# joejep/FOCNeRF

Hardware: AMD Instinct MI355X
Metric: train_samples_per_sec (higher is better)
Workload: dtype f16

## Files before the change

focnerf_amd/_lib.py:

```python
import ctypes
import os

import torch

_HERE = os.path.dirname(os.path.abspath(__file__))
LIB_PATH = os.environ.get("FOCNERF_LIB_PATH") or os.path.join(_HERE, "libfocnerf_hip.so")

c_u8p = ctypes.c_void_p
c_vp = ctypes.c_void_p
u32 = ctypes.c_uint32
u64 = ctypes.c_uint64
f32 = ctypes.c_float
i32 = ctypes.c_int

FOC_F32 = 0
FOC_F16 = 1



class FocOccTrainNode(ctypes.Structure):
    _fields_ = [
        ("struct_bytes", u32),
        ("n_rays", u32), ("max_steps", u32), ("cascade", u32), ("grid_size", u32), ("cap", u32), ("pad_align", u32),
        ("bound", f32), ("dt_gamma", f32), ("min_near", f32),
        ("rays_o", c_vp), ("rays_d", c_vp), ("aabb", c_vp), ("jitter", c_vp),
        ("bitfield", c_vp),
        ("nears", c_vp), ("fars", c_vp), ("enc_in", c_vp), ("deltas", c_vp),
        ("sh_rows", c_vp),
        ("rays", c_vp), ("counter", c_vp), ("march_scratch", c_vp),
        ("levels", u32), ("base_resolution", u32), ("gridtype", u32), ("interp", u32),
        ("align_corners", ctypes.c_int32), ("table_dtype", ctypes.c_int32),
        ("per_level_scale_log2", f32),
        ("embeddings", c_vp),
        ("offsets", c_vp), ("offsets_host", c_vp),
        ("planes", c_vp), ("grid_workspace", c_vp),
        ("grid_workspace_bytes", u64),
        ("sigma_input_dim", u32), ("sigma_hidden", u32), ("sigma_layers", u32), ("sigma_activation", u32), ("sigma_output_activation", u32),
        ("color_hidden", u32), ("color_layers", u32), ("color_activation", u32), ("c_width", u32),
        ("w_sigma", c_vp), ("w_color", c_vp),
        ("h", c_vp), ("c", c_vp),
        ("T_thresh", f32), ("density_scale", f32), ("bg_scalar", f32),
        ("bg_ray", c_vp),
        ("weights_sum", c_vp), ("image_raw", c_vp), ("image", c_vp), ("depth", c_vp),
        ("precounted", ctypes.c_int32),
        ("grad_image", c_vp), ("grad_ws", c_vp),
        ("grad_c", c_vp), ("grad_h0", c_vp), ("grad_h", c_vp), ("grad_planes", c_vp), ("grad_w_color", c_vp), ("grad_w_sigma", c_vp),
        ("grad_embeddings", c_vp), ("mlp_workspace", c_vp),
        ("mlp_workspace_bytes", u64),
    ]


class FocOccTrainObject(ctypes.Structure):
    _fields_ = [
        ("struct_bytes", u32),
        ("input_pad", f32),
        ("obj_feat", c_vp),
        ("ray_sumsq", c_vp),
        ("grad_sumsq", c_vp),
        ("grad_obj", c_vp),
    ]


class FocOccTrainTail(ctypes.Structure):
    _fields_ = [
        ("struct_bytes", u32),
        ("ray_dist", c_vp), ("ray_wm", c_vp), ("depth_raw", c_vp),
        ("grad_dist", c_vp), ("grad_depth", c_vp),
    ]


SIGNATURES = {
    "foc_abi_version": (i32, []),
    "foc_last_error": (ctypes.c_char_p, []),
    "foc_arch": (ctypes.c_char_p, []),
    "foc_near_far_from_aabb": (i32, [c_vp, c_vp, c_vp, u32, f32, c_vp, c_vp, c_vp]),
    "foc_sph_from_ray": (i32, [c_vp, c_vp, f32, u32, c_vp, c_vp]),
    "foc_morton3D": (i32, [c_vp, u32, c_vp, c_vp]),
    "foc_morton3D_invert": (i32, [c_vp, u32, c_vp, c_vp]),
    "foc_packbits": (i32, [c_vp, u32, f32, c_vp, c_vp]),
    "foc_march_rays_train": (i32, [c_vp, c_vp, c_vp, f32, f32, u32, u32, u32, u32, u32, c_vp, c_vp,
                                   c_vp, c_vp, c_vp, c_vp, c_vp, c_vp, c_vp, c_vp]),
    "foc_march_rays_train_field": (i32, [c_vp, c_vp, c_vp, f32, f32, u32, u32, u32, u32, u32, c_vp, c_vp,
                                         c_vp, c_vp, c_vp, c_vp, c_vp, c_vp, c_vp, u32, c_vp, f32, c_vp]),
    "foc_set_option": (i32, [ctypes.c_char_p, i32]),
    "foc_get_option": (i32, [ctypes.c_char_p, c_vp]),
    "foc_guard_pick_device": (i32, [i32, i32, i32, i32]),
    "foc_grid_forward_index_path": (i32, [u32, u32, u32]),
    "foc_view_tile_order": (i32, [c_vp, u32, u32, u32, c_vp, c_vp, c_vp]),
    "foc_occ_train_forward": (i32, [ctypes.POINTER(FocOccTrainNode), c_vp]),
    "foc_occ_train_backward": (i32, [ctypes.POINTER(FocOccTrainNode), c_vp]),
    "foc_occ_train_forward_pad31": (i32, [ctypes.POINTER(FocOccTrainNode), f32, c_vp]),
    "foc_occ_train_backward_pad31": (i32, [ctypes.POINTER(FocOccTrainNode), f32, c_vp]),
    "foc_occ_train_forward_obj": (i32, [ctypes.POINTER(FocOccTrainNode), ctypes.POINTER(FocOccTrainObject), c_vp]),
    "foc_occ_train_backward_obj": (i32, [ctypes.POINTER(FocOccTrainNode), ctypes.POINTER(FocOccTrainObject), c_vp]),
    "foc_occ_tail_forward_sumsq": (i32, [c_vp, c_vp, u32, c_vp, c_vp, u32, u32, f32, f32, c_vp, f32, c_vp, c_vp, c_vp, c_vp, c_vp, c_vp, c_vp, c_vp]),
    "foc_occ_tail_backward_sumsq": (i32, [c_vp, c_vp, c_vp, c_vp, u32, c_vp, c_vp, c_vp, c_vp, c_vp, u32, u32, f32, f32, c_vp, f32, c_vp, c_vp, c_vp, c_vp]),
    "foc_occ_tail_forward": (i32, [c_vp, c_vp, u32, c_vp, c_vp, u32, u32, f32, f32, c_vp, f32, c_vp, c_vp, c_vp, c_vp, c_vp, c_vp, c_vp]),
    "foc_occ_tail_backward": (i32, [c_vp, c_vp, c_vp, c_vp, u32, c_vp, c_vp, c_vp, c_vp, c_vp, u32, u32, f32, f32, c_vp, f32, c_vp, c_vp, c_vp]),
    "foc_occ_tail_forward_dist": (i32, [c_vp, c_vp, u32, c_vp, c_vp, u32, u32, f32, f32, c_vp, f32, c_vp, c_vp, c_vp, c_vp, c_vp, c_vp, c_vp, c_vp, c_vp,
                                        c_vp]),
    "foc_occ_tail_backward_dist": (i32, [c_vp, c_vp, c_vp, c_vp, u32, c_vp, c_vp, c_vp, c_vp, c_vp, u32, u32, f32, f32, c_vp, f32, c_vp, c_vp, c_vp, c_vp,
                                         c_vp, c_vp, c_vp]),
    "foc_occ_tail_forward_depth": (i32, [c_vp, c_vp, u32, c_vp, c_vp, u32, u32, f32, f32, c_vp, f32, c_vp, c_vp, c_vp, c_vp, c_vp, c_vp, c_vp, c_vp, c_vp,
                                         c_vp, c_vp]),
    "foc_occ_tail_backward_depth": (i32, [c_vp, c_vp, c_vp, c_vp, u32, c_vp, c_vp, c_vp, c_vp, c_vp, u32, u32, f32, f32, c_vp, f32, c_vp, c_vp, c_vp, c_vp,
                                          c_vp, c_vp, c_vp, c_vp, c_vp, c_vp, c_vp]),
    "foc_occ_train_forward_tail": (i32, [ctypes.POINTER(FocOccTrainNode), ctypes.POINTER(FocOccTrainObject), f32, ctypes.POINTER(FocOccTrainTail), c_vp]),
    "foc_occ_train_backward_tail": (i32, [ctypes.POINTER(FocOccTrainNode), ctypes.POINTER(FocOccTrainObject), f32, ctypes.POINTER(FocOccTrainTail), c_vp]),
    "foc_march_rays_train_scratch_bytes": (u64, [u32, u32]),
    "foc_composite_rays_train_forward": (i32, [c_vp, c_vp, c_vp, c_vp, u32, u32, f32, c_vp, c_vp, c_vp, c_vp]),
    "foc_composite_rays_train_backward": (i32, [c_vp, c_vp, c_vp, c_vp, c_vp, c_vp, c_vp, c_vp, u32, u32, f32,
                                                c_vp, c_vp, c_vp]),
    "foc_march_rays": (i32, [u32, u32, c_vp, c_vp, c_vp, c_vp, f32, f32, u32, u32, u32, c_vp, c_vp, c_vp,
                             c_vp, c_vp, c_vp, c_vp, c_vp]),
    "foc_composite_rays": (i32, [u32, u32, f32, c_vp, c_vp, c_vp, c_vp, c_vp, c_vp, c_vp, c_vp, c_vp]),
    "foc_compact_alive": (i32, [c_vp, u32, c_vp, c_vp, c_vp, c_vp]),
    "foc_march_rays_two_phase": (i32, [u32, u32, c_vp, c_vp, c_vp, c_vp, f32, f32, u32, u32, u32, c_vp, c_vp, c_vp, c_vp, c_vp, c_vp, c_vp, c_vp, i32, c_vp]),
    "foc_composite_compact": (i32, [u32, u32, f32, c_vp, c_vp, c_vp, c_vp, c_vp, c_vp, c_vp, c_vp, c_vp, c_vp, c_vp, c_vp, u32, u32, i32, c_vp]),
    "foc_march_rays_two_phase_fills": (i32, [u32, i32]),
    "foc_march_rays_two_phase_sample_major": (i32, [u32, u32, i32]),
    "foc_occ_render_step_scratch_bytes": (u64, [u32]),
    "foc_occ_render_step": (i32, [u32, u32, c_vp, c_vp, c_vp, c_vp, c_vp, c_vp, f32, f32, u32, u32, u32, c_vp, c_vp, c_vp, c_vp, c_vp, c_vp, c_vp, c_vp,
                                  c_vp, c_vp, c_vp, u32, f32, u32, c_vp, u32, c_vp, u32, u32, c_vp, f32, c_vp, c_vp, c_vp, c_vp, u32, c_vp, u32, u32, c_vp]),
    "foc_occ_render_step_pad31": (i32, [u32, u32, c_vp, c_vp, c_vp, c_vp, c_vp, c_vp, f32, f32, u32, u32, u32, c_vp, c_vp, c_vp, c_vp, c_vp, c_vp, c_vp, c_vp,
                                        c_vp, c_vp, c_vp, u32, f32, u32, c_vp, u32, c_vp, u32, u32, c_vp, f32, c_vp, c_vp, c_vp, c_vp, u32, c_vp, u32, u32, f32,
                                        c_vp]),
    "foc_occ_render_step_pad": (i32, [u32, u32, c_vp, c_vp, c_vp, c_vp, c_vp, c_vp, f32, f32, u32, u32, u32, c_vp, c_vp, c_vp, c_vp, c_vp, c_vp, c_vp, c_vp,
                                      c_vp, c_vp, c_vp, u32, f32, u32, c_vp, u32, c_vp, u32, u32, c_vp, f32, c_vp, c_vp, c_vp, c_vp, u32, c_vp, u32, u32, f32,
                                      c_vp]),
    "foc_grid_encode_forward": (i32, [c_vp, c_vp, c_vp, c_vp, u32, u32, u32, u32, f32, u32, c_vp, u32, i32, u32,
                                      i32, c_vp, c_vp]),
    "foc_grid_encode_forward_bl": (i32, [c_vp, c_vp, c_vp, c_vp, u32, u32, u32, u32, f32, u32, c_vp, u32, i32, u32,
                                         i32, c_vp, c_vp]),
    "foc_grid_encode_backward": (i32, [c_vp, c_vp, c_vp, c_vp, c_vp, u32, u32, u32, u32, f32, u32, c_vp, c_vp,
                                       u32, i32, u32, i32, i32, c_vp, c_vp]),
    "foc_grid_encode_backward_workspace_bytes": (u64, [u32, u32, u32, u32, i32]),
    "foc_grid_planes_to_rows": (i32, [c_vp, c_vp, u32, u32, u32, c_vp]),
    "foc_grid_rows_to_planes": (i32, [c_vp, c_vp, u32, u32, u32, c_vp]),
    "foc_grid_encode_backward_binned": (i32, [c_vp, c_vp, c_vp, c_vp, c_vp, u32, u32, u32, u32, f32, u32, c_vp, c_vp,
                                              u32, i32, u32, i32, i32, c_vp, c_vp, u64, c_vp]),
    "foc_grid_encode_forward_counted": (i32, [c_vp, c_vp, c_vp, c_vp, u32, u32, u32, u32, f32, u32, u32, i32, u32, i32, c_vp, c_vp, u64, c_vp]),
    "foc_grid_encode_backward_count": (i32, [c_vp, c_vp, u32, u32, u32, u32, f32, u32, u32, i32, u32, i32, c_vp, c_vp, u64, c_vp]),
    "foc_grid_encode_backward_binned_counted": (i32, [c_vp, c_vp, c_vp, c_vp, c_vp, u32, u32, u32, u32, f32, u32, c_vp, c_vp,
                                                      u32, i32, u32, i32, i32, c_vp, c_vp, u64, c_vp]),
    "foc_grad_total_variation": (i32, [c_vp, c_vp, c_vp, c_vp, f32, u32, u32, u32, u32, f32, u32, u32, i32, i32, c_vp]),
    "foc_freq_encode_forward": (i32, [c_vp, u32, u32, u32, u32, c_vp, c_vp]),
    "foc_freq_encode_backward": (i32, [c_vp, c_vp, u32, u32, u32, u32, c_vp, c_vp]),
    "foc_ffmlp_forward": (i32, [c_vp, c_vp, u32, u32, u32, u32, u32, u32, u32, c_vp, c_vp, c_vp]),
    "foc_ffmlp_inference": (i32, [c_vp, c_vp, u32, u32, u32, u32, u32, u32, u32, c_vp, c_vp, c_vp]),
    "foc_ffmlp_backward": (i32, [c_vp, c_vp, c_vp, c_vp, u32, u32, u32, u32, u32, u32, u32, i32,
                                 c_vp, c_vp, c_vp, c_vp, u64, c_vp]),
    "foc_ffmlp_backward_workspace_bytes": (u64, [u32, u32, u32]),
    "foc_ffmlp_forward_planar": (i32, [c_vp, c_vp, u32, u32, u32, u32, u32, u32, u32, c_vp, c_vp]),
    "foc_ffmlp_backward_planar": (i32, [c_vp, c_vp, c_vp, u32, u32, u32, u32, u32, u32, u32, i32, c_vp, c_vp, c_vp, u64, c_vp]),
    "foc_allocate_splitk": (i32, [u64]),
    "foc_free_splitk": (i32, []),
    "foc_combine_select": (i32, [c_vp, c_vp, c_vp, c_vp, u64, c_vp]),
    "foc_combine_pack_keys": (i32, [c_vp, u32, c_vp, u64, c_vp]),
    "foc_combine_unpack": (i32, [c_vp, u32, c_vp, c_vp, c_vp, u64, c_vp]),
    "foc_combine_select_composite": (i32, [c_vp, u32, c_vp, c_vp, u32, u32, c_vp, u32, c_vp, c_vp, c_vp, c_vp]),
    "foc_combine_select4": (i32, [c_vp, c_vp, u64, c_vp]),
    "foc_combine_select_composite_attr": (i32, [c_vp, u32, c_vp, c_vp, u32, c_vp, c_vp, u32, u32, c_vp, u32, c_vp, c_vp, c_vp, c_vp, c_vp, c_vp, c_vp, c_vp]),
    "foc_combine_select4_ids": (i32, [c_vp, u32, c_vp, c_vp, u64, c_vp]),
    "foc_mo_select": (i32, [c_vp, c_vp, c_vp, c_vp, u64, u32, u32, c_vp]),
    "foc_fixed_field_pack": (i32, [c_vp, c_vp, c_vp, c_vp, c_vp, c_vp, f32, u32, u32, f32, f32, c_vp, c_vp, c_vp, c_vp, u32, c_vp]),
    "foc_fixed_cull_scratch_bytes": (u64, [u32, u32]),
    "foc_fixed_cull": (i32, [c_vp, c_vp, c_vp, c_vp, c_vp, u32, u32, f32, c_vp, u32, u32, c_vp, c_vp, c_vp, c_vp, u64, c_vp]),
    "foc_fixed_cull_emit": (i32, [c_vp, c_vp, c_vp, c_vp, c_vp, u32, u32, f32, c_vp, c_vp, u32, c_vp, c_vp, c_vp]),
    "foc_fixed_field_pack_culled": (i32, [c_vp, c_vp, c_vp, c_vp, u32, c_vp, c_vp, u32, u32, f32, f32, c_vp, c_vp]),
    "foc_fixed_cull_placed": (i32, [c_vp, c_vp, c_vp, c_vp, c_vp, u32, u32, c_vp, c_vp, f32, c_vp, u32, u32, c_vp, c_vp, c_vp, c_vp, u64, c_vp]),
    "foc_fixed_cull_emit_placed": (i32, [c_vp, c_vp, c_vp, c_vp, c_vp, u32, u32, c_vp, f32, f32, c_vp, c_vp, u32, c_vp, c_vp, c_vp]),
    "foc_fixed_field_pack_culled_gain": (i32, [c_vp, c_vp, c_vp, c_vp, u32, c_vp, c_vp, u32, u32, f32, f32, f32, c_vp, c_vp]),
    "foc_composite_fixed_steps":(i32, [c_vp, c_vp, c_vp, c_vp, u32, u32, f32, c_vp, c_vp, c_vp]),
    "foc_fixed_sample": (i32, [c_vp, c_vp, c_vp, c_vp, c_vp, c_vp, u32, u32, f32, c_vp, c_vp, c_vp, u32, c_vp]),
    "foc_fixed_tail_forward": (i32, [c_vp, c_vp, c_vp, c_vp, c_vp, c_vp, f32, u32, u32, f32, f32, c_vp, c_vp, c_vp, c_vp, c_vp, c_vp, u32, c_vp, c_vp]),
    "foc_fixed_tail_backward": (i32, [c_vp, c_vp, c_vp, c_vp, c_vp, c_vp, c_vp, c_vp, c_vp, c_vp, c_vp, f32, u32, u32, f32, f32, c_vp, c_vp, u32, c_vp, c_vp]),
    "foc_fixed_tail_forward_dist": (i32, [c_vp, c_vp, c_vp, c_vp, c_vp, c_vp, f32, u32, u32, f32, f32, c_vp, c_vp, c_vp, c_vp, c_vp, c_vp, u32, c_vp, c_vp,
                                          c_vp, c_vp]),
    "foc_fixed_tail_backward_dist": (i32, [c_vp, c_vp, c_vp, c_vp, c_vp, c_vp, c_vp, c_vp, c_vp, c_vp, c_vp, c_vp, f32, u32, u32, f32, f32, c_vp, c_vp, u32,
                                           c_vp, c_vp, c_vp, c_vp, c_vp]),
    "foc_fixed_head_forward": (i32, [c_vp, c_vp, c_vp, c_vp, c_vp, u32, u32, f32, c_vp, c_vp, c_vp, c_vp, c_vp, c_vp, c_vp, u32, c_vp]),
    "foc_fixed_head_backward": (i32, [c_vp, c_vp, c_vp, c_vp, c_vp, c_vp, c_vp, c_vp, c_vp, c_vp, u32, u32, f32, c_vp, u32, c_vp]),
    "foc_color_head_forward": (i32, [c_vp, c_vp, u32, c_vp, u32, u32, u32, u32, c_vp, u32, c_vp, c_vp]),
    "foc_field_forward_train": (i32, [c_vp, c_vp, u32, c_vp, u32, c_vp, u32, u32, u32, u32, c_vp, c_vp, u32, c_vp, c_vp]),
    "foc_color_head_backward": (i32, [c_vp, c_vp, c_vp, u32, c_vp, c_vp, u32, u32, u32, u32, c_vp, c_vp, c_vp, u64, u32, c_vp, c_vp, c_vp]),
    "foc_color_head_forward_pad": (i32, [c_vp, c_vp, u32, c_vp, u32, u32, u32, u32, c_vp, u32, c_vp, f32, c_vp]),
    "foc_color_head_backward_pad": (i32, [c_vp, c_vp, c_vp, u32, c_vp, c_vp, u32, u32, u32, u32, c_vp, c_vp, c_vp, u64, u32, c_vp, c_vp, f32, c_vp]),
    "foc_field_forward_train_pad": (i32, [c_vp, c_vp, u32, c_vp, u32, c_vp, u32, u32, u32, u32, c_vp, c_vp, u32, c_vp, f32, c_vp]),
    "foc_color_head_forward_pad31": (i32, [c_vp, c_vp, u32, c_vp, u32, u32, u32, u32, c_vp, u32, c_vp, f32, c_vp]),
    "foc_color_head_backward_pad31": (i32, [c_vp, c_vp, c_vp, u32, c_vp, c_vp, u32, u32, u32, u32, c_vp, c_vp, c_vp, u64, u32, c_vp, c_vp, f32, c_vp]),
    "foc_field_forward_train_pad31": (i32, [c_vp, c_vp, u32, c_vp, u32, c_vp, u32, u32, u32, u32, c_vp, c_vp, u32, c_vp, f32, c_vp]),
    "foc_fixed_composite_forward": (i32, [c_vp, c_vp, c_vp, f32, u32, u32, f32, c_vp, c_vp]),
    "foc_fixed_composite_backward": (i32, [c_vp, c_vp, c_vp, c_vp, f32, u32, u32, f32, c_vp, c_vp, c_vp]),
    "foc_sample_head_forward": (i32, [c_vp, c_vp, u64, c_vp, c_vp, c_vp, u32, c_vp]),
    "foc_sample_head_backward": (i32, [c_vp, c_vp, c_vp, u64, c_vp, u32, c_vp]),
    "foc_sh_encode": (i32, [c_vp, u64, c_vp, c_vp]),
    "foc_rgb_head_forward": (i32, [c_vp, u64, c_vp, c_vp]),
    "foc_rgb_head_backward": (i32, [c_vp, c_vp, u64, c_vp, c_vp]),
    "foc_fixed_render_inference": (i32, [c_vp, c_vp, c_vp, c_vp, c_vp, c_vp, f32, u32, u32, f32, f32, c_vp, c_vp, c_vp, c_vp, u32, c_vp, c_vp]),
    "foc_nerf_field_inference": (i32, [c_vp, i32, c_vp, u32, u32, u32, c_vp, u32, c_vp, u32, u32, u32, u32, c_vp, c_vp, c_vp, c_vp]),
    "foc_nerf_field_inference_pad": (i32, [c_vp, i32, c_vp, u32, u32, u32, c_vp, u32, c_vp, u32, u32, u32, u32, c_vp, c_vp, c_vp, f32, c_vp]),
    "foc_nerf_field_inference_pad31": (i32, [c_vp, i32, c_vp, u32, u32, u32, c_vp, u32, c_vp, u32, u32, u32, u32, c_vp, c_vp, c_vp, f32, c_vp]),
    "foc_mark_untrained_grid": (i32, [c_vp, u32, f32, f32, f32, f32, f32, u32, u32, c_vp, c_vp, c_vp]),
    "foc_grid_cells_xyz": (i32, [u32, u32, f32, c_vp, c_vp, c_vp]),
    "foc_grid_update_sample_workspace_bytes": (u64, [u32, u32]),
    "foc_grid_update_sample": (i32, [c_vp, u32, u32, f32, u32, c_vp, c_vp, c_vp, c_vp, c_vp, c_vp, u64, c_vp]),
    "foc_grid_update_apply_workspace_bytes": (u64, [u32, u32]),
    "foc_grid_update_apply": (i32, [c_vp, u32, u32, c_vp, c_vp, u32, f32, f32, f32, c_vp, c_vp, c_vp, u64, c_vp]),
    "foc_background_forward": (i32, [c_vp, c_vp, c_vp, f32, u32, c_vp, c_vp, f32, u32, c_vp, c_vp, c_vp]),
    "foc_background_backward_workspace_bytes": (u64, [u32]),
    "foc_background_backward": (i32, [c_vp, c_vp, c_vp, c_vp, f32, u32, c_vp, c_vp, f32, u32, c_vp, c_vp, c_vp, c_vp, u64, c_vp]),
}


def _load():
    if not os.path.exists(LIB_PATH):
        raise ImportError(
            f"focnerf_amd: {LIB_PATH} is missing. Build it with `python -c 'import __graft_entry__ as g; g.build()'` "
            f"or `make -C focnerf_amd/csrc`. There is no CPU or PyTorch fallback for these ops.")
    try:
        lib = ctypes.CDLL(LIB_PATH)
    except OSError as e:
        raise ImportError(f"focnerf_amd: failed to load {LIB_PATH}: {e}") from e
    for name, (res, args) in SIGNATURES.items():
        fn = getattr(lib, name)
        fn.restype = res
        fn.argtypes = args
    return lib


class _Stream(ctypes.c_void_p):
    device_index = None


_multi_device = None


def _on_tensor_device(fn):
    def call(*args):
        global _multi_device
        if _multi_device is None:
            _multi_device = torch.cuda.device_count() > 1
        if _multi_device and args:
            idx = getattr(args[-1], "device_index", None)
            if idx is not None and idx != torch.cuda.current_device():
                with torch.cuda.device(idx):
                    return fn(*args)
        return fn(*args)
    call.__name__ = getattr(fn, "__name__", "foc_call")
    return call


class _Lib:

    def __init__(self, cdll):
        self._cdll = cdll
        for name, (_, args) in SIGNATURES.items():
            fn = getattr(cdll, name)
            setattr(self, name, _on_tensor_device(fn) if args and args[-1] is c_vp and not name.endswith("_bytes") else fn)


lib = _Lib(_load())


def check(rc, what=""):
    if rc != 0:
        msg = lib.foc_last_error().decode("utf-8", "replace")
        raise RuntimeError(f"focnerf_amd {what}: {msg} (code {rc})")


def ptr(t):
    if t is None:
        return None
    return ctypes.c_void_p(t.data_ptr())


_raw_stream = getattr(torch._C, "_cuda_getCurrentRawStream", None) if os.environ.get("FOC_RAW_STREAM", "1") != "0" else None


def raw_stream(index):
    if _raw_stream is not None:
        return _raw_stream(index)
    return torch.cuda.current_stream(index).cuda_stream


def stream_of(t=None):
    dev = t.device if t is not None else None
    index = dev.index if dev is not None and dev.index is not None else torch.cuda.current_device()
    s = _Stream(raw_stream(index))
    s.device_index = index
    return s


def require_cuda(*tensors):
    for t in tensors:
        if t is not None and not t.is_cuda:
            raise RuntimeError("focnerf_amd: expected a CUDA(HIP) tensor; these ops have no CPU implementation")


def dtype_code(t):
    if t.dtype == torch.float32:
        return FOC_F32
    if t.dtype == torch.float16:
        return FOC_F16
    raise RuntimeError(f"focnerf_amd: unsupported dtype {t.dtype} (float32 or float16 expected)")


def get_option(name):
    v = ctypes.c_int(0)
    check(lib.foc_get_option(name.encode(), ctypes.cast(ctypes.byref(v), ctypes.c_void_p)), "get_option")
    return v.value


def set_option(name, value):
    check(lib.foc_set_option(name.encode(), int(value)), "set_option")


class option:

    def __init__(self, name, value):
        self.name, self.value = name, int(value)

    def __enter__(self):
        self.old = get_option(self.name)
        set_option(self.name, self.value)
        return self

# ... 4 lines not shown
```

focnerf_amd/csrc/combine.hip:

```cpp
#include "common.h"
#include "fs_common.h"
#include <string.h>

static thread_local char g_err[512] = "";

void foc_set_error(const char *fmt, ...) {
    va_list ap;
    va_start(ap, fmt);
    vsnprintf(g_err, sizeof(g_err), fmt, ap);
    va_end(ap);
}

__global__ void __launch_bounds__(256) k_combine_select(const float *__restrict__ dens, const float *__restrict__ rgb,
                                                        float *__restrict__ max_dens, float *__restrict__ best_rgb, uint64_t n) {
    for (uint64_t i = (uint64_t)blockIdx.x * 256 + threadIdx.x; i < n; i += (uint64_t)gridDim.x * 256) {
        const float d = dens[i], m = max_dens[i];
        if (d > m) { best_rgb[i * 3] = rgb[i * 3]; best_rgb[i * 3 + 1] = rgb[i * 3 + 1]; best_rgb[i * 3 + 2] = rgb[i * 3 + 2]; }
        max_dens[i] = (d != d || m != m) ? __builtin_nanf("") : (d > m ? d : m);
    }
}

__global__ void __launch_bounds__(256) k_combine_pack(const float *__restrict__ dens, uint32_t rank, uint64_t *__restrict__ keys, uint64_t n) {
    for (uint64_t i = (uint64_t)blockIdx.x * 256 + threadIdx.x; i < n; i += (uint64_t)gridDim.x * 256) {
        float d = dens[i];
// ... 64 lines not shown
__device__ __forceinline__ void combine_select_composite_body(const CombineFields &fields, const CombineAttr *at, uint32_t K,
                                                              const float *__restrict__ nears, const float *__restrict__ fars, uint32_t N,
                                                              uint32_t T, float bg0, float bg1, uint32_t n_bg, float *__restrict__ image4,
                                                              float *__restrict__ depth, float4 *__restrict__ merged4) {
    const uint32_t lane = threadIdx.x & 63;
    const uint32_t n = blockIdx.x * 4 + (threadIdx.x >> 6);
    if (n >= N) return;
    const FsGeom geo = fs_geom(nears, fars, n, T);
    float Tc = 1.0f, r = 0, g = 0, b = 0, a = 0, d = 0, ws = 0;
    float aw[NOBJ > 0 ? NOBJ : 1], ad[NOBJ > 0 ? NOBJ : 1];
    (void)aw; (void)ad;
    if constexpr (NOBJ > 0) {
#pragma unroll
        for (int k = 0; k < NOBJ; k++) aw[k] = ad[k] = 0.0f;
    }
    for (uint32_t base = 0; base < T; base += 64) {
        const uint32_t i = base + lane;
        const bool valid = i < T;
        float alpha = 0, sigma = 0, c0 = 0, c1 = 0, c2 = 0, oz = 0;
        uint32_t win = 0xFFu;
        if (valid) {
            const uint64_t s = (uint64_t)n * T + i;
            float4 best = fields.p[0][s];
            if constexpr (NOBJ > 0) win = at->plane[0] ? (uint32_t)at->plane[0][s] : at->id[0];
            for (uint32_t k = 1; k < K; k++) {
                const float4 f = fields.p[k][s];
                const float m = best.x;
                if constexpr (NOBJ > 0) {
                    const uint32_t idk = at->plane[k] ? (uint32_t)at->plane[k][s] : at->id[k];
                    if (f.x > m) win = idk;
                }
                if (f.x > m) { best.y = f.y; best.z = f.z; best.w = f.w; }
                best.x = (f.x != f.x || m != m) ? __builtin_nanf("") : (f.x > m ? f.x : m);
            }
            if (merged4) merged4[s] = best;
            if constexpr (NOBJ > 0) {
                if (at->winner) at->winner[s] = (uint8_t)win;
            }
            sigma = best.x; c0 = best.y; c1 = best.z; c2 = best.w;
            const FsSample p = fs_sample(geo, i, i, T, false, 0.0f, 0.0f);
            alpha = 1 - __expf(-p.delta * sigma);
            oz = p.oz;
        }
        const float om = valid ? (1 - alpha + 1e-15f) : 1.0f;
        const float w = alpha * fs_trans_scan(om, lane, Tc);
        r = fmaf(w, c0, r); g = fmaf(w, c1, g); b = fmaf(w, c2, b);
        a = fmaf(w, sigma, a); d = fmaf(w, oz, d); ws += w;
        if constexpr (NOBJ > 0) {
#pragma unroll
            for (int k = 0; k < NOBJ; k++) {
                const bool mine = win == (uint32_t)k;
                aw[k] = mine ? aw[k] + w : aw[k];
                ad[k] = mine ? fmaf(w, oz, ad[k]) : ad[k];
            }
        }
    }
    r = wave_sum(r); g = wave_sum(g); b = wave_sum(b); a = wave_sum(a); d = wave_sum(d); ws = wave_sum(ws);
    if constexpr (NOBJ > 0) {
        const uint32_t n_obj = at->n_obj;
        float my_w = 0.0f, my_d = 0.0f, top = 0.0f;
        int32_t inst = -1;
#pragma unroll
        for (int k = 0; k < NOBJ; k++) {
            if ((uint32_t)k < n_obj) {
                const float sw = wave_sum(aw[k]), sd = wave_sum(ad[k]);
                if (lane == (uint32_t)k) { my_w = sw; my_d = sd; }
                if (sw > top) { top = sw; inst = k; }
            }
        }
        if (lane < n_obj) {
            at->obj_weights[(uint64_t)n * n_obj + lane] = my_w;
            at->obj_depth[(uint64_t)n * n_obj + lane] = my_d;
        }
        if (lane == 0) at->instance[n] = inst;
    }
    if (lane == 0) {
        for (uint32_t q = 0; q < n_bg; q++) {
            const float rest = (1 - ws) * (q == 0 ? bg0 : bg1);
            const float o[4] = {r + rest, g + rest, b + rest, a + rest};
#pragma unroll
            for (int k = 0; k < 4; k++) image4[((uint64_t)q * N + n) * 4 + k] = fminf(1.0f, fmaxf(0.0f, o[k]));
        }
        depth[n] = d;
    }
}

__global__ void __launch_bounds__(256) k_combine_select_composite(CombineFields fields, uint32_t K, const float *__restrict__ nears,
                                                                  const float *__restrict__ fars, uint32_t N, uint32_t T, float bg0, float bg1,
                                                                  uint32_t n_bg, float *__restrict__ image4, float *__restrict__ depth,
                                                                  float4 *__restrict__ merged4) {
    combine_select_composite_body<0>(fields, nullptr, K, nears, fars, N, T, bg0, bg1, n_bg, image4, depth, merged4);
}

template <int NOBJ>
__global__ void __launch_bounds__(256) k_combine_select_composite_attr(CombineFields fields, CombineAttr at, uint32_t K,
                                                                       const float *__restrict__ nears, const float *__restrict__ fars, uint32_t N,
                                                                       uint32_t T, float bg0, float bg1, uint32_t n_bg, float *__restrict__ image4,
                                                                       float *__restrict__ depth, float4 *__restrict__ merged4) {
    combine_select_composite_body<NOBJ>(fields, &at, K, nears, fars, N, T, bg0, bg1, n_bg, image4, depth, merged4);
}

__global__ void __launch_bounds__(256) k_combine_select4(const float4 *__restrict__ f4, float4 *__restrict__ acc4, uint64_t n) {
    for (uint64_t i = (uint64_t)blockIdx.x * 256 + threadIdx.x; i < n; i += (uint64_t)gridDim.x * 256) {
        const float4 f = f4[i];
        float4 best = acc4[i];
        const float m = best.x;
        if (f.x > m) { best.y = f.y; best.z = f.z; best.w = f.w; }
        best.x = (f.x != f.x || m != m) ? __builtin_nanf("") : (f.x > m ? f.x : m);
        acc4[i] = best;
    }
}

__global__ void __launch_bounds__(256) k_combine_select4_ids(const float4 *__restrict__ f4, uint8_t id, float4 *__restrict__ acc4,
                                                             uint8_t *__restrict__ acc_ids, uint64_t n) {
    for (uint64_t i = (uint64_t)blockIdx.x * 256 + threadIdx.x; i < n; i += (uint64_t)gridDim.x * 256) {
        const float4 f = f4[i];
        float4 best = acc4[i];
        const float m = best.x;
        if (f.x > m) { best.y = f.y; best.z = f.z; best.w = f.w; acc_ids[i] = id; }
        best.x = (f.x != f.x || m != m) ? __builtin_nanf("") : (f.x > m ? f.x : m);
        acc4[i] = best;
    }
}

template <typename T>
__global__ void __launch_bounds__(256) k_mo_select(const T *__restrict__ sig_new, const T *__restrict__ feat_new, T *__restrict__ sig_best,
                                                   T *__restrict__ feat_best, uint64_t n, uint32_t width) {
    const uint64_t s0 = ((uint64_t)blockIdx.x * 4u + (threadIdx.x >> 6)) * 64u;
    if (s0 >= n) return;
    const uint32_t lane = threadIdx.x & 63u;
    bool take = false;
    if (s0 + lane < n) {
        const T a_raw = sig_new[s0 + lane];
        const float a = (float)a_raw, b = (float)sig_best[s0 + lane];
        take = (a != a) || (b == b && a >= b);
        if (take) sig_best[s0 + lane] = a_raw;
    }
    const uint64_t rows = __ballot(take);
    const uint32_t live = (uint32_t)(n - s0 < 64u ? n - s0 : 64u);
    const uint64_t base = s0 * width;
    for (uint32_t e = lane; e < live * width; e += 64u)
        if ((rows >> (e / width)) & 1ull) feat_best[base + e] = feat_new[base + e];
}

#include <stdlib.h>
#include <string.h>
#include <atomic>
#include <mutex>
struct FocOptionRow { const char *name; std::atomic<int> value; };
static FocOptionRow foc_option_table[FOC_OPT_COUNT] = {
    {"FOC_MLP_BWD_FUSED", 1}, {"FOC_FIELD_FWD_FUSED", 1}, {"FOC_GB_MERGE_MAX_RES", 480}, {"FOC_GB_FACTORED", 1}, {"FOC_GB_TAIL_SPLIT", 16}, {"FOC_GRID_FUSE_SMALL", 1},
    {"FOC_GRID_PAIRS", 1}, {"FOC_GRID_FAST", 1}, {"FOC_MARCH_SERIAL", -1}, {"FOC_MARCH_RAYS_ROW_MAX", 131072}, {"FOC_OCC_MARCH_FORM", -1},
    {"FOC_OCC_SAMPLE_MAJOR", 1}, {"FOC_OCC_FIELD_PIECE", 1 << 23}, {"FOC_DETERMINISTIC", 0},
};
static int foc_option_parse(int which, const char *text) {
    if (which == FOC_OPT_OCC_MARCH_FORM) {
        if (text[0] == 't') return 0;
        if (text[0] == 'r') return 1;
        if (text[0] == 'l') return 2;
        if (text[0] == 's') return 3;
    }
    return atoi(text);
}
static void foc_options_init() {
    static std::once_flag once;
    std::call_once(once, [] {
        for (int i = 0; i < FOC_OPT_COUNT; i++) {
            const char *e = getenv(foc_option_table[i].name);
            if (e && e[0]) foc_option_table[i].value.store(foc_option_parse(i, e), std::memory_order_relaxed);
        }
    });
}
int foc_opt(FocOpt which) { foc_options_init(); return foc_option_table[which].value.load(std::memory_order_relaxed); }

extern "C" {

int foc_set_option(const char *name, int value) {
    foc_options_init();
    for (int i = 0; i < FOC_OPT_COUNT; i++)
        if (name && strcmp(name, foc_option_table[i].name) == 0) { foc_option_table[i].value.store(value, std::memory_order_relaxed); return FOC_OK; }
    foc_set_error("set_option: unknown option '%s'", name ? name : "(null)");
    return FOC_E_INVALID;
}

int foc_get_option(const char *name, int *value) {
    foc_options_init();
    for (int i = 0; i < FOC_OPT_COUNT; i++)
        if (name && value && strcmp(name, foc_option_table[i].name) == 0) { *value = foc_option_table[i].value.load(std::memory_order_relaxed); return FOC_OK; }
    foc_set_error("get_option: unknown option '%s'", name ? name : "(null)");
    return FOC_E_INVALID;
}

int foc_guard_pick_device(int stream_is_null, int stream_device, int pointer_device, int current_device) {
    return foc_guard_pick(stream_is_null != 0, stream_device, pointer_device, current_device);
}


int foc_combine_select_composite(const float *const *fields4, uint32_t K, const float *nears, const float *fars, uint32_t N, uint32_t T,
                                 const float *bgs, uint32_t n_bg, float *image4, float *depth, float *merged4, void *stream) {
    FocDeviceGuard foc_guard_(stream, nears);
    FOC_REQUIRE(K >= 1 && K <= FOC_COMBINE_MAX_OBJECTS, FOC_E_INVALID, "combine_select_composite: 1 <= K <= %d objects per call (got %u)",
                FOC_COMBINE_MAX_OBJECTS, K);
    FOC_REQUIRE(n_bg >= 1 && n_bg <= 2 && bgs, FOC_E_INVALID, "combine_select_composite: one or two backgrounds");
    FOC_REQUIRE(T >= 2, FOC_E_INVALID, "combine_select_composite: T must be >= 2");
    if (N == 0) return FOC_OK;
    FOC_REQUIRE(fields4 && nears && fars && image4 && depth, FOC_E_INVALID, "combine_select_composite: null pointer");
    CombineFields f;
    for (uint32_t k = 0; k < FOC_COMBINE_MAX_OBJECTS; k++) {
        f.p[k] = reinterpret_cast<const float4 *>(k < K ? fields4[k] : fields4[0]);
        FOC_REQUIRE(f.p[k] && ((uintptr_t)f.p[k] & 15) == 0, FOC_E_INVALID, "combine_select_composite: field %u is null or not 16-byte aligned", k);
    }
    FOC_REQUIRE(((uintptr_t)merged4 & 15) == 0, FOC_E_INVALID, "combine_select_composite: merged4 must be 16-byte aligned");
    hipLaunchKernelGGL(k_combine_select_composite, dim3(foc_div_up(N, 4)), dim3(256), 0, (hipStream_t)stream, f, K, nears, fars, N, T, bgs[0],
                       n_bg > 1 ? bgs[1] : 0.0f, n_bg, image4, depth, reinterpret_cast<float4 *>(merged4));
    FOC_CHECK_LAUNCH("combine_select_composite");
    return FOC_OK;
}

int foc_combine_select4(const float *field4, float *acc4, uint64_t n, void *stream) {
    FocDeviceGuard foc_guard_(stream, field4);
    FOC_REQUIRE(n == 0 || (field4 && acc4), FOC_E_INVALID, "combine_select4: null pointer");
    FOC_REQUIRE((((uintptr_t)field4 | (uintptr_t)acc4) & 15) == 0, FOC_E_INVALID, "combine_select4: fields must be 16-byte aligned");
    if (n == 0) return FOC_OK;
    hipLaunchKernelGGL(k_combine_select4, dim3(foc_grid_1d(n, 256)), dim3(256), 0, (hipStream_t)stream, reinterpret_cast<const float4 *>(field4),
                       reinterpret_cast<float4 *>(acc4), n);
    FOC_CHECK_LAUNCH("combine_select4");
    return FOC_OK;
}

int foc_combine_select_composite_attr(const float *const *fields4, uint32_t K, const uint8_t *const *id_planes, const uint32_t *ids,
                                      uint32_t n_obj, const float *nears, const float *fars, uint32_t N, uint32_t T, const float *bgs,
                                      uint32_t n_bg, float *image4, float *depth, float *merged4, float *obj_weights, float *obj_depth,
                                      int32_t *instance, uint8_t *winner, void *stream) {
    FocDeviceGuard foc_guard_(stream, nears);
    FOC_REQUIRE(K >= 1 && K <= FOC_COMBINE_MAX_OBJECTS, FOC_E_INVALID, "combine_select_composite_attr: 1 <= K <= %d fields per call (got %u)",
                FOC_COMBINE_MAX_OBJECTS, K);
    FOC_REQUIRE(n_obj >= 1 && n_obj <= FOC_COMBINE_MAX_OBJECTS, FOC_E_INVALID, "combine_select_composite_attr: 1 <= n_obj <= %d objects (got %u)",
                FOC_COMBINE_MAX_OBJECTS, n_obj);
    FOC_REQUIRE(n_bg >= 1 && n_bg <= 2 && bgs, FOC_E_INVALID, "combine_select_composite_attr: one or two backgrounds");
    FOC_REQUIRE(T >= 2, FOC_E_INVALID, "combine_select_composite_attr: T must be >= 2");
    FOC_REQUIRE(fields4, FOC_E_INVALID, "combine_select_composite_attr: fields4 is null");
    CombineFields f;
    CombineAttr at;
    for (uint32_t k = 0; k < FOC_COMBINE_MAX_OBJECTS; k++) {
        const uint32_t j = k < K ? k : 0;
        at.plane[k] = id_planes ? id_planes[j] : nullptr;
        FOC_REQUIRE(at.plane[k] || ids, FOC_E_INVALID, "combine_select_composite_attr: field %u has neither an id plane nor a constant id (ids is null)", j);
        at.id[k] = at.plane[k] ? 0u : ids[j];
        FOC_REQUIRE(at.id[k] < n_obj, FOC_E_INVALID, "combine_select_composite_attr: ids[%u] = %u is not below n_obj = %u", j, at.id[k], n_obj);
    }
    if (N == 0) return FOC_OK;
    FOC_REQUIRE(nears && fars && image4 && depth, FOC_E_INVALID, "combine_select_composite_attr: null pointer");
    FOC_REQUIRE(obj_weights && obj_depth && instance, FOC_E_INVALID, "combine_select_composite_attr: obj_weights, obj_depth and instance must not be null");
    for (uint32_t k = 0; k < FOC_COMBINE_MAX_OBJECTS; k++) {
        f.p[k] = reinterpret_cast<const float4 *>(k < K ? fields4[k] : fields4[0]);
        FOC_REQUIRE(f.p[k] && ((uintptr_t)f.p[k] & 15) == 0, FOC_E_INVALID, "combine_select_composite_attr: field %u is null or not 16-byte aligned", k);
    }
    FOC_REQUIRE(((uintptr_t)merged4 & 15) == 0, FOC_E_INVALID, "combine_select_composite_attr: merged4 must be 16-byte aligned");
    FOC_REQUIRE(((uintptr_t)obj_weights & 3) == 0 && ((uintptr_t)obj_depth & 3) == 0 && ((uintptr_t)instance & 3) == 0, FOC_E_INVALID,
                "combine_select_composite_attr: obj_weights, obj_depth and instance must be 4-byte aligned");
    at.n_obj = n_obj;
    at.obj_weights = obj_weights; at.obj_depth = obj_depth; at.instance = instance; at.winner = winner;
    const dim3 grid(foc_div_up(N, 4)), block(256);
    const float bg1 = n_bg > 1 ? bgs[1] : 0.0f;
    float4 *m4 = reinterpret_cast<float4 *>(merged4);
    if (n_obj <= 4)
        hipLaunchKernelGGL(k_combine_select_composite_attr<4>, grid, block, 0, (hipStream_t)stream, f, at, K, nears, fars, N, T, bgs[0], bg1, n_bg, image4, depth, m4);
    else if (n_obj <= 8)
        hipLaunchKernelGGL(k_combine_select_composite_attr<8>, grid, block, 0, (hipStream_t)stream, f, at, K, nears, fars, N, T, bgs[0], bg1, n_bg, image4, depth, m4);
    else
        hipLaunchKernelGGL(k_combine_select_composite_attr<16>, grid, block, 0, (hipStream_t)stream, f, at, K, nears, fars, N, T, bgs[0], bg1, n_bg, image4, depth, m4);
    FOC_CHECK_LAUNCH("combine_select_composite_attr");
    return FOC_OK;
}

int foc_combine_select4_ids(const float *field4, uint32_t id, float *acc4, uint8_t *acc_ids, uint64_t n, void *stream) {
    FocDeviceGuard foc_guard_(stream, field4);
    FOC_REQUIRE(id < FOC_COMBINE_MAX_OBJECTS, FOC_E_INVALID, "combine_select4_ids: id %u is not below %d", id, FOC_COMBINE_MAX_OBJECTS);
    FOC_REQUIRE(n == 0 || (field4 && acc4 && acc_ids), FOC_E_INVALID, "combine_select4_ids: null pointer");
    FOC_REQUIRE((((uintptr_t)field4 | (uintptr_t)acc4) & 15) == 0, FOC_E_INVALID, "combine_select4_ids: fields must be 16-byte aligned");
    if (n == 0) return FOC_OK;
    hipLaunchKernelGGL(k_combine_select4_ids, dim3(foc_grid_1d(n, 256)), dim3(256), 0, (hipStream_t)stream, reinterpret_cast<const float4 *>(field4),
                       (uint8_t)id, reinterpret_cast<float4 *>(acc4), acc_ids, n);
    FOC_CHECK_LAUNCH("combine_select4_ids");
    return FOC_OK;
}

int foc_mo_select(const void *sigma_new, const void *feat_new, void *sigma_best, void *feat_best, uint64_t n, uint32_t feat_width,
                  uint32_t elem_bytes, void *stream) {
    FocDeviceGuard foc_guard_(stream, sigma_new);
    FOC_REQUIRE(elem_bytes == 2 || elem_bytes == 4, FOC_E_INVALID, "mo_select: elem_bytes must be 2 (half) or 4 (float), got %u", elem_bytes);
    FOC_REQUIRE(feat_width >= 1 && feat_width <= 64, FOC_E_INVALID, "mo_select: feat_width %u outside 1..64", feat_width);
    FOC_REQUIRE(n == 0 || (sigma_new && feat_new && sigma_best && feat_best), FOC_E_INVALID, "mo_select: null pointer");
    FOC_REQUIRE(n < (1ull << 38), FOC_E_INVALID, "mo_select: n too large");
    if (n == 0) return FOC_OK;
    const dim3 grid((uint32_t)((n + 255u) / 256u));
    if (elem_bytes == 2)
        hipLaunchKernelGGL(k_mo_select<__half>, grid, dim3(256), 0, (hipStream_t)stream, (const __half *)sigma_new, (const __half *)feat_new,
                           (__half *)sigma_best, (__half *)feat_best, n, feat_width);
    else
        hipLaunchKernelGGL(k_mo_select<float>, grid, dim3(256), 0, (hipStream_t)stream, (const float *)sigma_new, (const float *)feat_new,
                           (float *)sigma_best, (float *)feat_best, n, feat_width);
    FOC_CHECK_LAUNCH("mo_select");
    return FOC_OK;
}

// ... 44 lines not shown
```

focnerf_amd/csrc/common.h:

```cpp
#pragma once
#include <hip/hip_runtime.h>
#include <hip/hip_fp16.h>
#include <stdint.h>
#include <stdio.h>
#include <stdarg.h>
#include "../../include/focnerf.h"

#define FOC_WAVE 64

void foc_set_error(const char *fmt, ...);

enum FocOpt {
    FOC_OPT_MLP_BWD_FUSED,
    FOC_OPT_FIELD_FWD_FUSED,
    FOC_OPT_GB_MERGE_MAX_RES,
    FOC_OPT_GB_FACTORED,
    FOC_OPT_GB_TAIL_SPLIT,
    FOC_OPT_GRID_FUSE_SMALL,
    FOC_OPT_GRID_PAIRS,
    FOC_OPT_GRID_FAST,
    FOC_OPT_MARCH_SERIAL,
    FOC_OPT_MARCH_RAYS_ROW_MAX,
    FOC_OPT_OCC_MARCH_FORM,
    FOC_OPT_OCC_SAMPLE_MAJOR,
    FOC_OPT_OCC_FIELD_PIECE,
    FOC_OPT_DETERMINISTIC,
    FOC_OPT_COUNT
};
int foc_opt(FocOpt which);

#define FOC_REQUIRE(cond, code, ...)                    \
    do {                                                \
        if (!(cond)) {                                  \
            foc_set_error(__VA_ARGS__);                 \
            return (code);                              \
        }                                               \
    } while (0)

#define FOC_CHECK_LAUNCH(name)                                                     \
    do {                                                                           \
        hipError_t e_ = hipGetLastError();                                         \
        if (e_ != hipSuccess) {                                                    \
            foc_set_error("%s: launch failed: %s", name, hipGetErrorString(e_));   \
            return FOC_E_LAUNCH;                                                   \
        }                                                                          \
    } while (0)

static inline int foc_guard_pick(bool stream_is_null, int stream_device, int pointer_device, int current_device) {
    if (!stream_is_null && stream_device >= 0) return stream_device;
    if (pointer_device >= 0) return pointer_device;
    return current_device;
}
struct FocDeviceGuard {
    int prev = -1;
    explicit FocDeviceGuard(void *stream, const void *first_pointer = nullptr) {
        static int n_devices = -1;
        if (n_devices < 0 && hipGetDeviceCount(&n_devices) != hipSuccess) { (void)hipGetLastError(); n_devices = 0; }
        if (n_devices == 1) return;
        int cur = 0;
        if (hipGetDevice(&cur) != hipSuccess) return;
        int sdev = -1, pdev = -1;
        if (stream != nullptr) {
            if (hipStreamGetDevice(static_cast<hipStream_t>(stream), &sdev) != hipSuccess) { (void)hipGetLastError(); sdev = -1; }
        } else if (first_pointer != nullptr) {
            hipPointerAttribute_t attr;
            if (hipPointerGetAttributes(&attr, first_pointer) == hipSuccess && attr.type == hipMemoryTypeDevice) pdev = attr.device;
            else (void)hipGetLastError();
        }
        const int want = foc_guard_pick(stream == nullptr, sdev, pdev, cur);
        if (want != cur && hipSetDevice(want) == hipSuccess) prev = cur;
    }
    ~FocDeviceGuard() { if (prev >= 0) (void)hipSetDevice(prev); }
    FocDeviceGuard(const FocDeviceGuard &) = delete;
    FocDeviceGuard &operator=(const FocDeviceGuard &) = delete;
};

static inline uint32_t foc_div_up(uint64_t a, uint64_t b) { return (uint32_t)((a + b - 1) / b); }

static inline uint32_t foc_grid_1d(uint64_t n, uint32_t block, uint32_t max_blocks = 256 * 8) {
    uint64_t g = (n + block - 1) / block;
    if (g < 1) g = 1;
    if (g > max_blocks) g = max_blocks;
    return (uint32_t)g;
}

__device__ __forceinline__ _Float16 foc_f2h(float v) { asm volatile("" : "+v"(v)); return (_Float16)v; }

__global__ static void __launch_bounds__(256) k_foc_zero(uint32_t *__restrict__ p, uint64_t n_words) {
    for (uint64_t i = (uint64_t)blockIdx.x * 256 + threadIdx.x; i < n_words; i += (uint64_t)gridDim.x * 256) p[i] = 0u;
}
static inline hipError_t foc_zero_async(void *p, size_t bytes, hipStream_t st) {
    const uint64_t n = bytes / 4;
    if (n == 0) return hipSuccess;
    uint64_t blocks = (n + 255) / 256;
    if (blocks > 4096) blocks = 4096;
    hipLaunchKernelGGL(k_foc_zero, dim3((uint32_t)blocks), dim3(256), 0, st, reinterpret_cast<uint32_t *>(p), n);
    return hipGetLastError();
}

__device__ __forceinline__ void foc_lds_barrier() { asm volatile("s_waitcnt lgkmcnt(0)\n\ts_barrier" ::: "memory"); }

__device__ __forceinline__ float wave_sum(float v) {
#pragma unroll
    for (int o = 32; o > 0; o >>= 1) v += __shfl_xor(v, o, 64);
    return v;
}
__device__ __forceinline__ int wave_sum_i(int v) {
#pragma unroll
    for (int o = 32; o > 0; o >>= 1) v += __shfl_xor(v, o, 64);
    return v;
}
__device__ __forceinline__ float wave_incl_prod(float v, int lane) {
#pragma unroll
    for (int o = 1; o < 64; o <<= 1) {
        float u = __shfl_up(v, o, 64);
        if (lane >= o) v *= u;
    }
    return v;
}
__device__ __forceinline__ float wave_prod_scan(float om, uint32_t lane, float &P) {
    P = wave_incl_prod(om, (int)lane);
    float Pex = __shfl_up(P, 1, 64);
    if (lane == 0) Pex = 1.0f;
    return Pex;
}
__device__ __forceinline__ float wave_incl_sum(float v, int lane) {
#pragma unroll
    for (int o = 1; o < 64; o <<= 1) {
        float u = __shfl_up(v, o, 64);
        if (lane >= o) v += u;
    }
    return v;
}
__device__ __forceinline__ int wave_incl_sum_i(int v, int lane) {
#pragma unroll
    for (int o = 1; o < 64; o <<= 1) {
        int u = __shfl_up(v, o, 64);
        if (lane >= o) v += u;
    }
    return v;
}
```

focnerf_amd/csrc/fixedstep.hip:

```cpp
#include "common.h"
#include "fs_common.h"
#include <float.h>

__global__ void __launch_bounds__(256) k_fs_sample(const float *__restrict__ rays_o, const float *__restrict__ rays_d, const float *__restrict__ nears,
                                                   const float *__restrict__ fars, const float *__restrict__ aabb, const float *__restrict__ noise,
                                                   uint32_t N, uint32_t T, float bound, float *__restrict__ xyzs, float *__restrict__ enc_in,
                                                   _Float16 *__restrict__ ray_sh, uint32_t ray_block) {
    const uint64_t total = ray_block ? (uint64_t)((N + FS_RAY_BLOCK - 1) / FS_RAY_BLOCK) * FS_RAY_BLOCK * T : (uint64_t)N * T;
    const FsBox box = fs_box(aabb);
    const float two_b = 2 * bound;
    for (uint64_t s = (uint64_t)blockIdx.x * 256 + threadIdx.x; s < total; s += (uint64_t)gridDim.x * 256) {
        uint32_t n, i;
        bool own = true;
        if (ray_block) {
            const uint32_t blk = (uint32_t)(s / ((uint64_t)FS_RAY_BLOCK * T)), in = (uint32_t)(s - (uint64_t)blk * FS_RAY_BLOCK * T);
            i = in / FS_RAY_BLOCK;
            n = blk * FS_RAY_BLOCK + in % FS_RAY_BLOCK;
            own = n < N;
            n = own ? n : N - 1;
        } else {
            n = (uint32_t)(s / T); i = (uint32_t)(s - (uint64_t)n * T);
        }
        const FsGeom g = fs_geom(nears, fars, n, T);
        const float z = fs_z(g, i, T, noise, (uint64_t)n * T + i);
        float x, y, w;
        fs_point(rays_o[n * 3], rays_o[n * 3 + 1], rays_o[n * 3 + 2], rays_d[n * 3], rays_d[n * 3 + 1], rays_d[n * 3 + 2], z, box, x, y, w);
        if (xyzs) { xyzs[s * 3] = x; xyzs[s * 3 + 1] = y; xyzs[s * 3 + 2] = w; }
        if (enc_in) { enc_in[s * 3] = fs_norm(x, bound, two_b); enc_in[s * 3 + 1] = fs_norm(y, bound, two_b); enc_in[s * 3 + 2] = fs_norm(w, bound, two_b); }
        if (ray_sh && i == 0 && own) {
            h8 lo, hi;
            foc_sh16_h(rays_d[n * 3], rays_d[n * 3 + 1], rays_d[n * 3 + 2], lo, hi);
            h8 *dst = reinterpret_cast<h8 *>(ray_sh + (uint64_t)n * 16);
            dst[0] = lo; dst[1] = hi;
        }
    }
}

__global__ void __launch_bounds__(256) k_fs_head_fwd(const _Float16 *__restrict__ h, const float *__restrict__ rays_d, const float *__restrict__ nears,
                                                     const float *__restrict__ fars, const float *__restrict__ noise, uint32_t N, uint32_t T,
                                                     float density_scale, float *__restrict__ sigma_out, float *__restrict__ trans_out,
                                                     float *__restrict__ weights_out, float *__restrict__ weights_sum, float *__restrict__ depth,
                                                     _Float16 *__restrict__ cin, const _Float16 *__restrict__ obj, uint32_t cin_ld) {
    const uint32_t lane = threadIdx.x & 63;
    const uint32_t n = blockIdx.x * 4 + (threadIdx.x >> 6);
    if (n >= N) return;
    const FsGeom g = fs_geom(nears, fars, n, T);
    h8 shlo, shhi;
    h8 ob1 = {0, 0, 0, 0, 0, 0, 0, 0}, ob2 = {0, 0, 0, 0, 0, 0, 0, 0};
    _Float16 ob0 = (_Float16)0;
    if (cin) {
        foc_sh16_h(rays_d[n * 3], rays_d[n * 3 + 1], rays_d[n * 3 + 2], shlo, shhi);
        if (obj) {
            ob0 = obj[0];
#pragma unroll
            for (int k = 0; k < 8; k++) ob1[k] = obj[1 + k];
#pragma unroll
            for (int k = 0; k < 7; k++) ob2[k] = obj[9 + k];
        }
    }
    float Tc = 1.0f, ws = 0, dp = 0;
    for (uint32_t base = 0; base < T; base += 64) {
        const uint32_t i = base + lane;
        const bool valid = i < T;
        const uint64_t s = (uint64_t)n * T + (valid ? i : T - 1);
        h8 r0, r1;
        if (cin) { r0 = *reinterpret_cast<const h8 *>(h + s * 16); r1 = *reinterpret_cast<const h8 *>(h + s * 16 + 8); }
        else r0[0] = h[s * 16];
        const float sigma = expf((float)r0[0]);
        const FsSample p = fs_sample_ld(g, i, valid ? i : T - 1, T, noise, s);
        const float alpha = valid ? 1 - expf((-p.delta * density_scale) * sigma) : 0.0f;
        const float om = valid ? (1 - alpha + 1e-15f) : 1.0f;
        const float Tb = fs_trans_scan(om, lane, Tc);
        const float w = alpha * Tb;
        if (valid) {
            sigma_out[s] = sigma; trans_out[s] = Tb; weights_out[s] = w;
            ws += w; dp += w * p.oz;
            if (cin) {
                h8 c2, c3;
#pragma unroll
                for (int k = 0; k < 7; k++) { c2[k] = r0[k + 1]; c3[k] = r1[k + 1]; }
                c2[7] = r1[0]; c3[7] = ob0;
                h8 *dst = reinterpret_cast<h8 *>(cin + s * cin_ld);
                dst[0] = shlo; dst[1] = shhi; dst[2] = c2; dst[3] = c3;
                if (cin_ld == 48) { dst[4] = ob1; dst[5] = ob2; }
            }
        }
    }
    ws = wave_sum(ws); dp = wave_sum(dp);
    if (lane == 0) { weights_sum[n] = ws; depth[n] = dp; }
}

__global__ void __launch_bounds__(256) k_fs_head_bwd(const _Float16 *__restrict__ h, const float *__restrict__ sigma_in, const float *__restrict__ trans_in,
                                                     const float *__restrict__ nears, const float *__restrict__ fars, const float *__restrict__ noise,
                                                     const float *__restrict__ grad_w, const float *__restrict__ grad_ws, const float *__restrict__ grad_depth,
                                                     const _Float16 *__restrict__ grad_cin, uint32_t N, uint32_t T, float density_scale,
                                                     _Float16 *__restrict__ grad_h, uint32_t cin_ld) {
    const uint32_t lane = threadIdx.x & 63;
    const uint32_t n = blockIdx.x * 4 + (threadIdx.x >> 6);
    if (n >= N) return;
    const FsGeom g = fs_geom(nears, fars, n, T);
    const float gws = grad_ws ? grad_ws[n] : 0.0f, gdp = grad_depth ? grad_depth[n] : 0.0f;
    float S_carry = 0.0f;
    const uint32_t n_chunks = (T + 63) / 64;
    for (uint32_t cidx = n_chunks; cidx-- > 0;) {
        const uint32_t i = cidx * 64 + lane;
        const bool valid = i < T;
        const uint64_t s = (uint64_t)n * T + (valid ? i : T - 1);
        const float sigma = sigma_in[s], Tb = trans_in[s];
        const FsSample p = fs_sample_ld(g, i, valid ? i : T - 1, T, noise, s);
        const float dsigma = fs_head_bwd_step(p, valid, sigma, Tb, (grad_w ? grad_w[s] : 0.0f) + gws, gdp, density_scale, lane, S_carry);
        const float dh0 = dsigma * foc_trunc_exp_bwd((float)h[s * 16]);
        if (valid) {
            h8 o0, o1;
            if (grad_cin) {
                const h8 c2 = *reinterpret_cast<const h8 *>(grad_cin + s * cin_ld + 16), c3 = *reinterpret_cast<const h8 *>(grad_cin + s * cin_ld + 24);
#pragma unroll
                for (int k = 0; k < 7; k++) { o0[k + 1] = c2[k]; o1[k + 1] = c3[k]; }
                o1[0] = c2[7];
            } else {
#pragma unroll
                for (int k = 0; k < 8; k++) { o0[k] = (_Float16)0; o1[k] = (_Float16)0; }
            }
            o0[0] = foc_f2h(dh0);
            h8 *dst = reinterpret_cast<h8 *>(grad_h + s * 16);
            dst[0] = o0; dst[1] = o1;
        }
    }
}

__global__ void __launch_bounds__(256) k_fs_composite_fwd(const _Float16 *__restrict__ c, const float *__restrict__ weights, const float *__restrict__ bg_ray,
                                                          float bg_scalar, uint32_t N, uint32_t T, float thresh, float *__restrict__ image) {
    const uint32_t lane = threadIdx.x & 63;
    const uint32_t n = blockIdx.x * 4 + (threadIdx.x >> 6);
    if (n >= N) return;
    float r = 0, g = 0, b = 0, ws = 0;
    for (uint32_t i = lane; i < T; i += 64) {
        const uint64_t s = (uint64_t)n * T + i;
        const float w = weights[s];
        ws += w;
        if (w > thresh) {
            const uint2 raw = *reinterpret_cast<const uint2 *>(c + s * 16);
            const _Float16 *cc = reinterpret_cast<const _Float16 *>(&raw);
            r += w * foc_sigmoid_h((float)cc[0]); g += w * foc_sigmoid_h((float)cc[1]); b += w * foc_sigmoid_h((float)cc[2]);
        }
    }
    r = wave_sum(r); g = wave_sum(g); b = wave_sum(b); ws = wave_sum(ws);
    if (lane == 0) {
        const FocBg bg = foc_bg(bg_ray, bg_scalar, n);
        image[n * 3] = r + (1 - ws) * bg.b0; image[n * 3 + 1] = g + (1 - ws) * bg.b1; image[n * 3 + 2] = b + (1 - ws) * bg.b2;
    }
}

__global__ void __launch_bounds__(256) k_fs_composite_bwd(const float *__restrict__ grad_image, const _Float16 *__restrict__ c, const float *__restrict__ weights,
                                                          const float *__restrict__ bg_ray, float bg_scalar, uint32_t N, uint32_t T, float thresh,
                                                          _Float16 *__restrict__ grad_c, float *__restrict__ grad_w) {
    const uint64_t total = (uint64_t)N * T;
    for (uint64_t s = (uint64_t)blockIdx.x * 256 + threadIdx.x; s < total; s += (uint64_t)gridDim.x * 256) {
        const uint32_t n = (uint32_t)(s / T);
        const FsRayGrad q = fs_ray_grad(grad_image, bg_ray, bg_scalar, n);
        h8 o0;
        const h8 o1 = {0, 0, 0, 0, 0, 0, 0, 0};
        grad_w[s] = fs_composite_bwd_sample(q, weights[s], thresh, c + s * 16, o0);
        h8 *dst = reinterpret_cast<h8 *>(grad_c + s * 16);
        dst[0] = o0; dst[1] = o1;
    }
}

template <bool NOISE, bool DIST>
__global__ void __launch_bounds__(256) k_fs_tail_fwd(const _Float16 *__restrict__ h, const _Float16 *__restrict__ c, const float *__restrict__ nears,
                                                     const float *__restrict__ fars, const float *__restrict__ noise, const float *__restrict__ bg_ray,
                                                     float bg_scalar, uint32_t N, uint32_t T, float density_scale, float thresh,
                                                     float *__restrict__ sigma_out, float *__restrict__ trans_out, float *__restrict__ weights_out,
                                                     float *__restrict__ weights_sum, float *__restrict__ depth, float *__restrict__ image, uint32_t c_ld,
                                                     float *__restrict__ ray_sumsq, float *__restrict__ ray_dist, float *__restrict__ ray_wm) {
    const uint32_t lane = threadIdx.x & 63;
    const uint32_t n = blockIdx.x * 4 + (threadIdx.x >> 6);
    if (n >= N) return;
    const FsGeom g = fs_geom(nears, fars, n, T);
    float Tc = 1.0f, ws = 0, dp = 0, r = 0, gg = 0, b = 0, sq = 0;
    FsDist dist = {0, 0, 0};
    const bool live = g.far > g.near;
    for (uint32_t base = 0; base < T; base += 64) {
        const uint32_t i = base + lane;
        const bool valid = i < T;
        const uint32_t ic = valid ? i : T - 1;
        const uint64_t s = (uint64_t)n * T + ic;
        const _Float16 h0 = h[s * 16];
        const uint2 raw = *reinterpret_cast<const uint2 *>(c + s * c_ld);
        float u0 = 0.0f, u1 = 0.0f;
        if (NOISE) { u0 = noise[s]; u1 = noise[(uint64_t)n * T + min(ic + 1u, T - 1u)]; }
        const float sigma = expf((float)h0);
        const FsSample p = fs_sample(g, i, ic, T, NOISE, u0, u1);
        const float alpha = valid ? 1 - expf((-p.delta * density_scale) * sigma) : 0.0f;
        const float om = valid ? (1 - alpha + 1e-15f) : 1.0f;
        const float Tb = fs_trans_scan(om, lane, Tc);
        const float w = alpha * Tb;
        if constexpr (DIST) {
            if (live) fs_dist_fwd_step(dist, w, fs_dist_m(g, p), p.delta, lane);
        }
        if (valid) {
            sigma_out[s] = sigma; trans_out[s] = Tb; weights_out[s] = w;
            ws += w; dp += w * p.oz; sq = fmaf(sigma, sigma, sq);
            if (w > thresh) {
                const _Float16 *cc = reinterpret_cast<const _Float16 *>(&raw);
                r += w * foc_sigmoid_h((float)cc[0]); gg += w * foc_sigmoid_h((float)cc[1]); b += w * foc_sigmoid_h((float)cc[2]);
            }
        }
    }
    ws = wave_sum(ws); dp = wave_sum(dp); r = wave_sum(r); gg = wave_sum(gg); b = wave_sum(b);
    if (ray_sumsq) {
        sq = wave_sum(sq);
        if (lane == 0) ray_sumsq[n] = sq;
    }
    if constexpr (DIST) {
        const float ds = wave_sum(dist.acc);
        if (lane == 0) { ray_dist[n] = ds; ray_wm[n] = dist.WM; }
    }
    if (lane == 0) {
        const FocBg bg = foc_bg(bg_ray, bg_scalar, n);
        image[n * 3] = r + (1 - ws) * bg.b0; image[n * 3 + 1] = gg + (1 - ws) * bg.b1; image[n * 3 + 2] = b + (1 - ws) * bg.b2;
        weights_sum[n] = ws; depth[n] = dp;
    }
}

template <bool NOISE, bool DIST>
__global__ void __launch_bounds__(256) k_fs_tail_bwd(const float *__restrict__ grad_image, const float *__restrict__ grad_ws, const float *__restrict__ grad_depth,
                                                     const _Float16 *__restrict__ c, const float *__restrict__ sigma_in, const float *__restrict__ trans_in,
                                                     const float *__restrict__ weights, const float *__restrict__ nears, const float *__restrict__ fars,
                                                     const float *__restrict__ noise, const float *__restrict__ bg_ray, float bg_scalar, uint32_t N, uint32_t T,
                                                     float density_scale, float thresh, _Float16 *__restrict__ grad_c, _Float16 *__restrict__ grad_h0, uint32_t c_ld,
                                                     const float *__restrict__ grad_sumsq, const float *__restrict__ weights_sum,
                                                     const float *__restrict__ ray_wm, const float *__restrict__ grad_dist) {
    const uint32_t lane = threadIdx.x & 63;
    const uint32_t n = blockIdx.x * 4 + (threadIdx.x >> 6);
    if (n >= N) return;
    const FsGeom g = fs_geom(nears, fars, n, T);
    const float gws = grad_ws ? grad_ws[n] : 0.0f, gdp = grad_depth ? grad_depth[n] : 0.0f;
    const float gsq2 = grad_sumsq ? 2.0f * grad_sumsq[n] : 0.0f;
    float gdist = 0.0f, W_total = 0.0f, WM_total = 0.0f;
    FsDist dist = {0, 0, 0};
    if constexpr (DIST) {
        if (g.far > g.near) gdist = grad_dist[n];
        W_total = weights_sum[n]; WM_total = ray_wm[n];
    }
    const FsRayGrad q = fs_ray_grad(grad_image, bg_ray, bg_scalar, n);
    const FocExp15 e15 = foc_exp15();
    float S_carry = 0.0f;
    const uint32_t n_chunks = (T + 63) / 64;
    for (uint32_t cidx = n_chunks; cidx-- > 0;) {
        const uint32_t i = cidx * 64 + lane;
        const bool valid = i < T;
        const uint32_t ic = valid ? i : T - 1;
        const uint64_t s = (uint64_t)n * T + ic;
        const float sigma = sigma_in[s], Tb = trans_in[s], w = weights[s];
        const uint2 raw = *reinterpret_cast<const uint2 *>(c + s * c_ld);
        float u0 = 0.0f, u1 = 0.0f;
        if (NOISE) { u0 = noise[s]; u1 = noise[(uint64_t)n * T + min(ic + 1u, T - 1u)]; }
        h8 o0;
        const h8 o1 = {0, 0, 0, 0, 0, 0, 0, 0};
        const float gw = fs_composite_bwd_sample(q, w, thresh, reinterpret_cast<const _Float16 *>(&raw), o0);
        if (valid) {
            if (c_ld == 4u) *reinterpret_cast<uint2 *>(grad_c + s * 4) = *reinterpret_cast<const uint2 *>(&o0);
            else { h8 *dst = reinterpret_cast<h8 *>(grad_c + s * 16); dst[0] = o0; dst[1] = o1; }
        }
        const FsSample p = fs_sample(g, i, ic, T, NOISE, u0, u1);
        float gi = gw + gws;
        if constexpr (DIST) {
            if (gdist != 0.0f) gi = fmaf(gdist, fs_dist_bwd_step(dist, valid ? w : 0.0f, fs_dist_m(g, p), p.delta, W_total, WM_total, lane), gi);
        }
        float dsigma = fs_head_bwd_step(p, valid, sigma, Tb, gi, gdp, density_scale, lane, S_carry);
        if (gsq2 != 0.0f) dsigma = fmaf(gsq2, sigma, dsigma);
        const float dh0 = dsigma * foc_trunc_exp_bwd_of_sigma(sigma, e15);
        if (valid) grad_h0[s] = foc_f2h(dh0);
    }
}


template <bool PACK>
__device__ __forceinline__ void fs_infer_finish(FsRayAcc &a, uint32_t n, uint32_t lane, const float *__restrict__ bg_ray, float bg_scalar,
                                                float *__restrict__ image, float *__restrict__ depth, float *__restrict__ weights_sum) {
    const float ws = wave_sum(a.ws), dp = wave_sum(a.dp), r = wave_sum(a.r), gg = wave_sum(a.g), b = wave_sum(a.b);
    if (lane == 0 && (!PACK || image)) {
        const FocBg bg = foc_bg(bg_ray, bg_scalar, n);
        image[n * 3] = r + (1 - ws) * bg.b0; image[n * 3 + 1] = gg + (1 - ws) * bg.b1; image[n * 3 + 2] = b + (1 - ws) * bg.b2;
        depth[n] = dp;
        weights_sum[n] = ws;
    }
}

template <bool PACK>
__global__ void __launch_bounds__(256) k_fs_render_infer(const float *__restrict__ sigma_in, const float *__restrict__ rgb_in, const float *__restrict__ nears,
                                                         const float *__restrict__ fars, const float *__restrict__ noise, const float *__restrict__ bg_ray,
                                                         float bg_scalar, uint32_t N, uint32_t T, float density_scale, float thresh,
                                                         float *__restrict__ image, float *__restrict__ depth, float *__restrict__ weights_sum,
                                                         float *__restrict__ rgb_masked, float4 *__restrict__ field4) {
    const uint32_t lane = threadIdx.x & 63;
    const uint32_t n = blockIdx.x * 4 + (threadIdx.x >> 6);
    if (n >= N) return;
    const FsGeom g = fs_geom(nears, fars, n, T);
    FsRayAcc a = {1.0f, 0, 0, 0, 0, 0};
    for (uint32_t base = 0; base < T; base += 64) {
        const uint32_t i = base + lane;
        const bool valid = i < T;
        const uint64_t s = (uint64_t)n * T + (valid ? i : T - 1);
        const float sigma = sigma_in[s];
        float c0 = 0, c1 = 0, c2 = 0;
        if (valid) { c0 = rgb_in[s * 3]; c1 = rgb_in[s * 3 + 1]; c2 = rgb_in[s * 3 + 2]; }
        fs_infer_tile<PACK>(a, g, n, i, lane, T, sigma, c0, c1, c2, noise, density_scale, thresh, rgb_masked, field4, nullptr);
    }
    fs_infer_finish<PACK>(a, n, lane, bg_ray, bg_scalar, image, depth, weights_sum);
}

#define FS_BLK_RAYS 16u
template <bool PACK>
__global__ void __launch_bounds__(1024) k_fs_render_infer_blk(const float *__restrict__ sigma_in, const float *__restrict__ rgb_in, const float *__restrict__ nears,
                                                              const float *__restrict__ fars, const float *__restrict__ noise, const float *__restrict__ bg_ray,
                                                              float bg_scalar, uint32_t N, uint32_t T, float density_scale, float thresh,
                                                              float *__restrict__ image, float *__restrict__ depth, float *__restrict__ weights_sum,
                                                              float *__restrict__ rgb_masked, float4 *__restrict__ field4, float *__restrict__ sigma_rm) {
    __shared__ float tile_s[64][FS_BLK_RAYS + 1];
    __shared__ float tile_c[64][FS_BLK_RAYS * 3 + 1];
    const uint32_t tid = threadIdx.x, lane = tid & 63;
    const uint32_t wv = __builtin_amdgcn_readfirstlane(tid >> 6);
    const uint32_t n0 = blockIdx.x * FS_BLK_RAYS;
    const uint64_t row0 = fs_block_row(n0, 0, T);
    const bool is_s = tid < 256;
    const uint32_t li = is_s ? tid : tid - 256;
    const uint32_t l_step = is_s ? li >> 2 : li / 12, l_part = is_s ? (li & 3) : li % 12;
    const float *src = is_s ? sigma_in + row0 + l_part * 4 : rgb_in + row0 * 3 + l_part * 4;
    const uint32_t src_ld = is_s ? FS_RAY_BLOCK : FS_RAY_BLOCK * 3;
    float *dst = is_s ? &tile_s[l_step][l_part * 4] : &tile_c[l_step][l_part * 4];
    float4 nx = make_float4(0, 0, 0, 0);
    if (l_step < T) nx = *reinterpret_cast<const float4 *>(src + (uint64_t)l_step * src_ld);
    const uint32_t n = n0 + wv;
    const bool own = n < N;
    const FsGeom g = fs_geom(nears, fars, own ? n : N - 1, T);
    FsRayAcc a = {1.0f, 0, 0, 0, 0, 0};
    for (uint32_t base = 0; base < T; base += 64) {
        dst[0] = nx.x; dst[1] = nx.y; dst[2] = nx.z; dst[3] = nx.w;
        __syncthreads();
        if (base + 64 + l_step < T) nx = *reinterpret_cast<const float4 *>(src + (uint64_t)(base + 64 + l_step) * src_ld);
        if (own)
            fs_infer_tile<PACK>(a, g, n, base + lane, lane, T, tile_s[lane][wv], tile_c[lane][wv * 3], tile_c[lane][wv * 3 + 1], tile_c[lane][wv * 3 + 2],
                                noise, density_scale, thresh, rgb_masked, field4, sigma_rm);
        __syncthreads();
    }
    if (own) fs_infer_finish<PACK>(a, n, lane, bg_ray, bg_scalar, image, depth, weights_sum);
}

struct VtState { uint32_t count, first_enc, bad, pad; };

__device__ __forceinline__ bool vt_turn(const float *__restrict__ d, uint32_t i) {
    const float ax = d[(i + 1) * 3] - d[i * 3], ay = d[(i + 1) * 3 + 1] - d[i * 3 + 1], az = d[(i + 1) * 3 + 2] - d[i * 3 + 2];
    const float bx = d[(i + 2) * 3] - d[(i + 1) * 3], by = d[(i + 2) * 3 + 1] - d[(i + 1) * 3 + 1], bz = d[(i + 2) * 3 + 2] - d[(i + 1) * 3 + 2];
    return (bx * ax + by * ay) + bz * az < 0.0f;
}

__global__ void __launch_bounds__(256) k_vt_find(const float *__restrict__ d, uint32_t N, VtState *__restrict__ st) {
    for (uint32_t i = blockIdx.x * 256 + threadIdx.x; i + 2 < N; i += gridDim.x * 256)
        if (vt_turn(d, i)) { atomicAdd(&st->count, 1u); atomicMax(&st->first_enc, N - i); }
}

__global__ void __launch_bounds__(256) k_vt_check(const float *__restrict__ d, uint32_t N, VtState *__restrict__ st) {
    const uint32_t fe = st->first_enc;
    if (fe == 0u) return;
    const uint32_t W = N - fe + 2u;
    for (uint32_t i = blockIdx.x * 256 + threadIdx.x; i + 2 < N; i += gridDim.x * 256) {
        const bool expect = (i + 2u) % W == 0u || (i + 1u) % W == 0u;
        if (vt_turn(d, i) != expect) st->bad = 1u;
    }
}

__global__ void __launch_bounds__(256) k_vt_perm(uint32_t N, uint32_t th, uint32_t tw, const VtState *__restrict__ st, int64_t *__restrict__ perm) {
    const uint32_t fe = st->first_enc, W = fe ? N - fe + 2u : 0u;
    const uint32_t H = W ? N / W : 0u;
    const bool grid = W >= 16u && N % W == 0u && H >= 8u && st->count == 2u * (H - 1u) && st->bad == 0u;
    for (uint32_t p = blockIdx.x * 256 + threadIdx.x; p < N; p += gridDim.x * 256) {
        uint32_t src = p;
        if (grid) {
            const uint64_t wt = (uint64_t)W * th;
            const uint32_t ty = (uint32_t)(p / wt), rem = (uint32_t)(p - ty * wt);
            const uint32_t rows_here = min(th, H - ty * th);
            const uint32_t tx = min(rem / (rows_here * tw), (W - 1u) / tw), r2 = rem - tx * rows_here * tw;
            const uint32_t cols_here = min(tw, W - tx * tw);
            src = (ty * th + r2 / cols_here) * W + tx * tw + r2 % cols_here;
        }
        perm[p] = (int64_t)src;
    }
}

extern "C" {

int foc_fixed_sample(const float *rays_o, const float *rays_d, const float *nears, const float *fars, const float *aabb, const float *noise,
                     uint32_t N, uint32_t T, float bound, float *xyzs, float *enc_in, void *ray_sh, uint32_t ray_block, void *stream) {
    FocDeviceGuard foc_guard_(stream, rays_o);
    if (N == 0) return FOC_OK;
    FOC_REQUIRE(rays_o && rays_d && nears && fars && aabb && (xyzs || enc_in), FOC_E_INVALID, "fixed_sample: null pointer");
    FOC_REQUIRE(T >= 2, FOC_E_INVALID, "fixed_sample: T must be >= 2");
    FOC_REQUIRE(ray_block == 0 || ray_block == FS_RAY_BLOCK, FOC_E_INVALID, "fixed_sample: ray_block must be 0 (ray-major) or %u (got %u)", FS_RAY_BLOCK, ray_block);
    const uint64_t rows = ray_block ? (uint64_t)foc_div_up(N, FS_RAY_BLOCK) * FS_RAY_BLOCK * T : (uint64_t)N * T;
    hipLaunchKernelGGL(k_fs_sample, dim3(foc_grid_1d(rows, 256, 256 * 16)), dim3(256), 0, (hipStream_t)stream, rays_o, rays_d, nears, fars, aabb,
                       noise, N, T, bound, xyzs, enc_in, (_Float16 *)ray_sh, ray_block);
    FOC_CHECK_LAUNCH("fixed_sample");
    return FOC_OK;
}

int foc_fixed_head_forward(const void *h, const float *rays_d, const float *nears, const float *fars, const float *noise, uint32_t N, uint32_t T,
                           float density_scale, float *sigma, float *trans, float *weights, float *weights_sum, float *depth, void *cin,
                           const void *obj_feat, uint32_t cin_width, void *stream) {
    FocDeviceGuard foc_guard_(stream, h);
    if (N == 0) return FOC_OK;
    FOC_REQUIRE(h && rays_d && nears && fars && sigma && trans && weights && weights_sum && depth, FOC_E_INVALID, "fixed_head_forward: null pointer");
    FOC_REQUIRE(T >= 2, FOC_E_INVALID, "fixed_head_forward: T must be >= 2");
    FOC_REQUIRE(cin_width == 32 || cin_width == 48, FOC_E_INVALID, "fixed_head_forward: cin_width must be 32 or 48 (got %u)", cin_width);
    FOC_REQUIRE(!obj_feat || cin_width == 48, FOC_E_INVALID, "fixed_head_forward: an object feature needs the 48-wide colour input");
    hipLaunchKernelGGL(k_fs_head_fwd, dim3(foc_div_up(N, 4)), dim3(256), 0, (hipStream_t)stream, (const _Float16 *)h, rays_d, nears, fars, noise, N, T,
                       density_scale, sigma, trans, weights, weights_sum, depth, (_Float16 *)cin, (const _Float16 *)obj_feat, cin_width);
    FOC_CHECK_LAUNCH("fixed_head_forward");
    return FOC_OK;
}

int foc_fixed_head_backward(const void *h, const float *sigma, const float *trans, const float *nears, const float *fars, const float *noise,
                            const float *grad_w, const float *grad_ws, const float *grad_depth, const void *grad_cin, uint32_t N, uint32_t T,
                            float density_scale, void *grad_h, uint32_t cin_width, void *stream) {
    FocDeviceGuard foc_guard_(stream, h);
    if (N == 0) return FOC_OK;
    FOC_REQUIRE(h && sigma && trans && nears && fars && grad_h, FOC_E_INVALID, "fixed_head_backward: null pointer");
    FOC_REQUIRE(T >= 2, FOC_E_INVALID, "fixed_head_backward: T must be >= 2");
    FOC_REQUIRE(cin_width == 32 || cin_width == 48, FOC_E_INVALID, "fixed_head_backward: cin_width must be 32 or 48 (got %u)", cin_width);
    hipLaunchKernelGGL(k_fs_head_bwd, dim3(foc_div_up(N, 4)), dim3(256), 0, (hipStream_t)stream, (const _Float16 *)h, sigma, trans, nears, fars, noise,
                       grad_w, grad_ws, grad_depth, (const _Float16 *)grad_cin, N, T, density_scale, (_Float16 *)grad_h, cin_width);
    FOC_CHECK_LAUNCH("fixed_head_backward");
    return FOC_OK;
}

int foc_fixed_composite_forward(const void *c, const float *weights, const float *bg_ray, float bg_scalar, uint32_t N, uint32_t T, float thresh,
                                float *image, void *stream) {
    FocDeviceGuard foc_guard_(stream, c);
    if (N == 0) return FOC_OK;
    FOC_REQUIRE(c && weights && image, FOC_E_INVALID, "fixed_composite_forward: null pointer");
    hipLaunchKernelGGL(k_fs_composite_fwd, dim3(foc_div_up(N, 4)), dim3(256), 0, (hipStream_t)stream, (const _Float16 *)c, weights, bg_ray, bg_scalar, N, T,
                       thresh, image);
    FOC_CHECK_LAUNCH("fixed_composite_forward");
    return FOC_OK;
}

int foc_fixed_composite_backward(const float *grad_image, const void *c, const float *weights, const float *bg_ray, float bg_scalar, uint32_t N,
                                 uint32_t T, float thresh, void *grad_c, float *grad_w, void *stream) {
    FocDeviceGuard foc_guard_(stream, grad_image);
    if (N == 0) return FOC_OK;
    FOC_REQUIRE(grad_image && c && weights && grad_c && grad_w, FOC_E_INVALID, "fixed_composite_backward: null pointer");
    hipLaunchKernelGGL(k_fs_composite_bwd, dim3(foc_grid_1d((uint64_t)N * T, 256, 256 * 16)), dim3(256), 0, (hipStream_t)stream, grad_image,
                       (const _Float16 *)c, weights, bg_ray, bg_scalar, N, T, thresh, (_Float16 *)grad_c, grad_w);
    FOC_CHECK_LAUNCH("fixed_composite_backward");
    return FOC_OK;
}

static int fixed_tail_forward(const char *who, const void *h, const void *c, const float *nears, const float *fars, const float *noise, const float *bg_ray,
                              float bg_scalar, uint32_t N, uint32_t T, float density_scale, float thresh, float *sigma, float *trans, float *weights,
                              float *weights_sum, float *depth, float *image, uint32_t c_width, float *ray_sumsq, float *ray_dist, float *ray_wm, void *stream) {
    FocDeviceGuard foc_guard_(stream, h);
    if (N == 0) return FOC_OK;
    FOC_REQUIRE(c_width == 16 || c_width == 4, FOC_E_INVALID, "%s: c_width must be 16 or 4 (got %u)", who, c_width);
    FOC_REQUIRE(h && c && nears && fars && sigma && trans && weights && weights_sum && depth && image, FOC_E_INVALID, "%s: null pointer", who);
    FOC_REQUIRE(T >= 2, FOC_E_INVALID, "%s: T must be >= 2", who);
    auto kern = ray_dist ? (noise ? k_fs_tail_fwd<true, true> : k_fs_tail_fwd<false, true>) : (noise ? k_fs_tail_fwd<true, false> : k_fs_tail_fwd<false, false>);
    hipLaunchKernelGGL(kern, dim3(foc_div_up(N, 4)), dim3(256), 0, (hipStream_t)stream, (const _Float16 *)h, (const _Float16 *)c, nears, fars, noise,
                       bg_ray, bg_scalar, N, T, density_scale, thresh, sigma, trans, weights, weights_sum, depth, image, c_width, ray_sumsq, ray_dist, ray_wm);
    FOC_CHECK_LAUNCH(who);
    return FOC_OK;
}

int foc_fixed_tail_forward(const void *h, const void *c, const float *nears, const float *fars, const float *noise, const float *bg_ray, float bg_scalar,
                           uint32_t N, uint32_t T, float density_scale, float thresh, float *sigma, float *trans, float *weights, float *weights_sum,
                           float *depth, float *image, uint32_t c_width, float *ray_sumsq, void *stream) {
    return fixed_tail_forward("fixed_tail_forward", h, c, nears, fars, noise, bg_ray, bg_scalar, N, T, density_scale, thresh, sigma, trans, weights, weights_sum,
                              depth, image, c_width, ray_sumsq, nullptr, nullptr, stream);
}

int foc_fixed_tail_forward_dist(const void *h, const void *c, const float *nears, const float *fars, const float *noise, const float *bg_ray, float bg_scalar,
                                uint32_t N, uint32_t T, float density_scale, float thresh, float *sigma, float *trans, float *weights, float *weights_sum,
                                float *depth, float *image, uint32_t c_width, float *ray_sumsq, float *ray_dist, float *ray_wm, void *stream) {
    FOC_REQUIRE((ray_dist && ray_wm) || N == 0, FOC_E_INVALID, "fixed_tail_forward_dist: null ray_dist / ray_wm");
    return fixed_tail_forward("fixed_tail_forward_dist", h, c, nears, fars, noise, bg_ray, bg_scalar, N, T, density_scale, thresh, sigma, trans, weights,
                              weights_sum, depth, image, c_width, ray_sumsq, ray_dist, ray_wm, stream);
}

static int fixed_tail_backward(const char *who, const float *grad_image, const float *grad_ws, const float *grad_depth, const void *c, const float *sigma,
                               const float *trans, const float *weights, const float *nears, const float *fars, const float *noise, const float *bg_ray,
                               float bg_scalar, uint32_t N, uint32_t T, float density_scale, float thresh, void *grad_c, void *grad_h0, uint32_t c_width,
                               const float *grad_sumsq, const float *weights_sum, const float *ray_wm, const float *grad_dist, void *stream) {
    FocDeviceGuard foc_guard_(stream, grad_image);
    if (N == 0) return FOC_OK;
    FOC_REQUIRE(c_width == 16 || c_width == 4, FOC_E_INVALID, "%s: c_width must be 16 or 4 (got %u)", who, c_width);
    FOC_REQUIRE(grad_image && c && sigma && trans && weights && nears && fars && grad_c && grad_h0, FOC_E_INVALID, "%s: null pointer", who);
    FOC_REQUIRE(T >= 2, FOC_E_INVALID, "%s: T must be >= 2", who);
    auto kern = grad_dist ? (noise ? k_fs_tail_bwd<true, true> : k_fs_tail_bwd<false, true>) : (noise ? k_fs_tail_bwd<true, false> : k_fs_tail_bwd<false, false>);
    hipLaunchKernelGGL(kern, dim3(foc_div_up(N, 4)), dim3(256), 0, (hipStream_t)stream, grad_image, grad_ws, grad_depth, (const _Float16 *)c, sigma,
                       trans, weights, nears, fars, noise, bg_ray, bg_scalar, N, T, density_scale, thresh, (_Float16 *)grad_c, (_Float16 *)grad_h0, c_width,
                       grad_sumsq, weights_sum, ray_wm, grad_dist);
    FOC_CHECK_LAUNCH(who);
    return FOC_OK;
}

int foc_fixed_tail_backward(const float *grad_image, const float *grad_ws, const float *grad_depth, const void *c, const float *sigma, const float *trans,
                            const float *weights, const float *nears, const float *fars, const float *noise, const float *bg_ray, float bg_scalar,
                            uint32_t N, uint32_t T, float density_scale, float thresh, void *grad_c, void *grad_h0, uint32_t c_width, const float *grad_sumsq,
                            void *stream) {
    return fixed_tail_backward("fixed_tail_backward", grad_image, grad_ws, grad_depth, c, sigma, trans, weights, nears, fars, noise, bg_ray, bg_scalar, N, T,
                               density_scale, thresh, grad_c, grad_h0, c_width, grad_sumsq, nullptr, nullptr, nullptr, stream);
}

int foc_fixed_tail_backward_dist(const float *grad_image, const float *grad_ws, const float *grad_depth, const void *c, const float *sigma, const float *trans,
                                 const float *weights, const float *weights_sum, const float *nears, const float *fars, const float *noise, const float *bg_ray,
                                 float bg_scalar, uint32_t N, uint32_t T, float density_scale, float thresh, void *grad_c, void *grad_h0, uint32_t c_width,
                                 const float *grad_sumsq, const float *ray_wm, const float *ray_dist, const float *grad_dist, void *stream) {
    (void)ray_dist;
    FOC_REQUIRE(!grad_dist || (weights_sum && ray_wm) || N == 0, FOC_E_INVALID, "fixed_tail_backward_dist: grad_dist needs weights_sum and ray_wm");
    return fixed_tail_backward("fixed_tail_backward_dist", grad_image, grad_ws, grad_depth, c, sigma, trans, weights, nears, fars, noise, bg_ray, bg_scalar, N,
                               T, density_scale, thresh, grad_c, grad_h0, c_width, grad_sumsq, weights_sum, ray_wm, grad_dist, stream);
}

int foc_fixed_render_inference(const float *sigma, const float *rgb, const float *nears, const float *fars, const float *noise, const float *bg_ray,
                               float bg_scalar, uint32_t N, uint32_t T, float density_scale, float thresh, float *image, float *depth, float *weights_sum,
                               float *rgb_masked, uint32_t ray_block, float *sigma_raymajor, void *stream) {
    FocDeviceGuard foc_guard_(stream, sigma);
    if (N == 0) return FOC_OK;
    FOC_REQUIRE(sigma && rgb && nears && fars && image && depth && weights_sum, FOC_E_INVALID, "fixed_render_inference: null pointer");
    FOC_REQUIRE(T >= 2, FOC_E_INVALID, "fixed_render_inference: T must be >= 2");
    FOC_REQUIRE(ray_block == 0 || ray_block == FS_RAY_BLOCK, FOC_E_INVALID, "fixed_render_inference: ray_block must be 0 or %u (got %u)", FS_RAY_BLOCK, ray_block);
    FOC_REQUIRE(ray_block || !sigma_raymajor, FOC_E_INVALID, "fixed_render_inference: sigma_raymajor is the un-blocked copy of a blocked sigma (ray_block == 0: sigma already is ray-major)");
    if (ray_block) {
        FOC_REQUIRE((((uintptr_t)sigma | (uintptr_t)rgb) & 15) == 0, FOC_E_INVALID, "fixed_render_inference: blocked sigma / rgb must be 16-byte aligned");
        hipLaunchKernelGGL(k_fs_render_infer_blk<false>, dim3(foc_div_up(N, FS_BLK_RAYS)), dim3(1024), 0, (hipStream_t)stream, sigma, rgb, nears, fars, noise, bg_ray, bg_scalar,
                           N, T, density_scale, thresh, image, depth, weights_sum, rgb_masked, (float4 *)nullptr, sigma_raymajor);
        FOC_CHECK_LAUNCH("fixed_render_inference");
        return FOC_OK;
    }
    hipLaunchKernelGGL(k_fs_render_infer<false>, dim3(foc_div_up(N, 4)), dim3(256), 0, (hipStream_t)stream, sigma, rgb, nears, fars, noise, bg_ray, bg_scalar, N, T,
                       density_scale, thresh, image, depth, weights_sum, rgb_masked, (float4 *)nullptr);
    FOC_CHECK_LAUNCH("fixed_render_inference");
    return FOC_OK;
}

int foc_fixed_field_pack(const float *sigma, const float *rgb, const float *nears, const float *fars, const float *noise, const float *bg_ray,
                         float bg_scalar, uint32_t N, uint32_t T, float density_scale, float thresh, float *image, float *depth, float *weights_sum,
                         float *field4, uint32_t ray_block, void *stream) {
    FocDeviceGuard foc_guard_(stream, sigma);
    if (N == 0) return FOC_OK;
    FOC_REQUIRE(sigma && rgb && nears && fars && field4, FOC_E_INVALID, "fixed_field_pack: null pointer");
    FOC_REQUIRE((image && depth && weights_sum) || (!image && !depth && !weights_sum), FOC_E_INVALID,
                "fixed_field_pack: image, depth and weights_sum go together (all or none)");
    FOC_REQUIRE(((uintptr_t)field4 & 15) == 0, FOC_E_INVALID, "fixed_field_pack: field4 must be 16-byte aligned");
    FOC_REQUIRE(T >= 2, FOC_E_INVALID, "fixed_field_pack: T must be >= 2");
    FOC_REQUIRE(ray_block == 0 || ray_block == FS_RAY_BLOCK, FOC_E_INVALID, "fixed_field_pack: ray_block must be 0 or %u (got %u)", FS_RAY_BLOCK, ray_block);
    if (ray_block) {
        FOC_REQUIRE((((uintptr_t)sigma | (uintptr_t)rgb) & 15) == 0, FOC_E_INVALID, "fixed_field_pack: blocked sigma / rgb must be 16-byte aligned");
        hipLaunchKernelGGL(k_fs_render_infer_blk<true>, dim3(foc_div_up(N, FS_BLK_RAYS)), dim3(1024), 0, (hipStream_t)stream, sigma, rgb, nears, fars, noise, bg_ray, bg_scalar,
                           N, T, density_scale, thresh, image, depth, weights_sum, (float *)nullptr, (float4 *)field4, (float *)nullptr);
        FOC_CHECK_LAUNCH("fixed_field_pack");
        return FOC_OK;
    }
    hipLaunchKernelGGL(k_fs_render_infer<true>, dim3(foc_div_up(N, 4)), dim3(256), 0, (hipStream_t)stream, sigma, rgb, nears, fars, noise, bg_ray, bg_scalar, N, T,
                       density_scale, thresh, image, depth, weights_sum, (float *)nullptr, (float4 *)field4);
    FOC_CHECK_LAUNCH("fixed_field_pack");
    return FOC_OK;
}

int foc_view_tile_order(const float *rays_d, uint32_t N, uint32_t tile_h, uint32_t tile_w, int64_t *perm, void *state16, void *stream) {
    FocDeviceGuard foc_guard_(stream, rays_d);
    if (N == 0) return FOC_OK;
    FOC_REQUIRE(rays_d && perm && state16, FOC_E_INVALID, "view_tile_order: null pointer");
    FOC_REQUIRE(tile_h >= 1 && tile_w >= 1 && tile_h * tile_w <= 4096, FOC_E_INVALID, "view_tile_order: tile %u x %u", tile_h, tile_w);
    FOC_REQUIRE(N < (1u << 31), FOC_E_INVALID, "view_tile_order: N too large");
    hipStream_t st = (hipStream_t)stream;
    VtState *state = reinterpret_cast<VtState *>(state16);
    if (foc_zero_async(state, sizeof(VtState), st) != hipSuccess) { foc_set_error("view_tile_order: zero fill failed"); return FOC_E_LAUNCH; }
    if (N >= 3) {
        hipLaunchKernelGGL(k_vt_find, dim3(foc_grid_1d(N, 256)), dim3(256), 0, st, rays_d, N, state);
        hipLaunchKernelGGL(k_vt_check, dim3(foc_grid_1d(N, 256)), dim3(256), 0, st, rays_d, N, state);
    }
    hipLaunchKernelGGL(k_vt_perm, dim3(foc_grid_1d(N, 256)), dim3(256), 0, st, N, tile_h, tile_w, state, perm);
    FOC_CHECK_LAUNCH("view_tile_order");
    return FOC_OK;
}

}
```

focnerf_amd/csrc/fs_common.h:

```cpp
#pragma once
#include "common.h"
#include "sample_math.h"

struct FsGeom { float near, far, span, sample_dist, step; };

#define FS_RAY_BLOCK 64u
__host__ __device__ __forceinline__ uint64_t fs_block_row(uint32_t n, uint32_t i, uint32_t T) {
    return (uint64_t)(n / FS_RAY_BLOCK) * FS_RAY_BLOCK * T + (uint64_t)i * FS_RAY_BLOCK + n % FS_RAY_BLOCK;
}

__device__ __forceinline__ FsGeom fs_geom(const float *__restrict__ nears, const float *__restrict__ fars, uint32_t n, uint32_t T) {
    FsGeom g;
    g.near = nears[n]; g.far = fars[n];
    g.span = g.far - g.near;
    g.sample_dist = g.span / (float)T;
    g.step = 1.0f / (float)(T - 1);
    return g;
}
__device__ __forceinline__ float fs_z0(const FsGeom &g, uint32_t i, uint32_t T) {
    const float lin = (i < T / 2) ? (g.step * (float)i) : fmaf(-g.step, (float)(T - 1 - i), 1.0f);
    return g.near + g.span * lin;
}
__device__ __forceinline__ float fs_jitter(const FsGeom &g, float z, float u) { return z + (u - 0.5f) * g.sample_dist; }
__device__ __forceinline__ float fs_z(const FsGeom &g, uint32_t i, uint32_t T, const float *__restrict__ noise, uint64_t s) {
    float z = fs_z0(g, i, T);
    if (noise) z = fs_jitter(g, z, noise[s]);
    return z;
}
__device__ __forceinline__ float fs_zu(const FsGeom &g, uint32_t i, uint32_t T, bool jitter, float u) {
    float z = fs_z0(g, i, T);
    if (jitter) z = fs_jitter(g, z, u);
    return z;
}

struct FsSample { float z, delta, oz; };
__device__ __forceinline__ FsSample fs_sample(const FsGeom &g, uint32_t i, uint32_t ic, uint32_t T, bool jitter, float u0, float u1) {
    FsSample p;
    p.z = fs_zu(g, ic, T, jitter, u0);
    p.delta = g.sample_dist;
    if (i + 1 < T) p.delta = fs_zu(g, i + 1, T, jitter, u1) - p.z;
    p.oz = (p.z - g.near) / g.span;
    p.oz = p.oz < 0.0f ? 0.0f : (p.oz > 1.0f ? 1.0f : p.oz);
    return p;
}
__device__ __forceinline__ FsSample fs_sample_ld(const FsGeom &g, uint32_t i, uint32_t ic, uint32_t T, const float *__restrict__ noise, uint64_t s) {
    const bool jitter = noise != nullptr;
    return fs_sample(g, i, ic, T, jitter, jitter ? noise[s] : 0.0f, jitter && i + 1 < T ? noise[s + 1] : 0.0f);
}

__device__ __forceinline__ float fs_trans_scan(float om, uint32_t lane, float &Tc) {
    float P;
    const float Tb = Tc * wave_prod_scan(om, lane, P);
    Tc *= __shfl(P, 63, 64);
    return Tb;
}

__device__ __forceinline__ float wave_suffix_incl_sum(float v, int lane) {
#pragma unroll
    for (int o = 1; o < 64; o <<= 1) {
        const float u = __shfl_down(v, o, 64);
        if (lane + o < 64) v += u;
    }
    return v;
}
__device__ __forceinline__ float fs_head_bwd_step(const FsSample &p, bool valid, float sigma, float Tb, float gi, float gdp, float density_scale, uint32_t lane,
                                                  float &S_carry) {
    const float ex = expf((-p.delta * density_scale) * sigma);
    const float alpha = 1 - ex;
    const float om = 1 - alpha + 1e-15f;
    if (gdp != 0.0f) gi += gdp * p.oz;
    const float gw_i = valid ? gi * (alpha * Tb) : 0.0f;
    const float incl = wave_suffix_incl_sum(gw_i, (int)lane);
    const float S_i = S_carry + (incl - gw_i);
    const float dalpha = gi * Tb - S_i / om;
    S_carry += __shfl(incl, 0, 64);
    return dalpha * (p.delta * density_scale) * ex;
}

struct FsDist { float W, WM, acc; };
__device__ __forceinline__ float fs_dist_m(const FsGeom &g, const FsSample &p) { return (p.z - g.near) + 0.5f * p.delta; }
__device__ __forceinline__ void fs_dist_fwd_step(FsDist &d, float w, float m, float delta, uint32_t lane) {
    const float wm = w * m;
    const float iw = wave_incl_sum(w, (int)lane), iwm = wave_incl_sum(wm, (int)lane);
    float ew = __shfl_up(iw, 1, 64), ewm = __shfl_up(iwm, 1, 64);
    if (lane == 0) { ew = 0.0f; ewm = 0.0f; }
    const float Wb = d.W + ew, WMb = d.WM + ewm;
    d.acc += (1.0f / 3.0f) * delta * (w * w) + 2.0f * (w * (m * Wb - WMb));
    d.W += __shfl(iw, 63, 64); d.WM += __shfl(iwm, 63, 64);
}
__device__ __forceinline__ float fs_dist_bwd_step(FsDist &d, float w, float m, float delta, float W_total, float WM_total, uint32_t lane) {
    const float wm = w * m;
    const float iw = wave_suffix_incl_sum(w, (int)lane), iwm = wave_suffix_incl_sum(wm, (int)lane);
    float ew = __shfl_down(iw, 1, 64), ewm = __shfl_down(iwm, 1, 64);
    if (lane == 63) { ew = 0.0f; ewm = 0.0f; }
    const float Wa = d.W + ew, WMa = d.WM + ewm;
    const float Wb = (W_total - Wa) - w, WMb = (WM_total - WMa) - wm;
    d.W += __shfl(iw, 0, 64); d.WM += __shfl(iwm, 0, 64);
    return (2.0f / 3.0f) * delta * w + 2.0f * (m * (Wb - Wa) + (WMa - WMb));
}

struct FsRayGrad { float g0, g1, g2; FocBg bg; };
__device__ __forceinline__ FsRayGrad fs_ray_grad(const float *__restrict__ grad_image, const float *__restrict__ bg_ray, float bg_scalar, uint32_t n) {
    return FsRayGrad{grad_image[n * 3], grad_image[n * 3 + 1], grad_image[n * 3 + 2], foc_bg(bg_ray, bg_scalar, n)};
}
__device__ __forceinline__ float fs_composite_bwd_sample(const FsRayGrad &q, float w, float thresh, const _Float16 *cc, h8 &o0) {
    float gw = -(q.g0 * q.bg.b0 + q.g1 * q.bg.b1 + q.g2 * q.bg.b2);
#pragma unroll
    for (int k = 0; k < 8; k++) o0[k] = (_Float16)0;
    if (w > thresh) {
        const uint2 raw = *reinterpret_cast<const uint2 *>(cc);
        const _Float16 *y = reinterpret_cast<const _Float16 *>(&raw);
        const float y0 = foc_sigmoid_h((float)y[0]), y1 = foc_sigmoid_h((float)y[1]), y2 = foc_sigmoid_h((float)y[2]);
        gw += q.g0 * y0 + q.g1 * y1 + q.g2 * y2;
        o0[0] = foc_f2h(q.g0 * w * y0 * (1 - y0)); o0[1] = foc_f2h(q.g1 * w * y1 * (1 - y1)); o0[2] = foc_f2h(q.g2 * w * y2 * (1 - y2));
    }
    return gw;
}

struct FsBox { float a0, a1, a2, a3, a4, a5; };
__device__ __forceinline__ FsBox fs_box(const float *__restrict__ aabb) { return FsBox{aabb[0], aabb[1], aabb[2], aabb[3], aabb[4], aabb[5]}; }
__device__ __forceinline__ void fs_point(float ox, float oy, float oz, float dx, float dy, float dz, float z, const FsBox &b, float &x, float &y, float &w) {
    x = ox + dx * z; y = oy + dy * z; w = oz + dz * z;
    x = fminf(fmaxf(x, b.a0), b.a3); y = fminf(fmaxf(y, b.a1), b.a4); w = fminf(fmaxf(w, b.a2), b.a5);
}
__device__ __forceinline__ float fs_norm(float x, float bound, float two_b) { return (x + bound) / two_b; }

struct FsRayAcc { float Tc, ws, dp, r, g, b; };

template <bool PACK>
__device__ __forceinline__ void fs_infer_tile(FsRayAcc &a, const FsGeom &g, uint32_t n, uint32_t i, uint32_t lane, uint32_t T, float sigma, float c0, float c1,
                                              float c2, const float *__restrict__ noise, float density_scale, float thresh, float *__restrict__ rgb_masked,
                                              float4 *__restrict__ field4, float *__restrict__ sigma_rm) {
    const bool valid = i < T;
    const uint64_t s = (uint64_t)n * T + (valid ? i : T - 1);
    const FsSample p = fs_sample_ld(g, i, valid ? i : T - 1, T, noise, s);
    const float alpha = valid ? 1 - expf((-p.delta * density_scale) * sigma) : 0.0f;
    const float om = valid ? (1 - alpha + 1e-15f) : 1.0f;
    const float w = alpha * fs_trans_scan(om, lane, a.Tc);
    if (valid) {
        a.ws += w; a.dp += w * p.oz;
        const bool on = w > thresh;
        if (on) { a.r += w * c0; a.g += w * c1; a.b += w * c2; }
        if (rgb_masked) { rgb_masked[s * 3] = on ? c0 : 0.0f; rgb_masked[s * 3 + 1] = on ? c1 : 0.0f; rgb_masked[s * 3 + 2] = on ? c2 : 0.0f; }
        if (PACK) field4[s] = make_float4(sigma, on ? c0 : 0.0f, on ? c1 : 0.0f, on ? c2 : 0.0f);
        if (sigma_rm) sigma_rm[s] = sigma;
    }
}
```

focnerf_amd/csrc/raymarching.hip:

```cpp
#include "common.h"
#include "occ_cell.h"
#include "sample_math.h"
#include "ragged.h"
#include <float.h>

#define RM_SQRT3 1.7320508075688772f
#define RM_RPI   0.3183098861837907f

__device__ __forceinline__ float rm_sign(float x) { return copysignf(1.0f, x); }

__device__ __forceinline__ void rm_near_far(float ox, float oy, float oz, float dx, float dy, float dz, float a0, float a1, float a2, float a3, float a4, float a5,
                                            float min_near, float &near_out, float &far_out) {
    const float rdx = 1 / dx, rdy = 1 / dy, rdz = 1 / dz;
    float near = (a0 - ox) * rdx, far = (a3 - ox) * rdx, t;
    if (near > far) { t = near; near = far; far = t; }
    float near_y = (a1 - oy) * rdy, far_y = (a4 - oy) * rdy;
    if (near_y > far_y) { t = near_y; near_y = far_y; far_y = t; }
    bool miss = (near > far_y || near_y > far);
    if (!miss) {
        if (near_y > near) near = near_y;
        if (far_y < far) far = far_y;
        float near_z = (a2 - oz) * rdz, far_z = (a5 - oz) * rdz;
        if (near_z > far_z) { t = near_z; near_z = far_z; far_z = t; }
        miss = (near > far_z || near_z > far);
        if (!miss) {
            if (near_z > near) near = near_z;
            if (far_z < far) far = far_z;
            if (near < min_near) near = min_near;
        }
    }
    near_out = miss ? FLT_MAX : near;
    far_out = miss ? FLT_MAX : far;
}

__global__ void __launch_bounds__(256) k_near_far_from_aabb(const float *__restrict__ rays_o, const float *__restrict__ rays_d,
                                     const float *__restrict__ aabb, uint32_t N, float min_near,
                                     float *__restrict__ nears, float *__restrict__ fars) {
    const float a0 = aabb[0], a1 = aabb[1], a2 = aabb[2], a3 = aabb[3], a4 = aabb[4], a5 = aabb[5];
    for (uint32_t n = blockIdx.x * blockDim.x + threadIdx.x; n < N; n += gridDim.x * blockDim.x) {
        float near, far;
        rm_near_far(rays_o[n * 3], rays_o[n * 3 + 1], rays_o[n * 3 + 2], rays_d[n * 3], rays_d[n * 3 + 1], rays_d[n * 3 + 2], a0, a1, a2, a3, a4, a5, min_near, near, far);
        nears[n] = near;
        fars[n] = far;
    }
}

__global__ void __launch_bounds__(256) k_sph_from_ray(const float *__restrict__ rays_o, const float *__restrict__ rays_d, float radius,
                               uint32_t N, float *__restrict__ coords) {
    for (uint32_t n = blockIdx.x * blockDim.x + threadIdx.x; n < N; n += gridDim.x * blockDim.x) {
        const float ox = rays_o[n * 3], oy = rays_o[n * 3 + 1], oz = rays_o[n * 3 + 2];
        const float dx = rays_d[n * 3], dy = rays_d[n * 3 + 1], dz = rays_d[n * 3 + 2];
        const float A = fmaf(dz, dz, fmaf(dy, dy, dx * dx));
        const float B = fmaf(oz, dz, fmaf(oy, dy, ox * dx));
        const float C = fmaf(-radius, radius, fmaf(oz, oz, fmaf(oy, oy, ox * ox)));
        const float t = (-B + sqrtf(fmaf(B, B, -(A * C)))) / A;
        const float x = fmaf(t, dx, ox), y = fmaf(t, dy, oy), z = fmaf(t, dz, oz);
        const float theta = atan2f(sqrtf(fmaf(z, z, x * x)), y);
        const float phi = atan2f(z, x);
        coords[n * 2] = fmaf(2 * theta, RM_RPI, -1.0f);
        coords[n * 2 + 1] = phi * RM_RPI;
    }
}

__global__ void __launch_bounds__(256) k_morton3D(const int32_t *__restrict__ coords, uint32_t N, int32_t *__restrict__ indices) {
    for (uint32_t n = blockIdx.x * blockDim.x + threadIdx.x; n < N; n += gridDim.x * blockDim.x)
        indices[n] = (int32_t)rm_morton3D((uint32_t)coords[n * 3], (uint32_t)coords[n * 3 + 1], (uint32_t)coords[n * 3 + 2]);
}
__global__ void __launch_bounds__(256) k_morton3D_invert(const int32_t *__restrict__ indices, uint32_t N, int32_t *__restrict__ coords) {
    for (uint32_t n = blockIdx.x * blockDim.x + threadIdx.x; n < N; n += gridDim.x * blockDim.x) {
        const int32_t ind = indices[n];
        coords[n * 3] = (int32_t)rm_morton3D_invert((uint32_t)(ind >> 0));
        coords[n * 3 + 1] = (int32_t)rm_morton3D_invert((uint32_t)(ind >> 1));
        coords[n * 3 + 2] = (int32_t)rm_morton3D_invert((uint32_t)(ind >> 2));
    }
}

__global__ void __launch_bounds__(256) k_packbits_x4(const float4 *__restrict__ grid4, uint32_t N4, float thresh,
                              uint32_t *__restrict__ bitfield4) {
    for (uint32_t n = blockIdx.x * blockDim.x + threadIdx.x; n < N4; n += gridDim.x * blockDim.x) {
        uint32_t bits = 0;
#pragma unroll
        for (int q = 0; q < 8; q++) {
            const float4 v = grid4[(uint64_t)n * 8 + q];
            bits |= (v.x > thresh ? 1u : 0u) << (q * 4 + 0);
            bits |= (v.y > thresh ? 1u : 0u) << (q * 4 + 1);
            bits |= (v.z > thresh ? 1u : 0u) << (q * 4 + 2);
            bits |= (v.w > thresh ? 1u : 0u) << (q * 4 + 3);
        }
        bitfield4[n] = bits;
    }
}
__global__ void __launch_bounds__(256) k_packbits_tail(const float *__restrict__ grid, uint32_t n0, uint32_t N, float thresh,
                                uint8_t *__restrict__ bitfield) {
    for (uint32_t n = n0 + blockIdx.x * blockDim.x + threadIdx.x; n < N; n += gridDim.x * blockDim.x) {
        uint32_t bits = 0;
#pragma unroll
        for (int i = 0; i < 8; i++) bits |= (grid[(uint64_t)n * 8 + i] > thresh ? 1u : 0u) << i;
        bitfield[n] = (uint8_t)bits;
    }
}

struct RmCell { float x, y, z, dt, mip_bound; int nx, ny, nz; };

struct RmParams {
    float bound, dt_gamma, dt_min, dt_max, rH, H3, Hf, Cf, Hm1;
    uint32_t H;
    float norm_inv;
    int rederive;
    int gamma_pow2;
};
__device__ __forceinline__ float rm_out(const RmParams &p, float x) { return p.norm_inv != 0.0f ? (x + p.bound) * p.norm_inv : x; }

__device__ __forceinline__ bool rm_cell(const uint8_t *__restrict__ grid, const RmParams &p, float ox, float oy, float oz,
                                        float dx, float dy, float dz, float t, RmCell &c) {
    c.x = rm_clamp(fmaf(t, dx, ox), -p.bound, p.bound);
    c.y = rm_clamp(fmaf(t, dy, oy), -p.bound, p.bound);
    c.z = rm_clamp(fmaf(t, dz, oz), -p.bound, p.bound);
    c.dt = rm_clamp(t * p.dt_gamma, p.dt_min, p.dt_max);
    const int l1 = rm_mip_from_pos(c.x, c.y, c.z, p.Cf);
    const float mdt = (float)((double)(c.dt * p.Hf) * 0.5);
    const int l2 = (int)fminf(p.Cf - 1, fmaxf(0.0f, (float)rm_frexp_exp(mdt)));
    const int level = l1 > l2 ? l1 : l2;
    return rm_cell_bit(grid, rm_cell_index(c.x, c.y, c.z, level, p.bound, p.H, p.Hm1, p.H3, c.mip_bound, c.nx, c.ny, c.nz));
}

__device__ __forceinline__ float rm_skip_target(const RmParams &p, const RmCell &c, float t, float dx, float dy, float dz,
                                                float rdx, float rdy, float rdz) {
    const float tx = fmaf(fmaf(fmaf(0.5f, rm_sign(dx), (float)c.nx + 0.5f) * p.rH, 2.0f, -1.0f), c.mip_bound, -c.x) * rdx;
    const float ty = fmaf(fmaf(fmaf(0.5f, rm_sign(dy), (float)c.ny + 0.5f) * p.rH, 2.0f, -1.0f), c.mip_bound, -c.y) * rdy;
    const float tz = fmaf(fmaf(fmaf(0.5f, rm_sign(dz), (float)c.nz + 0.5f) * p.rH, 2.0f, -1.0f), c.mip_bound, -c.z) * rdz;
    return t + fmaxf(0.0f, fminf(tx, fminf(ty, tz)));
}

__device__ __forceinline__ float rm_skip(const RmParams &p, const RmCell &c, float t, float dx, float dy, float dz,
                                         float rdx, float rdy, float rdz) {
    const float tt = rm_skip_target(p, c, t, dx, dy, dz, rdx, rdy, rdz);
    do { t += rm_clamp(t * p.dt_gamma, p.dt_min, p.dt_max); } while (t < tt);
    return t;
}

static RmParams rm_make_params(float bound, float dt_gamma, uint32_t max_steps, uint32_t C, uint32_t H) {
    RmParams p;
    p.bound = bound; p.dt_gamma = dt_gamma;
    p.dt_min = 2 * RM_SQRT3 / (float)max_steps;
    p.dt_max = 2 * RM_SQRT3 * (float)(1 << (C - 1)) / (float)H;
    p.rH = 1 / (float)H;
    p.H3 = (float)(H * H * H);
    p.Hf = (float)H; p.Cf = (float)C; p.Hm1 = (float)(H - 1);
    p.H = H;
    p.norm_inv = 0.0f;
    p.rederive = 0;
    int e = 0;
    p.gamma_pow2 = (dt_gamma > 0.0f && frexpf(dt_gamma, &e) == 0.5f) ? 1 : 0;
    return p;
}

__global__ void __launch_bounds__(64) k_march_count(const float *__restrict__ rays_o, const float *__restrict__ rays_d,
                              const uint8_t *__restrict__ grid, RmParams p, uint32_t max_steps, uint32_t N,
                              float *__restrict__ nears, float *__restrict__ fars,
                              const float *__restrict__ noises, int32_t *__restrict__ counts, float *__restrict__ tstrip,
                              const float *__restrict__ aabb, float min_near) {
    const uint32_t n = blockIdx.x * blockDim.x + threadIdx.x;
    if (n >= N) return;
    const float ox = rays_o[n * 3], oy = rays_o[n * 3 + 1], oz = rays_o[n * 3 + 2];
    const float dx = rays_d[n * 3], dy = rays_d[n * 3 + 1], dz = rays_d[n * 3 + 2];
    const float rdx = 1 / dx, rdy = 1 / dy, rdz = 1 / dz;
    float near_n, far;
    if (aabb) {
        rm_near_far(ox, oy, oz, dx, dy, dz, aabb[0], aabb[1], aabb[2], aabb[3], aabb[4], aabb[5], min_near, near_n, far);
        nears[n] = near_n; fars[n] = far;
    } else { near_n = nears[n]; far = fars[n]; }
    float t = near_n;
    t = fmaf(rm_clamp(t * p.dt_gamma, p.dt_min, p.dt_max), noises[n], t);
    uint32_t num_steps = 0;
    RmCell c;
    float *strip = tstrip + (uint64_t)n * max_steps;
    while (t < far && num_steps < max_steps) {
        if (rm_cell(grid, p, ox, oy, oz, dx, dy, dz, t, c)) { strip[num_steps] = t; num_steps++; t += c.dt; }
        else t = rm_skip(p, c, t, dx, dy, dz, rdx, rdy, rdz);
    }
    counts[n] = (int32_t)num_steps;
}

#define RM_MAX_ROUNDS (1u << 22)
template <bool MED3>
__global__ void __launch_bounds__(256) k_march_count_wave(const float *__restrict__ rays_o, const float *__restrict__ rays_d,
// ... 1069 lines not shown
```

focnerf_amd/csrc/sample_math.h:

```cpp
#pragma once
#include "common.h"

typedef _Float16 h8 __attribute__((ext_vector_type(8)));

__device__ __forceinline__ void foc_sh16(float x, float y, float z, float (&o)[16]) {
    const float xy = x * y, xz = x * z, yz = y * z, x2 = x * x, y2 = y * y, z2 = z * z;
    o[0] = 0.28209479177387814f;
    o[1] = -0.48860251190291987f * y;
    o[2] = 0.48860251190291987f * z;
    o[3] = -0.48860251190291987f * x;
    o[4] = 1.0925484305920792f * xy;
    o[5] = -1.0925484305920792f * yz;
    o[6] = 0.94617469575755997f * z2 - 0.31539156525251999f;
    o[7] = -1.0925484305920792f * xz;
    o[8] = 0.54627421529603959f * x2 - 0.54627421529603959f * y2;
    o[9] = 0.59004358992664352f * y * (-3.0f * x2 + y2);
    o[10] = 2.8906114426405538f * xy * z;
    o[11] = 0.45704579946446572f * y * (1.0f - 5.0f * z2);
    o[12] = 0.3731763325901154f * z * (5.0f * z2 - 3.0f);
    o[13] = 0.45704579946446572f * x * (1.0f - 5.0f * z2);
    o[14] = 1.4453057213202769f * z * (x2 - y2);
    o[15] = 0.59004358992664352f * x * (-x2 + 3.0f * y2);
}
__device__ __forceinline__ void foc_sh16_h(float x, float y, float z, h8 &lo, h8 &hi) {
    float sh[16];
    foc_sh16(x, y, z, sh);
#pragma unroll
    for (int k = 0; k < 8; k++) { lo[k] = foc_f2h(sh[k]); hi[k] = foc_f2h(sh[8 + k]); }
}

__device__ __forceinline__ float foc_sigmoid_h(float x) { return (float)(_Float16)(1.0f / (1.0f + expf(-x))); }

__device__ __forceinline__ float foc_clamp15(float x) { return x < -15.0f ? -15.0f : (x > 15.0f ? 15.0f : x); }
__device__ __forceinline__ float foc_trunc_exp_bwd(float x) { return expf(foc_clamp15(x)); }
__device__ __forceinline__ float foc_trunc_exp_bwd(float x, float e) {
    const float xc = foc_clamp15(x);
    return xc != x ? expf(xc) : e;
}
struct FocExp15 { float lo, hi; };
__device__ __forceinline__ FocExp15 foc_exp15() {
    float a = -15.0f, b = 15.0f;
    asm volatile("" : "+v"(a));
    asm volatile("" : "+v"(b));
    return FocExp15{expf(a), expf(b)};
}
__device__ __forceinline__ float foc_trunc_exp_bwd_of_sigma(float sigma, const FocExp15 &e) { return fminf(fmaxf(sigma, e.lo), e.hi); }

struct FocBg { float b0, b1, b2; };
__device__ __forceinline__ FocBg foc_bg(const float *__restrict__ bg_ray, float bg_scalar, uint32_t k) {
    return FocBg{bg_ray ? bg_ray[k * 3] : bg_scalar, bg_ray ? bg_ray[k * 3 + 1] : bg_scalar, bg_ray ? bg_ray[k * 3 + 2] : bg_scalar};
}
```

focnerf_amd/fixedstep.py:

```python
import torch
from torch.autograd import Function

from . import raymarching
from ._lib import lib, ptr, stream_of, check
from .gridencoder import grid_encode


RAY_BLOCK = 64


def ray_block_default():
    import os
    return RAY_BLOCK if os.environ.get("FOC_RAY_BLOCK", str(RAY_BLOCK)) != "0" else 0


def blocked_rows(N, T, ray_block):
    return N * T if not ray_block else -(-N // ray_block) * ray_block * T


def fixed_sample(rays_o, rays_d, nears, fars, aabb, noise, T, bound, want_xyzs=False, want_ray_sh=False, ray_block=0):
    N = rays_o.shape[0]
    dev = rays_o.device
    rows = blocked_rows(N, T, ray_block)
    enc_in = torch.empty(rows, 3, dtype=torch.float32, device=dev)
    xyzs = torch.empty(rows, 3, dtype=torch.float32, device=dev) if want_xyzs else None
    ray_sh = torch.empty(N, 16, dtype=torch.float16, device=dev) if want_ray_sh else None
    check(lib.foc_fixed_sample(ptr(rays_o), ptr(rays_d), ptr(nears), ptr(fars), ptr(aabb), ptr(noise), N, T, float(bound), ptr(xyzs), ptr(enc_in),
                               ptr(ray_sh), int(ray_block), stream_of(rays_o)), "fixed_sample")
    if want_ray_sh:
        return enc_in, xyzs, ray_sh
    return enc_in, xyzs


def ray_sh_rows(rays_d):
    rays_d = rays_d.contiguous().float()
    N, dev = rays_d.shape[0], rays_d.device
    zeros, ones = torch.zeros(N, device=dev), torch.ones(N, device=dev)
    aabb = torch.tensor([-1., -1., -1., 1., 1., 1.], device=dev)
    return fixed_sample(torch.zeros_like(rays_d), rays_d, zeros, ones, aabb, None, 2, 1.0, want_ray_sh=True)[2]


class _density_head(Function):

    @staticmethod
    def forward(ctx, h, rays_d, nears, fars, noise, N, T, density_scale, obj_feat=None):
        from .field import object_feature_half
        h = h.contiguous()
        assert h.dtype == torch.float16 and h.shape == (N * T, 16)
        dev = h.device
        M = N * T
        sigma = torch.empty(M, dtype=torch.float32, device=dev)
        trans = torch.empty(M, dtype=torch.float32, device=dev)
        weights = torch.empty(M, dtype=torch.float32, device=dev)
        ws = torch.empty(N, dtype=torch.float32, device=dev)
        depth = torch.empty(N, dtype=torch.float32, device=dev)
        width = 32 if obj_feat is None else 48
        obj_feat = object_feature_half(obj_feat, "_density_head")
        cin = torch.empty(M, width, dtype=torch.float16, device=dev)
        check(lib.foc_fixed_head_forward(ptr(h), ptr(rays_d), ptr(nears), ptr(fars), ptr(noise), N, T, float(density_scale), ptr(sigma), ptr(trans),
                                         ptr(weights), ptr(ws), ptr(depth), ptr(cin), ptr(obj_feat), width, stream_of(h)), "fixed_head_forward")
        ctx.save_for_backward(h, sigma, trans, nears, fars, noise if noise is not None else torch.empty(0, device=dev))
        ctx.has_noise = noise is not None
        ctx.dims = (N, T, float(density_scale))
        ctx.width = width
        ctx.mark_non_differentiable(sigma)
        ctx.set_materialize_grads(False)
        return weights, ws, depth, sigma, cin

    @staticmethod
    def backward(ctx, g_weights, g_ws, g_depth, g_sigma, g_cin):
        h, sigma, trans, nears, fars, noise = ctx.saved_tensors
        N, T, ds = ctx.dims
        noise = noise if ctx.has_noise else None
        g_weights = g_weights.contiguous().float() if g_weights is not None else None
        g_ws = g_ws.contiguous().float() if g_ws is not None else None
        g_depth = g_depth.contiguous().float() if g_depth is not None else None
        g_cin = g_cin.contiguous().half() if g_cin is not None else None
        grad_h = torch.empty_like(h)
        check(lib.foc_fixed_head_backward(ptr(h), ptr(sigma), ptr(trans), ptr(nears), ptr(fars), ptr(noise), ptr(g_weights), ptr(g_ws), ptr(g_depth),
                                          ptr(g_cin), N, T, ds, ptr(grad_h), ctx.width, stream_of(h)), "fixed_head_backward")
        g_obj = None
        if ctx.width == 48 and ctx.needs_input_grad[8] and g_cin is not None:
            g_obj = g_cin[:, 31:47].float().sum(0)
        return grad_h, None, None, None, None, None, None, None, g_obj


class _fixed_composite(Function):

    @staticmethod
    def forward(ctx, c, weights, bg_ray, bg_scalar, N, T, thresh, weights_sum=None):
        c = c.contiguous()
        weights = weights.contiguous()
        assert c.dtype == torch.float16 and c.shape == (N * T, 16) and weights.dtype == torch.float32
        image = torch.empty(N, 3, dtype=torch.float32, device=c.device)
        check(lib.foc_fixed_composite_forward(ptr(c), ptr(weights), ptr(bg_ray), float(bg_scalar), N, T, float(thresh), ptr(image), stream_of(c)),
              "fixed_composite_forward")
        ctx.bg_grad = bg_ray is not None and ctx.needs_input_grad[2]
        if ctx.bg_grad and weights_sum is None:
            raise RuntimeError("_fixed_composite: a background that needs a gradient needs weights_sum")
        empty = torch.empty(0, device=c.device)
        ctx.save_for_backward(c, weights, bg_ray if bg_ray is not None else empty, weights_sum.detach() if ctx.bg_grad else empty)
        ctx.has_bg = bg_ray is not None
        ctx.dims = (N, T, float(thresh), float(bg_scalar))
        return image

    @staticmethod
    def backward(ctx, g_image):
        c, weights, bg_ray, weights_sum = ctx.saved_tensors
        N, T, thresh, bg_scalar = ctx.dims
        bg_ray = bg_ray if ctx.has_bg else None
        g_image = g_image.contiguous().float()
        grad_c = torch.empty_like(c)
        grad_w = torch.empty_like(weights)
        check(lib.foc_fixed_composite_backward(ptr(g_image), ptr(c), ptr(weights), ptr(bg_ray), bg_scalar, N, T, thresh, ptr(grad_c), ptr(grad_w),
                                               stream_of(c)), "fixed_composite_backward")
        g_bg = g_image * (1 - weights_sum).unsqueeze(-1) if ctx.bg_grad else None
        return grad_c, grad_w, g_bg, None, None, None, None, None


_C_WIDTH = 4


class _render_tail(Function):

    @staticmethod
    def forward(ctx, h, cweights, ray_sh, nears, fars, noise, bg_ray, bg_scalar, N, T, density_scale, thresh, num_layers, activation, obj_feat=None,
                want_sumsq=False, c_pre=None, w16_pre=None, input_pad=0.0, want_dist=False):
        from .field import _half_of, pad_twin, object_feature_half
        h = h.contiguous()
        assert h.dtype == torch.float16 and h.shape == (N * T, 16)
        assert ray_sh.dtype == torch.float16 and ray_sh.shape == (N, 16) and ray_sh.is_contiguous()
        dev, M = h.device, N * T
        st = stream_of(h)
        w16 = w16_pre if w16_pre is not None else _half_of(cweights)
        obj16 = object_feature_half(obj_feat, "_render_tail")
        assert obj16 is None or w16.numel() == 64 * (48 + 64 * (int(num_layers) - 1) + 16)
        if c_pre is not None:
            assert c_pre.dtype == torch.float16 and c_pre.shape == (M, _C_WIDTH) and c_pre.is_contiguous()
            c = c_pre
        else:
            c = torch.empty(M, _C_WIDTH, dtype=torch.float16, device=dev)
            args = (ptr(h), ptr(ray_sh), T, ptr(w16), M, 64, int(num_layers), int(activation), ptr(c), _C_WIDTH, ptr(obj16))
            fn, extra = pad_twin("foc_color_head_forward", input_pad, obj16 is not None)
            check(fn(*args, *extra, st), "color_head_forward")
        sigma = torch.empty(M, dtype=torch.float32, device=dev)
        trans = torch.empty(M, dtype=torch.float32, device=dev)
        weights = torch.empty(M, dtype=torch.float32, device=dev)
        ws = torch.empty(N, dtype=torch.float32, device=dev)
        depth = torch.empty(N, dtype=torch.float32, device=dev)
        image = torch.empty(N, 3, dtype=torch.float32, device=dev)
        sumsq = torch.empty(N, dtype=torch.float32, device=dev) if want_sumsq else None
        tail = (ptr(h), ptr(c), ptr(nears), ptr(fars), ptr(noise), ptr(bg_ray), float(bg_scalar), N, T, float(density_scale), float(thresh), ptr(sigma),
                ptr(trans), ptr(weights), ptr(ws), ptr(depth), ptr(image), _C_WIDTH, ptr(sumsq))
        dist = wm = None
        if want_dist:
            dist, wm = torch.empty(N, dtype=torch.float32, device=dev), torch.empty(N, dtype=torch.float32, device=dev)
            check(lib.foc_fixed_tail_forward_dist(*tail, ptr(dist), ptr(wm), st), "fixed_tail_forward_dist")
        else:
            check(lib.foc_fixed_tail_forward(*tail, st), "fixed_tail_forward")
        empty = torch.empty(0, device=dev)
        ctx.bg_grad = bg_ray is not None and ctx.needs_input_grad[6]
        ctx.save_for_backward(h, w16, sigma, trans, weights, c, ray_sh, nears, fars, noise if noise is not None else empty,
                              bg_ray if bg_ray is not None else empty, obj16 if obj16 is not None else empty,
                              ws if ctx.bg_grad or want_dist else empty, wm if want_dist else empty)
        ctx.outputs = (bool(want_sumsq), bool(want_dist))
        ctx.flags = (noise is not None, bg_ray is not None, obj16 is not None, obj_feat.dtype if obj_feat is not None else None,
                     tuple(obj_feat.shape) if obj_feat is not None else None)
        ctx.dims = (N, T, float(density_scale), float(thresh), float(bg_scalar), int(num_layers), int(activation), float(input_pad))
        ctx.mark_non_differentiable(sigma, weights, c)
        ctx.set_materialize_grads(False)
        return (image, ws, depth, sigma, weights, c) + ((sumsq,) if want_sumsq else ()) + ((dist,) if want_dist else ())

    @staticmethod
    def backward(ctx, g_image, g_ws, g_depth, _g_sigma, _g_weights, _g_c, *g_extra):
        from .backend import _scratch
        from .field import pad_twin
        h, w16, sigma, trans, weights, c, ray_sh, nears, fars, noise, bg_ray, obj16, ws, wm = ctx.saved_tensors
        g_extra = list(g_extra)
        g_sumsq = g_extra.pop(0) if ctx.outputs[0] else None
        g_dist = g_extra.pop(0) if ctx.outputs[1] else None
        has_noise, has_bg, has_obj, obj_dtype, obj_shape = ctx.flags
        obj16 = obj16 if has_obj else None
        N, T, ds, thresh, bg_scalar, num_layers, activation, input_pad = ctx.dims
        noise = noise if has_noise else None
        bg_ray = bg_ray if has_bg else None
        dev, M = h.device, N * T
        st = stream_of(h)
        g_image = g_image.contiguous().float() if g_image is not None else torch.zeros(N, 3, dtype=torch.float32, device=dev)
        g_ws = g_ws.contiguous().float() if g_ws is not None else None
        g_depth = g_depth.contiguous().float() if g_depth is not None else None
        g_sumsq = g_sumsq.contiguous().float() if g_sumsq is not None else None
        grad_c = torch.empty_like(c)
        grad_h0 = torch.empty(M, dtype=torch.float16, device=dev)
        if g_dist is not None:
            g_dist = g_dist.contiguous().float()
            check(lib.foc_fixed_tail_backward_dist(ptr(g_image), ptr(g_ws), ptr(g_depth), ptr(c), ptr(sigma), ptr(trans), ptr(weights), ptr(ws), ptr(nears),
                                                   ptr(fars), ptr(noise), ptr(bg_ray), bg_scalar, N, T, ds, thresh, ptr(grad_c), ptr(grad_h0), _C_WIDTH,
                                                   ptr(g_sumsq), ptr(wm), None, ptr(g_dist), st), "fixed_tail_backward_dist")
        else:
            check(lib.foc_fixed_tail_backward(ptr(g_image), ptr(g_ws), ptr(g_depth), ptr(c), ptr(sigma), ptr(trans), ptr(weights), ptr(nears), ptr(fars),
                                              ptr(noise), ptr(bg_ray), bg_scalar, N, T, ds, thresh, ptr(grad_c), ptr(grad_h0), _C_WIDTH, ptr(g_sumsq), st),
                  "fixed_tail_backward")
        grad_h = torch.empty_like(h)
        g_w = torch.empty_like(w16)
        wsb = _scratch.get("ffmlp_ws", lib.foc_ffmlp_backward_workspace_bytes(48 if has_obj else 32, 64, num_layers), dev)
        g_obj32 = torch.empty(16, dtype=torch.float32, device=dev) if has_obj and ctx.needs_input_grad[14] else None
        args = (ptr(grad_c), ptr(h), ptr(ray_sh), T, ptr(grad_h0), ptr(w16), M, 64, num_layers, activation, ptr(grad_h), ptr(g_w), ptr(wsb),
                wsb.numel(), _C_WIDTH, ptr(obj16), ptr(g_obj32))
        fn, extra = pad_twin("foc_color_head_backward", input_pad, has_obj)
        check(fn(*args, *extra, st), "color_head_backward")
        g_obj = g_obj32.to(obj_dtype).view(obj_shape) if g_obj32 is not None else None
        g_bg = g_image * (1 - ws).unsqueeze(-1) if ctx.bg_grad else None
        return (grad_h, g_w, None, None, None, None, g_bg) + (None,) * 7 + (g_obj, None, None, None, None, None)


class _masked_norm(Function):

    @staticmethod
    def forward(ctx, sumsq, outside):
        crit = torch.sqrt((sumsq * outside).sum())
        ctx.save_for_backward(crit, outside)
        return crit

    @staticmethod
    def backward(ctx, g):
        crit, outside = ctx.saved_tensors
        coef = torch.where(crit > 0, g / (2 * crit), torch.zeros_like(crit))
        return outside * coef, None


def _unfused_distortion(weights, nears, fars, noise, N, T):
    from .loss import ray_distortion
    span = (fars - nears).unsqueeze(-1)
    z = span * torch.linspace(0.0, 1.0, T, device=weights.device).unsqueeze(0)
    if noise is not None:
        z = z + (noise.view(N, T) - 0.5) * (span / T)
    delta = torch.cat([z[:, 1:] - z[:, :-1], span / T], dim=-1)
    live = (fars > nears).unsqueeze(-1)
    zero = torch.zeros_like(z)
    return ray_distortion(torch.where(live, weights.view(N, T), zero), torch.where(live, z + 0.5 * delta, zero), torch.where(live, delta, zero))


def _background(bg_color, N, dev):
    if bg_color is None:
        return None, 1.0
    if torch.is_tensor(bg_color):
        if bg_color.numel() > 1:
            return bg_color.to(dev, torch.float32).expand(N, 3).contiguous(), 0.0
        return None, float(bg_color)
    return None, float(bg_color)


def render_fixed_steps(model, rays_o, rays_d, yolo_details=None, num_steps=512, bg_color=None, perturb=False, weight_thresh=1e-10,
                       return_fields=None, _out=None, distortion=False, **kwargs):
    import time
    if return_fields is None:
        return_fields = not model.training
    t_start = time.time()
    prefix = rays_o.shape[:-1]
    rays_o = rays_o.contiguous().view(-1, 3).float()
    rays_d = rays_d.contiguous().view(-1, 3).float()
    N, T = rays_o.shape[0], int(num_steps)
    dev = rays_o.device
    aabb = model.aabb_train if model.training else model.aabb_infer
    nears, fars = raymarching.near_far_from_aabb(rays_o, rays_d, aabb, model.min_near)
    noise = torch.rand(N * T, dtype=torch.float32, device=dev) if perturb else None
    from .field import field_plan, field_infer
    plan = field_plan(model)
    if getattr(model, "bg_radius", 0) > 0:
        bg_color = model._background_colour(rays_o, rays_d, bg_color)
    want_tail = plan.tail and model.training and torch.is_grad_enabled()
    fused_infer = not torch.is_grad_enabled() and plan.infer
    if distortion and not torch.is_grad_enabled():
        raise ValueError("render_fixed_steps: distortion=True needs the training route (gradients enabled): the inference paths form no "
                         "differentiable weights; call it under torch.enable_grad() with model.train()")
    rb = ray_block_default() if fused_infer else 0
    enc_in, _, ray_sh = fixed_sample(rays_o, rays_d, nears, fars, aabb, noise, T, model.bound, want_ray_sh=True) if want_tail else \
        fixed_sample(rays_o, rays_d, nears, fars, aabb, noise, T, model.bound, ray_block=rb) + (None,)

    if fused_infer:
        obj_feat = model.encode_object_feature(yolo_details, dev) if plan.uses_object_feature else None
        sigma, rgb = field_infer(model, enc_in, rays_d, dir_div=T, dir_block=rb, obj_feat=obj_feat)
        bg_ray, bg_scalar = _background(bg_color, N, dev)
        direct = (_out is not None and _out[0].dtype == torch.float32 and _out[1].dtype == torch.float32 and _out[0].is_contiguous()
                  and _out[1].is_contiguous() and _out[0].numel() == N and _out[1].numel() == 3 * N and _out[0].device == dev)
        depth, image = (_out[0].view(N), _out[1].view(N, 3)) if direct else (torch.empty(N, dtype=torch.float32, device=dev),
                                                                              torch.empty(N, 3, dtype=torch.float32, device=dev))
        weights_sum = torch.empty(N, dtype=torch.float32, device=dev)
        rgb_masked = densities = None
        if return_fields:
            if direct and len(_out) == 4 and all(t.dtype == torch.float32 and t.is_contiguous() and t.device == dev for t in _out[2:]) \
                    and _out[2].numel() == N * T and _out[3].numel() == 3 * N * T and rb:
                densities, rgb_masked = _out[2].view(N * T), _out[3].view(N * T, 3)
            else:
                rgb_masked = torch.empty(N * T, 3, dtype=torch.float32, device=dev)
                densities = torch.empty(N * T, dtype=torch.float32, device=dev) if rb else None
        check(lib.foc_fixed_render_inference(ptr(sigma), ptr(rgb), ptr(nears), ptr(fars), ptr(noise), ptr(bg_ray), float(bg_scalar), N, T,
                                             float(model.density_scale), float(weight_thresh), ptr(image), ptr(depth), ptr(weights_sum), ptr(rgb_masked),
                                             rb, ptr(densities), stream_of(sigma)), "fixed_render_inference")
        t_mid = time.time()
        results = {'depth': depth.view(*prefix), 'image': image.view(*prefix, 3), 'weights_sum': weights_sum, 'criterion_outside_mask': None,
                   'timing': [t_mid - t_start, time.time() - t_mid]}
        if return_fields:
            results['densities'] = (densities if rb else sigma).view(N, T, 1)
            results['rgbs'] = rgb_masked.view(N, T, 3)
        return results

    enc = model.encoder
    from .field import hashgrid_mlp, fused_mlp
    c_pre = obj_feat = None
    cweights = fused_mlp(model, "color_net").weights if want_tail else None
    with torch.autocast("cuda", dtype=torch.float16):
        if plan.uses_object_feature:
            obj_feat = model.encode_object_feature(yolo_details, dev)
        if plan.field:
            colour = wc16 = None
            if want_tail and plan.train_forward:
                from .field import _half_of
                wc16 = _half_of(cweights)
                colour = (wc16, plan.colour, ray_sh, T, _C_WIDTH, obj_feat, plan.colour_input_pad)
            h = hashgrid_mlp(enc, fused_mlp(model, "sigma_net"), enc_in, None, colour)
            if colour is not None:
                h, c_pre = h
        else:
            feats = grid_encode(enc_in, enc.embeddings, enc.offsets, enc.per_level_scale, enc.base_resolution, False, enc.gridtype_id,
                                enc.align_corners, enc.interp_id)
            h = fused_mlp(model, "sigma_net")(feats)
        if h.shape[1] != 16:
            raise RuntimeError("render_fixed_steps expects a 16-wide sigma head (1 + geo_feat_dim = 16)")
        fused_tail = want_tail
        want_crit = model.training and yolo_details is not None and yolo_details[0] is not None
        criterion_outside_mask = None
        if fused_tail:
            cn = fused_mlp(model, "color_net")
            bg_ray, bg_scalar = _background(bg_color, N, dev)
            outs = _render_tail.apply(h, cweights, ray_sh, nears, fars, noise, bg_ray, bg_scalar, N, T, model.density_scale, weight_thresh,
                                      cn.num_layers, cn.activation, obj_feat, want_crit and yolo_details[0].numel() == N, c_pre,
                                      wc16 if c_pre is not None else None, plan.colour_input_pad, *((True,) if distortion else ()))
            image, weights_sum, depth, sigma, weights, c = outs[:6]
            ray_dist = outs[-1] if distortion else None
            if len(outs) - bool(distortion) == 7:
                criterion_outside_mask = _masked_norm.apply(outs[6], (~yolo_details[0].reshape(N)).to(torch.float32))
        else:
            weights, weights_sum, depth, sigma, cin = _density_head.apply(h, rays_d, nears, fars, noise, N, T, model.density_scale, obj_feat)
            if plan.colour_input_pad != 0:
                cin = torch.cat([cin[:, :-1], cin.new_full((cin.shape[0], 1), plan.colour_input_pad)], dim=1)
            if distortion:
                ray_dist = _unfused_distortion(weights, nears, fars, noise, N, T)
        if want_crit and criterion_outside_mask is None:
            from .activation import trunc_exp
            criterion_outside_mask = torch.norm(trunc_exp(h[:, 0]).view(N, T)[~yolo_details[0].squeeze(0)] - 0)
        if not fused_tail:
            c = fused_mlp(model, "color_net").forward_padded(cin)
    t_mid = time.time()

    if not fused_tail:
        bg_ray, bg_scalar = _background(bg_color, N, dev)
        image = _fixed_composite.apply(c, weights, bg_ray, bg_scalar, N, T, weight_thresh, weights_sum)

    results = {'depth': depth.view(*prefix), 'image': image.view(*prefix, 3), 'weights_sum': weights_sum,
               'criterion_outside_mask': criterion_outside_mask, 'timing': [t_mid - t_start, time.time() - t_mid]}
    if distortion:
        results['distortion'] = ray_dist.view(*prefix)
    if return_fields:
        from .head import rgb_head
        c16 = c.detach()
        if c16.shape[1] != 16:
            c16 = torch.nn.functional.pad(c16, (0, 16 - c16.shape[1]))
        rgb = rgb_head(c16) * (weights > weight_thresh).unsqueeze(-1)
        results['densities'] = sigma.view(N, T, 1)
        results['rgbs'] = rgb.view(N, T, 3)
    return results


@torch.no_grad()
def render_field4(model, rays_o, rays_d, num_steps=512, weight_thresh=1e-10, yolo_details=None, out=None, occupancy=None, placement=None,
                  scene_aabb=None):
    from .field import field_plan, field_infer
    if placement is None and scene_aabb is not None:
        raise ValueError("render_field4: scene_aabb belongs to a placement; without one the object is rendered in its own box")
    if placement is not None and occupancy is None:
        raise ValueError("render_field4: placement needs occupancy= (the placed path is the occupancy-culled one): pass "
                         "fixedcull.Occupancy.of(model) for a cuda_ray network or fixedcull.Occupancy.estimate(model) for any other")
    rays_o = rays_o.contiguous().view(-1, 3).float()
    rays_d = rays_d.contiguous().view(-1, 3).float()
    N, T = rays_o.shape[0], int(num_steps)
    dev = rays_o.device
    if out is None:
        out = torch.empty(N, T, 4, dtype=torch.float32, device=dev)
    assert out.shape == (N, T, 4) and out.dtype == torch.float32 and out.is_contiguous()
    plan = field_plan(model)
    if placement is not None:
        from .fixedcull import render_field4_placed
        return render_field4_placed(model, plan, rays_o, rays_d, T, weight_thresh, yolo_details, out, occupancy, placement, scene_aabb)
    if occupancy is not None:
        from .fixedcull import render_field4_culled
        return render_field4_culled(model, plan, rays_o, rays_d, T, weight_thresh, yolo_details, out, occupancy)
    if plan.infer and model.bg_radius <= 0:
        aabb = model.aabb_train if model.training else model.aabb_infer
        nears, fars = raymarching.near_far_from_aabb(rays_o, rays_d, aabb, model.min_near)
        rb = ray_block_default()
        enc_in, _ = fixed_sample(rays_o, rays_d, nears, fars, aabb, None, T, model.bound, ray_block=rb)
        obj_feat = model.encode_object_feature(yolo_details, dev) if plan.uses_object_feature else None
        sigma, rgb = field_infer(model, enc_in, rays_d, dir_div=T, dir_block=rb, obj_feat=obj_feat)
        check(lib.foc_fixed_field_pack(ptr(sigma), ptr(rgb), ptr(nears), ptr(fars), None, None, 1.0, N, T, float(model.density_scale),
                                       float(weight_thresh), None, None, None, ptr(out), rb, stream_of(sigma)), "fixed_field_pack")
        return out
    from .combine import pack_field4
    with torch.autocast("cuda", dtype=torch.float16):
        res = model.run(rays_o[None], rays_d[None], yolo_details, num_steps=T, upsample_steps=0, perturb=False, weight_thresh=weight_thresh,
                        return_fields=True)
    out.copy_(pack_field4(res['densities'], res['rgbs']))
    return out
```

include/focnerf.h:

```cpp
#ifndef FOCNERF_H
#define FOCNERF_H

#include <stdint.h>

#ifdef __cplusplus
extern "C" {
#endif

#define FOC_OK            0
#define FOC_E_INVALID     1
#define FOC_E_DTYPE       2
#define FOC_E_LAUNCH      3

#define FOC_F32 0
#define FOC_F16 1

#define FOC_ABI_VERSION 2
int         foc_abi_version(void);
const char *foc_last_error(void);
int foc_set_option(const char *name, int value);
int foc_get_option(const char *name, int *value);
int foc_guard_pick_device(int stream_is_null, int stream_device, int pointer_device, int current_device);
const char *foc_arch(void);

// ... 108 lines not shown
                             uint32_t B, uint32_t D, uint32_t C, uint32_t L, float S, uint32_t H,
                             const void *dy_dx, void *grad_inputs, uint32_t gridtype,
                             int align_corners, uint32_t interp, int dtype, int grad_is_bl,
                             const int32_t *offsets_host, void *stream);

uint64_t foc_grid_encode_backward_workspace_bytes(uint32_t B, uint32_t D, uint32_t C, uint32_t L, int dtype);
int foc_grid_encode_backward_binned(const void *grad, const float *inputs, const void *embeddings,
                                    const int32_t *offsets, void *grad_embeddings,
                                    uint32_t B, uint32_t D, uint32_t C, uint32_t L, float S, uint32_t H,
                                    const void *dy_dx, void *grad_inputs, uint32_t gridtype,
                                    int align_corners, uint32_t interp, int dtype, int grad_is_bl,
                                    const int32_t *offsets_host, void *workspace, uint64_t workspace_bytes,
                                    void *stream);

int foc_grid_encode_forward_counted(const float *inputs, const void *embeddings, const int32_t *offsets, void *outputs,
                                    uint32_t B, uint32_t D, uint32_t C, uint32_t L, float S, uint32_t H,
                                    uint32_t gridtype, int align_corners, uint32_t interp, int dtype,
                                    const int32_t *offsets_host, void *workspace, uint64_t workspace_bytes, void *stream);
int foc_grid_encode_backward_count(const float *inputs, const int32_t *offsets, uint32_t B, uint32_t D, uint32_t C,
                                   uint32_t L, float S, uint32_t H, uint32_t gridtype, int align_corners,
                                   uint32_t interp, int dtype, const int32_t *offsets_host, void *workspace,
                                   uint64_t workspace_bytes, void *stream);
int foc_grid_encode_backward_binned_counted(const void *grad, const float *inputs, const void *embeddings,
                                            const int32_t *offsets, void *grad_embeddings,
                                            uint32_t B, uint32_t D, uint32_t C, uint32_t L, float S, uint32_t H,
                                            const void *dy_dx, void *grad_inputs, uint32_t gridtype,
                                            int align_corners, uint32_t interp, int dtype, int grad_is_bl,
                                            const int32_t *offsets_host, void *workspace, uint64_t workspace_bytes,
                                            void *stream);

int foc_grad_total_variation(const void *inputs, const void *embeddings, void *grad,
                             const int32_t *offsets, float weight,
                             uint32_t B, uint32_t D, uint32_t C, uint32_t L, float S, uint32_t H,
                             uint32_t gridtype, int align_corners, int dtype, void *stream);


int foc_freq_encode_forward(const float *inputs, uint32_t B, uint32_t D, uint32_t deg, uint32_t C,
                            float *outputs, void *stream);
int foc_freq_encode_backward(const float *grad, const float *outputs, uint32_t B, uint32_t D,
                             uint32_t deg, uint32_t C, float *grad_inputs, void *stream);


int foc_ffmlp_forward(const void *inputs, const void *weights, uint32_t B, uint32_t input_dim,
                      uint32_t output_dim, uint32_t hidden_dim, uint32_t num_layers,
                      uint32_t activation, uint32_t output_activation,
                      void *forward_buffer, void *outputs, void *stream);

int foc_ffmlp_inference(const void *inputs, const void *weights, uint32_t B, uint32_t input_dim,
                        uint32_t output_dim, uint32_t hidden_dim, uint32_t num_layers,
                        uint32_t activation, uint32_t output_activation,
                        void *inference_buffer, void *outputs, void *stream);

int foc_ffmlp_backward(const void *grad, const void *inputs, const void *weights,
                       const void *forward_buffer, uint32_t B, uint32_t input_dim,
                       uint32_t output_dim, uint32_t hidden_dim, uint32_t num_layers,
                       uint32_t activation, uint32_t output_activation, int calc_grad_inputs,
                       void *backward_buffer, void *grad_inputs, void *grad_weights,
                       void *workspace, uint64_t workspace_bytes, void *stream);
uint64_t foc_ffmlp_backward_workspace_bytes(uint32_t input_dim, uint32_t hidden_dim, uint32_t num_layers);

int foc_ffmlp_forward_planar(const void *inputs_planar, const void *weights, uint32_t B, uint32_t input_dim,
                             uint32_t output_dim, uint32_t hidden_dim, uint32_t num_layers,
                             uint32_t activation, uint32_t output_activation, void *outputs, void *stream);
int foc_ffmlp_backward_planar(const void *grad, const void *inputs_planar, const void *weights, uint32_t B,
                              uint32_t input_dim, uint32_t output_dim, uint32_t hidden_dim, uint32_t num_layers,
                              uint32_t activation, uint32_t output_activation, int calc_grad_inputs,
                              void *grad_inputs_planar, void *grad_weights, void *workspace, uint64_t workspace_bytes, void *stream);

int foc_nerf_field_inference(const void *enc, int enc_planar, const float *dirs, uint32_t dir_div,
                             uint32_t dir_block, uint32_t n_dirs, const void *sigma_weights, uint32_t sigma_layers, const void *color_weights,
                             uint32_t color_layers, uint32_t hidden_dim, uint32_t activation, uint32_t B,
                             float *sigma, float *rgb, const void *obj_feat, void *stream);
int foc_nerf_field_inference_pad(const void *enc, int enc_planar, const float *dirs, uint32_t dir_div,
                                 uint32_t dir_block, uint32_t n_dirs, const void *sigma_weights, uint32_t sigma_layers, const void *color_weights,
                                 uint32_t color_layers, uint32_t hidden_dim, uint32_t activation, uint32_t B,
                                 float *sigma, float *rgb, const void *obj_feat, float input_pad, void *stream);
int foc_nerf_field_inference_pad31(const void *enc, int enc_planar, const float *dirs, uint32_t dir_div,
                                   uint32_t dir_block, uint32_t n_dirs, const void *sigma_weights, uint32_t sigma_layers, const void *color_weights,
                                   uint32_t color_layers, uint32_t hidden_dim, uint32_t activation, uint32_t B,
                                   float *sigma, float *rgb, const void *obj_feat, float input_pad, void *stream);

int foc_color_head_forward(const void *h, const void *ray_sh, uint32_t samples_per_ray, const void *weights,
                           uint32_t B, uint32_t hidden_dim, uint32_t num_layers, uint32_t activation,
                           void *outputs, uint32_t out_width, const void *obj_feat, void *stream);
int foc_color_head_backward(const void *grad, const void *h, const void *ray_sh, uint32_t samples_per_ray,
                            const void *grad_h0, const void *weights, uint32_t B, uint32_t hidden_dim,
                            uint32_t num_layers, uint32_t activation, void *grad_h, void *grad_weights,
                            void *workspace, uint64_t workspace_bytes, uint32_t out_width, const void *obj_feat, float *grad_obj, void *stream);
int foc_color_head_forward_pad(const void *h, const void *ray_sh, uint32_t samples_per_ray, const void *weights,
                               uint32_t B, uint32_t hidden_dim, uint32_t num_layers, uint32_t activation,
                               void *outputs, uint32_t out_width, const void *obj_feat, float input_pad, void *stream);
int foc_color_head_backward_pad(const void *grad, const void *h, const void *ray_sh, uint32_t samples_per_ray,
                                const void *grad_h0, const void *weights, uint32_t B, uint32_t hidden_dim,
                                uint32_t num_layers, uint32_t activation, void *grad_h, void *grad_weights,
                                void *workspace, uint64_t workspace_bytes, uint32_t out_width, const void *obj_feat, float *grad_obj,
                                float input_pad, void *stream);
int foc_color_head_forward_pad31(const void *h, const void *ray_sh, uint32_t samples_per_ray, const void *weights,
                                 uint32_t B, uint32_t hidden_dim, uint32_t num_layers, uint32_t activation,
                                 void *outputs, uint32_t out_width, const void *obj_feat, float input_pad, void *stream);
int foc_color_head_backward_pad31(const void *grad, const void *h, const void *ray_sh, uint32_t samples_per_ray,
                                  const void *grad_h0, const void *weights, uint32_t B, uint32_t hidden_dim,
                                  uint32_t num_layers, uint32_t activation, void *grad_h, void *grad_weights,
                                  void *workspace, uint64_t workspace_bytes, uint32_t out_width, const void *obj_feat, float *grad_obj,
                                  float input_pad, void *stream);

int foc_field_forward_train(const void *planes, const void *sigma_weights, uint32_t sigma_layers, const void *ray_sh, uint32_t samples_per_ray,
                            const void *color_weights, uint32_t color_layers, uint32_t hidden_dim, uint32_t activation, uint32_t B,
                            void *h, void *c, uint32_t out_width, const void *obj_feat, void *stream);
int foc_field_forward_train_pad(const void *planes, const void *sigma_weights, uint32_t sigma_layers, const void *ray_sh, uint32_t samples_per_ray,
                                const void *color_weights, uint32_t color_layers, uint32_t hidden_dim, uint32_t activation, uint32_t B,
                                void *h, void *c, uint32_t out_width, const void *obj_feat, float input_pad, void *stream);
int foc_field_forward_train_pad31(const void *planes, const void *sigma_weights, uint32_t sigma_layers, const void *ray_sh, uint32_t samples_per_ray,
                                  const void *color_weights, uint32_t color_layers, uint32_t hidden_dim, uint32_t activation, uint32_t B,
                                  void *h, void *c, uint32_t out_width, const void *obj_feat, float input_pad, void *stream);

int foc_allocate_splitk(uint64_t size);
int foc_free_splitk(void);


int foc_combine_select(const float *dens, const float *rgb, float *max_dens, float *best_rgb,
                       uint64_t n, void *stream);

int foc_combine_pack_keys(const float *dens, uint32_t rank, uint64_t *keys, uint64_t n, void *stream);
int foc_combine_unpack(const uint64_t *keys, uint32_t rank, const float *rgb,
                       float *max_dens, float *masked_rgb, uint64_t n, void *stream);

int foc_composite_fixed_steps(const float *sigmas, const float *rgbs, const float *nears,
                              const float *fars, uint32_t N, uint32_t T, float bg,
                              float *image4, float *depth, void *stream);

#define FOC_COMBINE_MAX_OBJECTS 16

int foc_combine_select_composite(const float *const *fields4, uint32_t K, const float *nears, const float *fars,
                                 uint32_t N, uint32_t T, const float *bgs, uint32_t n_bg, float *image4, float *depth,
                                 float *merged4, void *stream);

int foc_combine_select4(const float *field4, float *acc4, uint64_t n, void *stream);

int foc_combine_select_composite_attr(const float *const *fields4, uint32_t K, const uint8_t *const *id_planes,
                                      const uint32_t *ids, uint32_t n_obj, const float *nears, const float *fars,
                                      uint32_t N, uint32_t T, const float *bgs, uint32_t n_bg, float *image4, float *depth,
                                      float *merged4, float *obj_weights, float *obj_depth, int32_t *instance,
                                      uint8_t *winner, void *stream);

int foc_combine_select4_ids(const float *field4, uint32_t id, float *acc4, uint8_t *acc_ids, uint64_t n, void *stream);

int foc_mo_select(const void *sigma_new, const void *feat_new, void *sigma_best, void *feat_best, uint64_t n,
                  uint32_t feat_width, uint32_t elem_bytes, void *stream);


int foc_fixed_sample(const float *rays_o, const float *rays_d, const float *nears, const float *fars,
                     const float *aabb, const float *noise, uint32_t N, uint32_t T, float bound,
                     float *xyzs, float *enc_in, void *ray_sh, uint32_t ray_block, void *stream);

int foc_fixed_head_forward(const void *h, const float *rays_d, const float *nears, const float *fars,
                           const float *noise, uint32_t N, uint32_t T, float density_scale,
                           float *sigma, float *trans, float *weights, float *weights_sum, float *depth,
                           void *cin, const void *obj_feat, uint32_t cin_width, void *stream);
int foc_fixed_head_backward(const void *h, const float *sigma, const float *trans, const float *nears,
                            const float *fars, const float *noise, const float *grad_w, const float *grad_ws,
                            const float *grad_depth, const void *grad_cin, uint32_t N, uint32_t T,
                            float density_scale, void *grad_h, uint32_t cin_width, void *stream);

int foc_fixed_tail_forward(const void *h, const void *c, const float *nears, const float *fars, const float *noise,
                           const float *bg_ray, float bg_scalar, uint32_t N, uint32_t T, float density_scale, float thresh,
                           float *sigma, float *trans, float *weights, float *weights_sum, float *depth, float *image,
                           uint32_t c_width, float *ray_sumsq, void *stream);
int foc_fixed_tail_backward(const float *grad_image, const float *grad_ws, const float *grad_depth, const void *c,
                            const float *sigma, const float *trans, const float *weights, const float *nears,
                            const float *fars, const float *noise, const float *bg_ray, float bg_scalar, uint32_t N,
                            uint32_t T, float density_scale, float thresh, void *grad_c, void *grad_h0, uint32_t c_width,
                            const float *grad_sumsq, void *stream);

int foc_occ_tail_forward(const void *h, const void *c, uint32_t c_width, const float *deltas, const int32_t *rays,
                         uint32_t M, uint32_t N, float T_thresh, float density_scale, const float *bg_ray, float bg_scalar,
                         const float *nears, const float *fars, float *weights_sum, float *image_raw, float *image,
                         float *depth, void *stream);
int foc_occ_tail_backward(const float *grad_image, const float *grad_ws, const void *h, const void *c, uint32_t c_width,
                          const float *deltas, const int32_t *rays, const int32_t *counter, const float *weights_sum,
                          const float *image_raw, uint32_t M, uint32_t N, float T_thresh, float density_scale,
                          const float *bg_ray, float bg_scalar, void *grad_c, void *grad_h0, void *stream);
int foc_occ_tail_forward_sumsq(const void *h, const void *c, uint32_t c_width, const float *deltas, const int32_t *rays,
                               uint32_t M, uint32_t N, float T_thresh, float density_scale, const float *bg_ray, float bg_scalar,
                               const float *nears, const float *fars, float *weights_sum, float *image_raw, float *image,
                               float *depth, float *ray_sumsq, void *stream);
int foc_occ_tail_backward_sumsq(const float *grad_image, const float *grad_ws, const void *h, const void *c, uint32_t c_width,
                                const float *deltas, const int32_t *rays, const int32_t *counter, const float *weights_sum,
                                const float *image_raw, uint32_t M, uint32_t N, float T_thresh, float density_scale,
                                const float *bg_ray, float bg_scalar, void *grad_c, void *grad_h0, const float *grad_sumsq, void *stream);

int foc_fixed_tail_forward_dist(const void *h, const void *c, const float *nears, const float *fars, const float *noise,
                                const float *bg_ray, float bg_scalar, uint32_t N, uint32_t T, float density_scale, float thresh,
                                float *sigma, float *trans, float *weights, float *weights_sum, float *depth, float *image,
                                uint32_t c_width, float *ray_sumsq, float *ray_dist, float *ray_wm, void *stream);
int foc_fixed_tail_backward_dist(const float *grad_image, const float *grad_ws, const float *grad_depth, const void *c,
                                 const float *sigma, const float *trans, const float *weights, const float *weights_sum, const float *nears,
                                 const float *fars, const float *noise, const float *bg_ray, float bg_scalar, uint32_t N,
                                 uint32_t T, float density_scale, float thresh, void *grad_c, void *grad_h0, uint32_t c_width,
                                 const float *grad_sumsq, const float *ray_wm, const float *ray_dist, const float *grad_dist, void *stream);
int foc_occ_tail_forward_dist(const void *h, const void *c, uint32_t c_width, const float *deltas, const int32_t *rays,
                              uint32_t M, uint32_t N, float T_thresh, float density_scale, const float *bg_ray, float bg_scalar,
                              const float *nears, const float *fars, float *weights_sum, float *image_raw, float *image,
                              float *depth, float *ray_sumsq, float *ray_dist, float *ray_wm, void *stream);
int foc_occ_tail_backward_dist(const float *grad_image, const float *grad_ws, const void *h, const void *c, uint32_t c_width,
                               const float *deltas, const int32_t *rays, const int32_t *counter, const float *weights_sum,
                               const float *image_raw, uint32_t M, uint32_t N, float T_thresh, float density_scale,
                               const float *bg_ray, float bg_scalar, void *grad_c, void *grad_h0, const float *grad_sumsq,
                               const float *ray_wm, const float *ray_dist, const float *grad_dist, void *stream);
int foc_occ_tail_forward_depth(const void *h, const void *c, uint32_t c_width, const float *deltas, const int32_t *rays,
                               uint32_t M, uint32_t N, float T_thresh, float density_scale, const float *bg_ray, float bg_scalar,
                               const float *nears, const float *fars, float *weights_sum, float *image_raw, float *image,
                               float *depth, float *ray_sumsq, float *ray_dist, float *ray_wm, float *depth_raw, void *stream);
int foc_occ_tail_backward_depth(const float *grad_image, const float *grad_ws, const void *h, const void *c, uint32_t c_width,
                                const float *deltas, const int32_t *rays, const int32_t *counter, const float *weights_sum,
                                const float *image_raw, uint32_t M, uint32_t N, float T_thresh, float density_scale,
                                const float *bg_ray, float bg_scalar, void *grad_c, void *grad_h0, const float *grad_sumsq,
                                const float *ray_wm, const float *ray_dist, const float *grad_dist, const float *nears,
                                const float *fars, const float *depth_raw, const float *grad_depth, void *stream);

typedef struct FocOccTrainNode {
    uint32_t struct_bytes;
    uint32_t n_rays, max_steps, cascade, grid_size, cap, pad_align;
    float bound, dt_gamma, min_near;
    const float *rays_o, *rays_d, *aabb, *jitter;
    const uint8_t *bitfield;
    float *nears, *fars, *enc_in, *deltas;
    void *sh_rows;
    int32_t *rays, *counter, *march_scratch;
    uint32_t levels, base_resolution, gridtype, interp;
    int32_t align_corners, table_dtype;
    float per_level_scale_log2;
    const void *embeddings;
    const int32_t *offsets, *offsets_host;
    void *planes, *grid_workspace;
    uint64_t grid_workspace_bytes;
    uint32_t sigma_input_dim, sigma_hidden, sigma_layers, sigma_activation, sigma_output_activation;
    uint32_t color_hidden, color_layers, color_activation, c_width;
    const void *w_sigma, *w_color;
    void *h, *c;
    float T_thresh, density_scale, bg_scalar;
    const float *bg_ray;
    float *weights_sum, *image_raw, *image, *depth;
    int32_t precounted;
    const float *grad_image, *grad_ws;
    void *grad_c, *grad_h0, *grad_h, *grad_planes, *grad_w_color, *grad_w_sigma, *grad_embeddings, *mlp_workspace;
    uint64_t mlp_workspace_bytes;
} FocOccTrainNode;
int foc_occ_train_forward(const FocOccTrainNode *node, void *stream);
int foc_occ_train_backward(const FocOccTrainNode *node, void *stream);
int foc_occ_train_forward_pad31(const FocOccTrainNode *node, float input_pad, void *stream);
int foc_occ_train_backward_pad31(const FocOccTrainNode *node, float input_pad, void *stream);
typedef struct FocOccTrainObject {
    uint32_t struct_bytes;
    float input_pad;
    const void *obj_feat;
    float *ray_sumsq;
    const float *grad_sumsq;
    float *grad_obj;
} FocOccTrainObject;
int foc_occ_train_forward_obj(const FocOccTrainNode *node, const FocOccTrainObject *object, void *stream);
int foc_occ_train_backward_obj(const FocOccTrainNode *node, const FocOccTrainObject *object, void *stream);
typedef struct FocOccTrainTail {
    uint32_t struct_bytes;
    float *ray_dist, *ray_wm, *depth_raw;
    const float *grad_dist, *grad_depth;
} FocOccTrainTail;
int foc_occ_train_forward_tail(const FocOccTrainNode *node, const FocOccTrainObject *object, float input_pad,
                               const FocOccTrainTail *tail, void *stream);
int foc_occ_train_backward_tail(const FocOccTrainNode *node, const FocOccTrainObject *object, float input_pad,
                                const FocOccTrainTail *tail, void *stream);

int foc_view_tile_order(const float *rays_d, uint32_t N, uint32_t tile_h, uint32_t tile_w, int64_t *perm, void *state16,
                        void *stream);

int foc_fixed_composite_forward(const void *c, const float *weights, const float *bg_ray, float bg_scalar,
                                uint32_t N, uint32_t T, float thresh, float *image, void *stream);
int foc_fixed_composite_backward(const float *grad_image, const void *c, const float *weights,
                                 const float *bg_ray, float bg_scalar, uint32_t N, uint32_t T, float thresh,
                                 void *grad_c, float *grad_w, void *stream);

int foc_fixed_render_inference(const float *sigma, const float *rgb, const float *nears, const float *fars,
                               const float *noise, const float *bg_ray, float bg_scalar, uint32_t N, uint32_t T,
                               float density_scale, float thresh, float *image, float *depth, float *weights_sum,
                               float *rgb_masked, uint32_t ray_block, float *sigma_raymajor, void *stream);

int foc_fixed_field_pack(const float *sigma, const float *rgb, const float *nears, const float *fars,
                         const float *noise, const float *bg_ray, float bg_scalar, uint32_t N, uint32_t T,
                         float density_scale, float thresh, float *image, float *depth, float *weights_sum,
                         float *field4, uint32_t ray_block, void *stream);

uint64_t foc_fixed_cull_scratch_bytes(uint32_t N, uint32_t T);
int foc_fixed_cull(const float *rays_o, const float *rays_d, const float *nears, const float *fars, const float *aabb,
                   uint32_t N, uint32_t T, float bound, const uint8_t *bitfield, uint32_t cascade, uint32_t grid_size,
                   uint64_t *mask, uint32_t *offsets, uint32_t *count, void *scratch, uint64_t scratch_bytes, void *stream);
int foc_fixed_cull_emit(const float *rays_o, const float *rays_d, const float *nears, const float *fars, const float *aabb,
                        uint32_t N, uint32_t T, float bound, const uint64_t *mask, const uint32_t *offsets, uint32_t m_occ,
                        float *enc_in_c, float *dirs_c, void *stream);

int foc_fixed_field_pack_culled(const float *sigma_c, const float *rgb_c, const uint64_t *mask, const uint32_t *offsets,
                                uint32_t m_occ, const float *nears, const float *fars, uint32_t N, uint32_t T,
                                float density_scale, float thresh, float *field4, void *stream);

int foc_fixed_cull_placed(const float *rays_o, const float *rays_d, const float *nears, const float *fars, const float *scene_aabb,
                          uint32_t N, uint32_t T, const float *world_to_object, const float *obj_aabb, float bound,
                          const uint8_t *bitfield, uint32_t cascade, uint32_t grid_size, uint64_t *mask, uint32_t *offsets,
                          uint32_t *count, void *scratch, uint64_t scratch_bytes, void *stream);
// ... 44 lines not shown
```

Before: 1.380 billion.

## Prefetch tail chunks in composite kernels and fuse AABB near/far into sampling

The tail forward and backward compositing kernels now double-buffer their per-chunk loads: the next 64-sample chunk's h, c and noise (or sigma/trans/weights) is fetched before the current chunk is processed, so memory latency can overlap compute. Separately, the training fixed-step sampler computes each ray's AABB near/far inline and writes nears/fars itself, which drops the separate near_far_from_aabb kernel launch. Both are behind options that default to on. The cost is higher register pressure from holding two chunks of inputs at once, and the near/far test is now evaluated redundantly for every sample of a ray.

```diff
diff --git a/focnerf_amd/_lib.py b/focnerf_amd/_lib.py
--- a/focnerf_amd/_lib.py
+++ b/focnerf_amd/_lib.py
@@ -173,6 +173,7 @@
     "foc_fixed_field_pack_culled_gain": (i32, [c_vp, c_vp, c_vp, c_vp, u32, c_vp, c_vp, u32, u32, f32, f32, f32, c_vp, c_vp]),
     "foc_composite_fixed_steps":(i32, [c_vp, c_vp, c_vp, c_vp, u32, u32, f32, c_vp, c_vp, c_vp]),
     "foc_fixed_sample": (i32, [c_vp, c_vp, c_vp, c_vp, c_vp, c_vp, u32, u32, f32, c_vp, c_vp, c_vp, u32, c_vp]),
+    "foc_fixed_sample_aabb": (i32, [c_vp, c_vp, c_vp, f32, c_vp, u32, u32, f32, c_vp, c_vp, c_vp, u32, c_vp, c_vp, c_vp]),
     "foc_fixed_tail_forward": (i32, [c_vp, c_vp, c_vp, c_vp, c_vp, c_vp, f32, u32, u32, f32, f32, c_vp, c_vp, c_vp, c_vp, c_vp, c_vp, u32, c_vp, c_vp]),
     "foc_fixed_tail_backward": (i32, [c_vp, c_vp, c_vp, c_vp, c_vp, c_vp, c_vp, c_vp, c_vp, c_vp, c_vp, f32, u32, u32, f32, f32, c_vp, c_vp, u32, c_vp, c_vp]),
     "foc_fixed_tail_forward_dist": (i32, [c_vp, c_vp, c_vp, c_vp, c_vp, c_vp, f32, u32, u32, f32, f32, c_vp, c_vp, c_vp, c_vp, c_vp, c_vp, u32, c_vp, c_vp,
diff --git a/focnerf_amd/csrc/combine.hip b/focnerf_amd/csrc/combine.hip
--- a/focnerf_amd/csrc/combine.hip
+++ b/focnerf_amd/csrc/combine.hip
@@ -240,6 +240,7 @@
     {"FOC_MLP_BWD_FUSED", 1}, {"FOC_FIELD_FWD_FUSED", 1}, {"FOC_GB_MERGE_MAX_RES", 480}, {"FOC_GB_FACTORED", 1}, {"FOC_GB_TAIL_SPLIT", 16}, {"FOC_GRID_FUSE_SMALL", 1},
     {"FOC_GRID_PAIRS", 1}, {"FOC_GRID_FAST", 1}, {"FOC_MARCH_SERIAL", -1}, {"FOC_MARCH_RAYS_ROW_MAX", 131072}, {"FOC_OCC_MARCH_FORM", -1},
     {"FOC_OCC_SAMPLE_MAJOR", 1}, {"FOC_OCC_FIELD_PIECE", 1 << 23}, {"FOC_DETERMINISTIC", 0},
+    {"FOC_TAIL_PIPELINE", 1}, {"FOC_SAMPLE_AABB", 1},
 };
 static int foc_option_parse(int which, const char *text) {
     if (which == FOC_OPT_OCC_MARCH_FORM) {
diff --git a/focnerf_amd/csrc/common.h b/focnerf_amd/csrc/common.h
--- a/focnerf_amd/csrc/common.h
+++ b/focnerf_amd/csrc/common.h
@@ -25,6 +25,8 @@
     FOC_OPT_OCC_SAMPLE_MAJOR,
     FOC_OPT_OCC_FIELD_PIECE,
     FOC_OPT_DETERMINISTIC,
+    FOC_OPT_TAIL_PIPELINE,
+    FOC_OPT_SAMPLE_AABB,
     FOC_OPT_COUNT
 };
 int foc_opt(FocOpt which);
diff --git a/focnerf_amd/csrc/fixedstep.hip b/focnerf_amd/csrc/fixedstep.hip
--- a/focnerf_amd/csrc/fixedstep.hip
+++ b/focnerf_amd/csrc/fixedstep.hip
@@ -2,10 +2,12 @@
 #include "fs_common.h"
 #include <float.h>
 
+template <bool AABB>
 __global__ void __launch_bounds__(256) k_fs_sample(const float *__restrict__ rays_o, const float *__restrict__ rays_d, const float *__restrict__ nears,
                                                    const float *__restrict__ fars, const float *__restrict__ aabb, const float *__restrict__ noise,
                                                    uint32_t N, uint32_t T, float bound, float *__restrict__ xyzs, float *__restrict__ enc_in,
-                                                   _Float16 *__restrict__ ray_sh, uint32_t ray_block) {
+                                                   _Float16 *__restrict__ ray_sh, uint32_t ray_block, float min_near, float *__restrict__ nears_out,
+                                                   float *__restrict__ fars_out) {
     const uint64_t total = ray_block ? (uint64_t)((N + FS_RAY_BLOCK - 1) / FS_RAY_BLOCK) * FS_RAY_BLOCK * T : (uint64_t)N * T;
     const FsBox box = fs_box(aabb);
     const float two_b = 2 * bound;
@@ -21,15 +23,22 @@
         } else {
             n = (uint32_t)(s / T); i = (uint32_t)(s - (uint64_t)n * T);
         }
-        const FsGeom g = fs_geom(nears, fars, n, T);
+        const float ox = rays_o[n * 3], oy = rays_o[n * 3 + 1], oz = rays_o[n * 3 + 2], dx = rays_d[n * 3], dy = rays_d[n * 3 + 1], dz = rays_d[n * 3 + 2];
+        FsGeom g;
+        if constexpr (AABB) {
+            float near, far;
+            rm_near_far(ox, oy, oz, dx, dy, dz, box.a0, box.a1, box.a2, box.a3, box.a4, box.a5, min_near, near, far);
+            g = fs_geom_of(near, far, T);
+            if (i == 0 && own) { nears_out[n] = near; fars_out[n] = far; }
+        } else g = fs_geom(nears, fars, n, T);
         const float z = fs_z(g, i, T, noise, (uint64_t)n * T + i);
         float x, y, w;
-        fs_point(rays_o[n * 3], rays_o[n * 3 + 1], rays_o[n * 3 + 2], rays_d[n * 3], rays_d[n * 3 + 1], rays_d[n * 3 + 2], z, box, x, y, w);
+        fs_point(ox, oy, oz, dx, dy, dz, z, box, x, y, w);
         if (xyzs) { xyzs[s * 3] = x; xyzs[s * 3 + 1] = y; xyzs[s * 3 + 2] = w; }
         if (enc_in) { enc_in[s * 3] = fs_norm(x, bound, two_b); enc_in[s * 3 + 1] = fs_norm(y, bound, two_b); enc_in[s * 3 + 2] = fs_norm(w, bound, two_b); }
         if (ray_sh && i == 0 && own) {
             h8 lo, hi;
-            foc_sh16_h(rays_d[n * 3], rays_d[n * 3 + 1], rays_d[n * 3 + 2], lo, hi);
+            foc_sh16_h(dx, dy, dz, lo, hi);
             h8 *dst = reinterpret_cast<h8 *>(ray_sh + (uint64_t)n * 16);
             dst[0] = lo; dst[1] = hi;
         }
@@ -166,7 +175,21 @@
     }
 }
 
-template <bool NOISE, bool DIST>
+template <bool NOISE> struct FsTailFwdIn { _Float16 h0; uint2 raw; float u0, u1; };
+template <bool NOISE>
+__device__ __forceinline__ FsTailFwdIn<NOISE> fs_tail_fwd_load(const _Float16 *__restrict__ h, const _Float16 *__restrict__ c, const float *__restrict__ noise,
+                                                               uint32_t n, uint32_t T, uint32_t i, uint32_t c_ld) {
+    const uint32_t ic = i < T ? i : T - 1;
+    const uint64_t s = (uint64_t)n * T + ic;
+    FsTailFwdIn<NOISE> in;
+    in.h0 = h[s * 16];
+    in.raw = *reinterpret_cast<const uint2 *>(c + s * c_ld);
+    in.u0 = 0.0f; in.u1 = 0.0f;
+    if (NOISE) { in.u0 = noise[s]; in.u1 = noise[(uint64_t)n * T + min(ic + 1u, T - 1u)]; }
+    return in;
+}
+
+template <bool NOISE, bool DIST, bool PIPE>
 __global__ void __launch_bounds__(256) k_fs_tail_fwd(const _Float16 *__restrict__ h, const _Float16 *__restrict__ c, const float *__restrict__ nears,
                                                      const float *__restrict__ fars, const float *__restrict__ noise, const float *__restrict__ bg_ray,
                                                      float bg_scalar, uint32_t N, uint32_t T, float density_scale, float thresh,
@@ -176,19 +199,20 @@
     const uint32_t lane = threadIdx.x & 63;
     const uint32_t n = blockIdx.x * 4 + (threadIdx.x >> 6);
     if (n >= N) return;
+    FsTailFwdIn<NOISE> in_a, in_b;
+    if (PIPE) in_a = fs_tail_fwd_load<NOISE>(h, c, noise, n, T, lane, c_ld);
     const FsGeom g = fs_geom(nears, fars, n, T);
     float Tc = 1.0f, ws = 0, dp = 0, r = 0, gg = 0, b = 0, sq = 0;
     FsDist dist = {0, 0, 0};
     const bool live = g.far > g.near;
-    for (uint32_t base = 0; base < T; base += 64) {
+    auto step = [&](uint32_t base, const FsTailFwdIn<NOISE> &cur) {
         const uint32_t i = base + lane;
         const bool valid = i < T;
         const uint32_t ic = valid ? i : T - 1;
         const uint64_t s = (uint64_t)n * T + ic;
-        const _Float16 h0 = h[s * 16];
-        const uint2 raw = *reinterpret_cast<const uint2 *>(c + s * c_ld);
-        float u0 = 0.0f, u1 = 0.0f;
-        if (NOISE) { u0 = noise[s]; u1 = noise[(uint64_t)n * T + min(ic + 1u, T - 1u)]; }
+        const _Float16 h0 = cur.h0;
+        const uint2 raw = cur.raw;
+        const float u0 = cur.u0, u1 = cur.u1;
         const float sigma = expf((float)h0);
         const FsSample p = fs_sample(g, i, ic, T, NOISE, u0, u1);
         const float alpha = valid ? 1 - expf((-p.delta * density_scale) * sigma) : 0.0f;
@@ -206,6 +230,18 @@
                 r += w * foc_sigmoid_h((float)cc[0]); gg += w * foc_sigmoid_h((float)cc[1]); b += w * foc_sigmoid_h((float)cc[2]);
             }
         }
+    };
+    if (PIPE) {
+        for (uint32_t base = 0;; base += 128) {
+            in_b = fs_tail_fwd_load<NOISE>(h, c, noise, n, T, base + 64 + lane, c_ld);
+            step(base, in_a);
+            if (base + 64 >= T) break;
+            in_a = fs_tail_fwd_load<NOISE>(h, c, noise, n, T, base + 128 + lane, c_ld);
+            step(base + 64, in_b);
+            if (base + 128 >= T) break;
+        }
+    } else {
+        for (uint32_t base = 0; base < T; base += 64) step(base, fs_tail_fwd_load<NOISE>(h, c, noise, n, T, base + lane, c_ld));
     }
     ws = wave_sum(ws); dp = wave_sum(dp); r = wave_sum(r); gg = wave_sum(gg); b = wave_sum(b);
     if (ray_sumsq) {
@@ -223,7 +259,22 @@
     }
 }
 
-template <bool NOISE, bool DIST>
+template <bool NOISE> struct FsTailBwdIn { float sigma, Tb, w; uint2 raw; float u0, u1; };
+template <bool NOISE>
+__device__ __forceinline__ FsTailBwdIn<NOISE> fs_tail_bwd_load(const _Float16 *__restrict__ c, const float *__restrict__ sigma_in, const float *__restrict__ trans_in,
+                                                               const float *__restrict__ weights, const float *__restrict__ noise, uint32_t n, uint32_t T,
+                                                               uint32_t i, uint32_t c_ld) {
+    const uint32_t ic = i < T ? i : T - 1;
+    const uint64_t s = (uint64_t)n * T + ic;
+    FsTailBwdIn<NOISE> in;
+    in.sigma = sigma_in[s]; in.Tb = trans_in[s]; in.w = weights[s];
+    in.raw = *reinterpret_cast<const uint2 *>(c + s * c_ld);
+    in.u0 = 0.0f; in.u1 = 0.0f;
+    if (NOISE) { in.u0 = noise[s]; in.u1 = noise[(uint64_t)n * T + min(ic + 1u, T - 1u)]; }
+    return in;
+}
+
+template <bool NOISE, bool DIST, bool PIPE>
 __global__ void __launch_bounds__(256) k_fs_tail_bwd(const float *__restrict__ grad_image, const float *__restrict__ grad_ws, const float *__restrict__ grad_depth,
                                                      const _Float16 *__restrict__ c, const float *__restrict__ sigma_in, const float *__restrict__ trans_in,
                                                      const float *__restrict__ weights, const float *__restrict__ nears, const float *__restrict__ fars,
@@ -234,6 +285,9 @@
     const uint32_t lane = threadIdx.x & 63;
     const uint32_t n = blockIdx.x * 4 + (threadIdx.x >> 6);
     if (n >= N) return;
+    const uint32_t n_chunks = (T + 63) / 64;
+    FsTailBwdIn<NOISE> in_a, in_b;
+    if (PIPE) in_a = fs_tail_bwd_load<NOISE>(c, sigma_in, trans_in, weights, noise, n, T, (n_chunks - 1) * 64 + lane, c_ld);
     const FsGeom g = fs_geom(nears, fars, n, T);
     const float gws = grad_ws ? grad_ws[n] : 0.0f, gdp = grad_depth ? grad_depth[n] : 0.0f;
     const float gsq2 = grad_sumsq ? 2.0f * grad_sumsq[n] : 0.0f;
@@ -246,16 +300,14 @@
     const FsRayGrad q = fs_ray_grad(grad_image, bg_ray, bg_scalar, n);
     const FocExp15 e15 = foc_exp15();
     float S_carry = 0.0f;
-    const uint32_t n_chunks = (T + 63) / 64;
-    for (uint32_t cidx = n_chunks; cidx-- > 0;) {
+    auto step = [&](uint32_t cidx, const FsTailBwdIn<NOISE> &cur) {
         const uint32_t i = cidx * 64 + lane;
         const bool valid = i < T;
         const uint32_t ic = valid ? i : T - 1;
         const uint64_t s = (uint64_t)n * T + ic;
-        const float sigma = sigma_in[s], Tb = trans_in[s], w = weights[s];
-        const uint2 raw = *reinterpret_cast<const uint2 *>(c + s * c_ld);
-        float u0 = 0.0f, u1 = 0.0f;
-        if (NOISE) { u0 = noise[s]; u1 = noise[(uint64_t)n * T + min(ic + 1u, T - 1u)]; }
+        const float sigma = cur.sigma, Tb = cur.Tb, w = cur.w;
+        const uint2 raw = cur.raw;
+        const float u0 = cur.u0, u1 = cur.u1;
         h8 o0;
         const h8 o1 = {0, 0, 0, 0, 0, 0, 0, 0};
         const float gw = fs_composite_bwd_sample(q, w, thresh, reinterpret_cast<const _Float16 *>(&raw), o0);
@@ -272,6 +324,19 @@
         if (gsq2 != 0.0f) dsigma = fmaf(gsq2, sigma, dsigma);
         const float dh0 = dsigma * foc_trunc_exp_bwd_of_sigma(sigma, e15);
         if (valid) grad_h0[s] = foc_f2h(dh0);
+    };
+    auto load = [&](uint32_t cidx) { return fs_tail_bwd_load<NOISE>(c, sigma_in, trans_in, weights, noise, n, T, cidx * 64 + lane, c_ld); };
+    if (PIPE) {
+        for (uint32_t cidx = n_chunks - 1;; cidx -= 2) {
+            in_b = load(cidx ? cidx - 1 : 0u);
+            step(cidx, in_a);
+            if (cidx == 0) break;
+            in_a = load(cidx > 1 ? cidx - 2 : 0u);
+            step(cidx - 1, in_b);
+            if (cidx == 1) break;
+        }
+    } else {
+        for (uint32_t cidx = n_chunks; cidx-- > 0;) step(cidx, load(cidx));
     }
 }
 
@@ -399,9 +464,23 @@
     FOC_REQUIRE(T >= 2, FOC_E_INVALID, "fixed_sample: T must be >= 2");
     FOC_REQUIRE(ray_block == 0 || ray_block == FS_RAY_BLOCK, FOC_E_INVALID, "fixed_sample: ray_block must be 0 (ray-major) or %u (got %u)", FS_RAY_BLOCK, ray_block);
     const uint64_t rows = ray_block ? (uint64_t)foc_div_up(N, FS_RAY_BLOCK) * FS_RAY_BLOCK * T : (uint64_t)N * T;
-    hipLaunchKernelGGL(k_fs_sample, dim3(foc_grid_1d(rows, 256, 256 * 16)), dim3(256), 0, (hipStream_t)stream, rays_o, rays_d, nears, fars, aabb,
-                       noise, N, T, bound, xyzs, enc_in, (_Float16 *)ray_sh, ray_block);
+    hipLaunchKernelGGL(k_fs_sample<false>, dim3(foc_grid_1d(rows, 256, 256 * 16)), dim3(256), 0, (hipStream_t)stream, rays_o, rays_d, nears, fars, aabb,
+                       noise, N, T, bound, xyzs, enc_in, (_Float16 *)ray_sh, ray_block, 0.0f, (float *)nullptr, (float *)nullptr);
     FOC_CHECK_LAUNCH("fixed_sample");
+    return FOC_OK;
+}
+
+int foc_fixed_sample_aabb(const float *rays_o, const float *rays_d, const float *aabb, float min_near, const float *noise, uint32_t N, uint32_t T,
+                          float bound, float *xyzs, float *enc_in, void *ray_sh, uint32_t ray_block, float *nears_out, float *fars_out, void *stream) {
+    FocDeviceGuard foc_guard_(stream, rays_o);
+    if (N == 0) return FOC_OK;
+    FOC_REQUIRE(rays_o && rays_d && aabb && nears_out && fars_out && (xyzs || enc_in), FOC_E_INVALID, "fixed_sample_aabb: null pointer");
+    FOC_REQUIRE(T >= 2, FOC_E_INVALID, "fixed_sample_aabb: T must be >= 2");
+    FOC_REQUIRE(ray_block == 0 || ray_block == FS_RAY_BLOCK, FOC_E_INVALID, "fixed_sample_aabb: ray_block must be 0 (ray-major) or %u (got %u)", FS_RAY_BLOCK, ray_block);
+    const uint64_t rows = ray_block ? (uint64_t)foc_div_up(N, FS_RAY_BLOCK) * FS_RAY_BLOCK * T : (uint64_t)N * T;
+    hipLaunchKernelGGL(k_fs_sample<true>, dim3(foc_grid_1d(rows, 256, 256 * 16)), dim3(256), 0, (hipStream_t)stream, rays_o, rays_d, (const float *)nullptr,
+                       (const float *)nullptr, aabb, noise, N, T, bound, xyzs, enc_in, (_Float16 *)ray_sh, ray_block, min_near, nears_out, fars_out);
+    FOC_CHECK_LAUNCH("fixed_sample_aabb");
     return FOC_OK;
 }
 
@@ -464,7 +543,11 @@
     FOC_REQUIRE(c_width == 16 || c_width == 4, FOC_E_INVALID, "%s: c_width must be 16 or 4 (got %u)", who, c_width);
     FOC_REQUIRE(h && c && nears && fars && sigma && trans && weights && weights_sum && depth && image, FOC_E_INVALID, "%s: null pointer", who);
     FOC_REQUIRE(T >= 2, FOC_E_INVALID, "%s: T must be >= 2", who);
-    auto kern = ray_dist ? (noise ? k_fs_tail_fwd<true, true> : k_fs_tail_fwd<false, true>) : (noise ? k_fs_tail_fwd<true, false> : k_fs_tail_fwd<false, false>);
+    auto kern = ray_dist ? (noise ? k_fs_tail_fwd<true, true, false> : k_fs_tail_fwd<false, true, false>)
+                         : (noise ? k_fs_tail_fwd<true, false, false> : k_fs_tail_fwd<false, false, false>);
+    if (foc_opt(FOC_OPT_TAIL_PIPELINE))
+        kern = ray_dist ? (noise ? k_fs_tail_fwd<true, true, true> : k_fs_tail_fwd<false, true, true>)
+                        : (noise ? k_fs_tail_fwd<true, false, true> : k_fs_tail_fwd<false, false, true>);
     hipLaunchKernelGGL(kern, dim3(foc_div_up(N, 4)), dim3(256), 0, (hipStream_t)stream, (const _Float16 *)h, (const _Float16 *)c, nears, fars, noise,
                        bg_ray, bg_scalar, N, T, density_scale, thresh, sigma, trans, weights, weights_sum, depth, image, c_width, ray_sumsq, ray_dist, ray_wm);
     FOC_CHECK_LAUNCH(who);
@@ -495,7 +578,11 @@
     FOC_REQUIRE(c_width == 16 || c_width == 4, FOC_E_INVALID, "%s: c_width must be 16 or 4 (got %u)", who, c_width);
     FOC_REQUIRE(grad_image && c && sigma && trans && weights && nears && fars && grad_c && grad_h0, FOC_E_INVALID, "%s: null pointer", who);
     FOC_REQUIRE(T >= 2, FOC_E_INVALID, "%s: T must be >= 2", who);
-    auto kern = grad_dist ? (noise ? k_fs_tail_bwd<true, true> : k_fs_tail_bwd<false, true>) : (noise ? k_fs_tail_bwd<true, false> : k_fs_tail_bwd<false, false>);
+    auto kern = grad_dist ? (noise ? k_fs_tail_bwd<true, true, false> : k_fs_tail_bwd<false, true, false>)
+                          : (noise ? k_fs_tail_bwd<true, false, false> : k_fs_tail_bwd<false, false, false>);
+    if (foc_opt(FOC_OPT_TAIL_PIPELINE))
+        kern = grad_dist ? (noise ? k_fs_tail_bwd<true, true, true> : k_fs_tail_bwd<false, true, true>)
+                         : (noise ? k_fs_tail_bwd<true, false, true> : k_fs_tail_bwd<false, false, true>);
     hipLaunchKernelGGL(kern, dim3(foc_div_up(N, 4)), dim3(256), 0, (hipStream_t)stream, grad_image, grad_ws, grad_depth, (const _Float16 *)c, sigma,
                        trans, weights, nears, fars, noise, bg_ray, bg_scalar, N, T, density_scale, thresh, (_Float16 *)grad_c, (_Float16 *)grad_h0, c_width,
                        grad_sumsq, weights_sum, ray_wm, grad_dist);
diff --git a/focnerf_amd/csrc/fs_common.h b/focnerf_amd/csrc/fs_common.h
--- a/focnerf_amd/csrc/fs_common.h
+++ b/focnerf_amd/csrc/fs_common.h
@@ -9,13 +9,16 @@
     return (uint64_t)(n / FS_RAY_BLOCK) * FS_RAY_BLOCK * T + (uint64_t)i * FS_RAY_BLOCK + n % FS_RAY_BLOCK;
 }
 
-__device__ __forceinline__ FsGeom fs_geom(const float *__restrict__ nears, const float *__restrict__ fars, uint32_t n, uint32_t T) {
+__device__ __forceinline__ FsGeom fs_geom_of(float near, float far, uint32_t T) {
     FsGeom g;
-    g.near = nears[n]; g.far = fars[n];
+    g.near = near; g.far = far;
     g.span = g.far - g.near;
     g.sample_dist = g.span / (float)T;
     g.step = 1.0f / (float)(T - 1);
     return g;
+}
+__device__ __forceinline__ FsGeom fs_geom(const float *__restrict__ nears, const float *__restrict__ fars, uint32_t n, uint32_t T) {
+    return fs_geom_of(nears[n], fars[n], T);
 }
 __device__ __forceinline__ float fs_z0(const FsGeom &g, uint32_t i, uint32_t T) {
     const float lin = (i < T / 2) ? (g.step * (float)i) : fmaf(-g.step, (float)(T - 1 - i), 1.0f);
diff --git a/focnerf_amd/csrc/raymarching.hip b/focnerf_amd/csrc/raymarching.hip
--- a/focnerf_amd/csrc/raymarching.hip
+++ b/focnerf_amd/csrc/raymarching.hip
@@ -8,30 +8,6 @@
 #define RM_RPI   0.3183098861837907f
 
 __device__ __forceinline__ float rm_sign(float x) { return copysignf(1.0f, x); }
-
-__device__ __forceinline__ void rm_near_far(float ox, float oy, float oz, float dx, float dy, float dz, float a0, float a1, float a2, float a3, float a4, float a5,
-                                            float min_near, float &near_out, float &far_out) {
-    const float rdx = 1 / dx, rdy = 1 / dy, rdz = 1 / dz;
-    float near = (a0 - ox) * rdx, far = (a3 - ox) * rdx, t;
-    if (near > far) { t = near; near = far; far = t; }
-    float near_y = (a1 - oy) * rdy, far_y = (a4 - oy) * rdy;
-    if (near_y > far_y) { t = near_y; near_y = far_y; far_y = t; }
-    bool miss = (near > far_y || near_y > far);
-    if (!miss) {
-        if (near_y > near) near = near_y;
-        if (far_y < far) far = far_y;
-        float near_z = (a2 - oz) * rdz, far_z = (a5 - oz) * rdz;
-        if (near_z > far_z) { t = near_z; near_z = far_z; far_z = t; }
-        miss = (near > far_z || near_z > far);
-        if (!miss) {
-            if (near_z > near) near = near_z;
-            if (far_z < far) far = far_z;
-            if (near < min_near) near = min_near;
-        }
-    }
-    near_out = miss ? FLT_MAX : near;
-    far_out = miss ? FLT_MAX : far;
-}
 
 __global__ void __launch_bounds__(256) k_near_far_from_aabb(const float *__restrict__ rays_o, const float *__restrict__ rays_d,
                                      const float *__restrict__ aabb, uint32_t N, float min_near,
diff --git a/focnerf_amd/csrc/sample_math.h b/focnerf_amd/csrc/sample_math.h
--- a/focnerf_amd/csrc/sample_math.h
+++ b/focnerf_amd/csrc/sample_math.h
@@ -1,5 +1,6 @@
 #pragma once
 #include "common.h"
+#include <float.h>
 
 typedef _Float16 h8 __attribute__((ext_vector_type(8)));
 
@@ -50,3 +51,27 @@
 __device__ __forceinline__ FocBg foc_bg(const float *__restrict__ bg_ray, float bg_scalar, uint32_t k) {
     return FocBg{bg_ray ? bg_ray[k * 3] : bg_scalar, bg_ray ? bg_ray[k * 3 + 1] : bg_scalar, bg_ray ? bg_ray[k * 3 + 2] : bg_scalar};
 }
+
+__device__ __forceinline__ void rm_near_far(float ox, float oy, float oz, float dx, float dy, float dz, float a0, float a1, float a2, float a3, float a4, float a5,
+                                            float min_near, float &near_out, float &far_out) {
+    const float rdx = 1 / dx, rdy = 1 / dy, rdz = 1 / dz;
+    float near = (a0 - ox) * rdx, far = (a3 - ox) * rdx, t;
+    if (near > far) { t = near; near = far; far = t; }
+    float near_y = (a1 - oy) * rdy, far_y = (a4 - oy) * rdy;
+    if (near_y > far_y) { t = near_y; near_y = far_y; far_y = t; }
+    bool miss = (near > far_y || near_y > far);
+    if (!miss) {
+        if (near_y > near) near = near_y;
+        if (far_y < far) far = far_y;
+        float near_z = (a2 - oz) * rdz, far_z = (a5 - oz) * rdz;
+        if (near_z > far_z) { t = near_z; near_z = far_z; far_z = t; }
+        miss = (near > far_z || near_z > far);
+        if (!miss) {
+            if (near_z > near) near = near_z;
+            if (far_z < far) far = far_z;
+            if (near < min_near) near = min_near;
+        }
+    }
+    near_out = miss ? FLT_MAX : near;
+    far_out = miss ? FLT_MAX : far;
+}
diff --git a/focnerf_amd/fixedstep.py b/focnerf_amd/fixedstep.py
--- a/focnerf_amd/fixedstep.py
+++ b/focnerf_amd/fixedstep.py
@@ -30,6 +30,21 @@
     if want_ray_sh:
         return enc_in, xyzs, ray_sh
     return enc_in, xyzs
+
+
+def fixed_sample_aabb(rays_o, rays_d, aabb, min_near, noise, T, bound, want_xyzs=False, want_ray_sh=False, ray_block=0):
+    N = rays_o.shape[0]
+    dev = rays_o.device
+    rows = blocked_rows(N, T, ray_block)
+    nears = torch.empty(N, dtype=torch.float32, device=dev)
+    fars = torch.empty(N, dtype=torch.float32, device=dev)
+    enc_in = torch.empty(rows, 3, dtype=torch.float32, device=dev)
+    xyzs = torch.empty(rows, 3, dtype=torch.float32, device=dev) if want_xyzs else None
+    ray_sh = torch.empty(N, 16, dtype=torch.float16, device=dev) if want_ray_sh else None
+    aabb = aabb.contiguous().float()
+    check(lib.foc_fixed_sample_aabb(ptr(rays_o), ptr(rays_d), ptr(aabb), float(min_near), ptr(noise), N, T, float(bound), ptr(xyzs), ptr(enc_in),
+                                    ptr(ray_sh), int(ray_block), ptr(nears), ptr(fars), stream_of(rays_o)), "fixed_sample_aabb")
+    return nears, fars, enc_in, xyzs, ray_sh
 
 
 def ray_sh_rows(rays_d):
@@ -263,20 +278,26 @@
     N, T = rays_o.shape[0], int(num_steps)
     dev = rays_o.device
     aabb = model.aabb_train if model.training else model.aabb_infer
-    nears, fars = raymarching.near_far_from_aabb(rays_o, rays_d, aabb, model.min_near)
+    from .field import field_plan, field_infer
+    from ._lib import get_option
+    plan = field_plan(model)
+    want_tail = plan.tail and model.training and torch.is_grad_enabled()
+    sample_aabb = want_tail and get_option("FOC_SAMPLE_AABB") != 0
+    if not sample_aabb:
+        nears, fars = raymarching.near_far_from_aabb(rays_o, rays_d, aabb, model.min_near)
     noise = torch.rand(N * T, dtype=torch.float32, device=dev) if perturb else None
-    from .field import field_plan, field_infer
-    plan = field_plan(model)
     if getattr(model, "bg_radius", 0) > 0:
         bg_color = model._background_colour(rays_o, rays_d, bg_color)
-    want_tail = plan.tail and model.training and torch.is_grad_enabled()
     fused_infer = not torch.is_grad_enabled() and plan.infer
     if distortion and not torch.is_grad_enabled():
         raise ValueError("render_fixed_steps: distortion=True needs the training route (gradients enabled): the inference paths form no "
                          "differentiable weights; call it under torch.enable_grad() with model.train()")
     rb = ray_block_default() if fused_infer else 0
-    enc_in, _, ray_sh = fixed_sample(rays_o, rays_d, nears, fars, aabb, noise, T, model.bound, want_ray_sh=True) if want_tail else \
-        fixed_sample(rays_o, rays_d, nears, fars, aabb, noise, T, model.bound, ray_block=rb) + (None,)
+    if sample_aabb:
+        nears, fars, enc_in, _, ray_sh = fixed_sample_aabb(rays_o, rays_d, aabb, model.min_near, noise, T, model.bound, want_ray_sh=True)
+    else:
+        enc_in, _, ray_sh = fixed_sample(rays_o, rays_d, nears, fars, aabb, noise, T, model.bound, want_ray_sh=True) if want_tail else \
+            fixed_sample(rays_o, rays_d, nears, fars, aabb, noise, T, model.bound, ray_block=rb) + (None,)
 
     if fused_infer:
         obj_feat = model.encode_object_feature(yolo_details, dev) if plan.uses_object_feature else None
diff --git a/include/focnerf.h b/include/focnerf.h
--- a/include/focnerf.h
+++ b/include/focnerf.h
@@ -284,6 +284,9 @@
 int foc_fixed_sample(const float *rays_o, const float *rays_d, const float *nears, const float *fars,
                      const float *aabb, const float *noise, uint32_t N, uint32_t T, float bound,
                      float *xyzs, float *enc_in, void *ray_sh, uint32_t ray_block, void *stream);
+int foc_fixed_sample_aabb(const float *rays_o, const float *rays_d, const float *aabb, float min_near, const float *noise,
+                          uint32_t N, uint32_t T, float bound, float *xyzs, float *enc_in, void *ray_sh, uint32_t ray_block,
+                          float *nears_out, float *fars_out, void *stream);
 
 int foc_fixed_head_forward(const void *h, const float *rays_d, const float *nears, const float *fars,
                            const float *noise, uint32_t N, uint32_t T, float density_scale,
```

Measured after the change: 1.397 billion, median of 6. Within noise of the previous version (+1.2%).
